# NVIDIA/cuopt

Measured on AMD Instinct MI355X. Metric: pdlp_iterations_per_sec, higher is better.
Workload: dtype f64; 1 GPU; c3: synthetic random sparse LP S(m=1000000,n=1000000,k=10,seed=2), nnz=10000000, longest row 10, CSR fp64/int32, Stable2 preset, tolerances 0 (fixed iteration budget); rows=1000000, cols=1000000, nnz=10000000, parallelism=single GPU

## Files before the change

### cuopt_amd/capi.py

```python
import ctypes as C
import os

import numpy as np

_HERE = os.path.dirname(os.path.abspath(__file__))
LIB_PATH = os.environ.get("CUOPT_AMD_LIB") or os.path.join(_HERE, "lib", "libcuopt.so")

if not os.path.exists(LIB_PATH):
    raise ImportError(
        "cuopt_amd: %s is missing -- build it with `make -C cuopt_amd/csrc` (or "
        "`python -c 'import __graft_entry__ as g; g.build()'`). There is no CPU fallback." % LIB_PATH)

lib = C.CDLL(LIB_PATH, mode=C.RTLD_GLOBAL)

CUOPT_SUCCESS, CUOPT_INVALID_ARGUMENT, CUOPT_MPS_FILE_ERROR, CUOPT_MPS_PARSE_ERROR = 0, 1, 2, 3
CUOPT_VALIDATION_ERROR, CUOPT_OUT_OF_MEMORY, CUOPT_RUNTIME_ERROR = 4, 5, 6
CUOPT_MINIMIZE, CUOPT_MAXIMIZE = 1, -1
STATUS = {0: "NoTermination", 1: "Optimal", 2: "PrimalInfeasible", 3: "DualInfeasible",
          4: "IterationLimit", 5: "TimeLimit", 6: "NumericalError", 7: "PrimalFeasible",
          8: "FeasibleFound", 9: "ConcurrentLimit"}

c_int, c_double, c_void_p, c_char_p = C.c_int32, C.c_double, C.c_void_p, C.c_char_p
P = C.POINTER

# ... 184 lines not shown
for _n in ("cuOptGetObjectiveValue", "cuOptGetSolveTime", "cuOptGetMIPGap", "cuOptGetSolutionBound"):
    _proto(_n, c_int, c_void_p, P(c_double))
_proto("cuOptAmdGetPdlpStats", c_int, c_void_p, P(Result))
_proto("cuOptAmdGetSolveInfo", c_int, c_void_p, c_char_p, c_int)
_proto("cuOptAmdGetName", c_int, c_void_p, c_int, c_int, c_char_p, c_int)

_proto("cuoptamd_last_error", c_char_p)
_proto("cuoptamd_hyper_preset", None, c_int, P(Hyper))
_proto("cuoptamd_default_settings", None, P(SolverSettings))
_proto("cuoptamd_solver_create", c_int, P(c_void_p), P(LP), P(Hyper), P(SolverSettings), c_void_p,
       c_void_p, c_int, c_int, c_int, c_void_p)
_proto("cuoptamd_solver_destroy", None, c_void_p)
_proto("cuoptamd_solver_reset", c_int, c_void_p, c_void_p, c_void_p, c_void_p, c_void_p, P(SolverSettings), c_void_p,
       c_void_p)
_proto("cuoptamd_solver_advance", c_int, c_void_p, c_int, P(Result))
_proto("cuoptamd_solver_get_solution", c_int, c_void_p, c_void_p, c_void_p, c_void_p)
_proto("cuoptamd_solver_device", c_void_p, c_void_p)
_proto("cuoptamd_batch_solve", c_int, c_int, c_void_p, P(Hyper), P(SolverSettings), c_int, c_int, c_void_p, c_void_p, c_void_p, c_void_p)
_proto("cuoptamd_solver_get_warm_start", c_int, c_void_p, P(WarmStart))
_proto("cuoptamd_solver_set_warm_start", c_int, c_void_p, P(WarmStart))
_proto("cuoptamd_warm_start_remap", c_int, P(WarmStart), P(c_int), c_int, P(c_int), c_int, P(WarmStart))
_proto("cuoptamd_solver_row_range", c_int, c_void_p, P(c_int), P(c_int))
_proto("cuoptamd_solver_reorder_info", c_int, c_void_p, c_void_p, c_void_p, c_void_p)
_proto("cuoptamd_partition_rows", None, c_int, c_void_p, c_int, c_void_p)
_proto("cuoptamd_csr_transpose", None, c_int, c_int, *([c_void_p] * 6))

_proto("pdlpdev_last_error", c_char_p)
_proto("pdlpdev_device_count", c_int)
_proto("pdlpdev_device_info", c_int, c_int, c_char_p, c_int, P(c_int), P(C.c_int64))
_proto("pdlpdev_create", c_int, P(c_void_p), c_int, c_int, c_int, *([c_void_p] * 11))
_proto("pdlpdev_destroy", None, c_void_p)
_proto("pdlpdev_comm_unique_id", c_int, c_void_p)
_proto("pdlpdev_comm_init", c_int, c_void_p, c_int, c_int, c_void_p)
_proto("pdlpdev_softcomm_create", c_int, c_int, c_void_p)
_proto("pdlpdev_scaling_compute", c_int, c_void_p, c_int, c_int, c_int, c_double)
_proto("pdlpdev_scale_problem", c_int, c_void_p)
_proto("pdlpdev_init_norms", c_int, c_void_p, c_void_p)
_proto("pdlpdev_problem_norms", c_int, c_void_p, P(c_double), P(c_double))
_proto("pdlpdev_set_step_params", c_int, c_void_p, P(StepParams))
_proto("pdlpdev_set_step", c_int, c_void_p, c_double, c_double)
_proto("pdlpdev_set_k", c_int, c_void_p, c_int)
_proto("pdlpdev_set_initial", c_int, c_void_p, c_void_p, c_void_p)
_proto("pdlpdev_project_primal", c_int, c_void_p)
_proto("pdlpdev_compute_aty", c_int, c_void_p)
_proto("pdlpdev_run", c_int, c_void_p, c_int, P(Ctl))
_proto("pdlpdev_get_ctl", c_int, c_void_p, P(Ctl))
_proto("pdlpdev_clear_error", c_int, c_void_p)
_proto("pdlpdev_set_graph_mode", c_int, c_void_p, c_int)
_proto("pdlpdev_prepare_graphs", c_int, c_void_p)
_proto("pdlpdev_flush_average", c_int, c_void_p)
_proto("pdlpdev_make_average", c_int, c_void_p, c_int)
_proto("pdlpdev_eval", c_int, c_void_p, c_int, c_int, c_double, c_double, c_void_p)
_proto("pdlpdev_restart", c_int, c_void_p, c_int, c_int, c_void_p)
_proto("pdlpdev_save_best", c_int, c_void_p, c_int)
_proto("pdlpdev_trust_region_bounds", c_int, c_void_p, c_int, c_double, c_double, c_double, c_double, c_double, c_double, c_int, c_void_p)
_proto("pdlpdev_eval_infeasibility", c_int, c_void_p, c_int, c_int, c_void_p)
_proto("pdlpdev_get_solution", c_int, c_void_p, c_int, c_void_p, c_void_p, c_void_p)
_proto("pdlpdev_download", C.c_int64, c_void_p, c_int, c_void_p, C.c_int64)
_proto("pdlpdev_spmv", c_int, c_void_p, c_int, c_void_p, c_void_p)
_proto("pdlpdev_time_kernel", c_int, c_void_p, c_int, c_int, P(c_double))
_proto("pdlpdev_synchronize", c_int, c_void_p)
_proto("pdlpdev_device_bytes", C.c_int64, c_void_p)
_proto("cuoptamd_dual_simplex", c_int, c_void_p, c_double, c_int, c_void_p, c_void_p, c_void_p, c_void_p, c_void_p, c_void_p, c_void_p)
_proto("cuoptamd_dual_simplex_from", c_int, c_void_p, c_void_p, c_void_p, c_double, c_int, c_void_p, c_void_p, c_void_p, c_void_p, c_void_p, c_void_p, c_void_p)
_proto("pdlpdev_shard_dataflow", c_int, c_void_p)
_proto("pdlpdev_shard_transport", c_int, c_void_p)
_proto("pdlpdev_shard_wire_bytes", c_int, c_void_p, c_void_p)
_proto("pdlpdev_dense_info", c_int, c_void_p, c_void_p)
_proto("pdlpdev_layout_info", c_int, c_void_p, c_void_p)
_proto("pdlpdev_analyze", c_int, P(c_void_p), c_int, c_int, c_int, c_void_p, c_void_p, c_void_p, c_int)
_proto("pdlpdev_analysis_info", c_int, c_void_p, c_void_p)
_proto("pdlpdev_analysis_maps", c_int, c_void_p, c_void_p, c_void_p)
_proto("pdlpdev_analysis_download", c_int, c_void_p, c_int, c_void_p, c_void_p, c_void_p)
_proto("pdlpdev_create_from_analysis", c_int, P(c_void_p), c_void_p, c_void_p, c_void_p, c_void_p, c_void_p, c_void_p)
_proto("pdlpdev_analysis_destroy", None, c_void_p)
_proto("pdlpdev_debug_sort_pairs", c_int, c_int, C.c_int64, c_void_p, c_void_p, c_int, c_void_p, c_void_p)
_proto("pdlpdev_debug_scan", c_int, c_int, C.c_int64, c_void_p, c_void_p)
_proto("pdlpdev_debug_layout_checksums", c_int, c_void_p, c_void_p)
_proto("cuoptamd_solver_clone", c_int, c_void_p, c_void_p, c_void_p, c_void_p, c_void_p, c_void_p, P(c_void_p))
_proto("cuoptamd_batch_create", c_int, c_void_p, c_int, P(c_void_p))
_proto("cuoptamd_batch_advance", c_int, c_void_p, c_int, c_void_p)
_proto("cuoptamd_batch_destroy", None, c_void_p)
_proto("cuoptamd_batch_reset", c_int, c_void_p, c_void_p, c_void_p, c_void_p, c_void_p)
_proto("cuoptamd_batch_get_solutions", c_int, c_void_p, c_void_p, c_void_p, c_void_p)
_proto("cuoptamd_batch_branch", c_int, c_void_p, c_void_p, c_void_p, c_void_p)
_proto("cuoptamd_batch_solution_views", c_int, c_void_p, c_void_p, c_void_p, c_void_p)
_proto("cuoptamd_batch_device", c_void_p, c_void_p)
_proto("pdlpdev_create_share_stream", None, c_void_p)
_proto("pdlpdev_debug_ipc_export", c_int, c_int, c_int, c_void_p, P(c_void_p))
_proto("pdlpdev_debug_ipc_store", c_int, c_int, c_void_p, c_int, c_double)
_proto("pdlpdev_debug_ipc_wait", c_int, c_int, c_void_p, c_int, c_double)
_proto("pdlpdev_resident_size", c_int, c_int, c_int, C.c_int64)
_proto("pdlpdev_batch_time_kernels", c_int, c_void_p, c_int, c_void_p)
_proto("pdlpdev_synthetic_lp", c_int, c_int, c_int, c_int, c_int, C.c_uint64, *([c_void_p] * 8))

BUF = {n: i for i, n in enumerate(
    ["X", "Y", "X_OTHER", "Y_OTHER", "ATY", "ATY_OTHER", "XBAR", "SUM_X", "SUM_Y", "AVG_X", "AVG_Y",
     "DROW", "DCOL", "A_VALUES", "AT_VALUES", "C", "LB", "UB", "LO", "HI", "RC_CURRENT", "RC_AVERAGE",
     "LAST_RESTART_X", "LAST_RESTART_Y"])}
KERNEL = {n: i for i, n in enumerate(
    ["PRIMAL", "SPMV_A_DUAL", "SPMV_AT_STEP", "STEP_DECISION", "SPMV_A_PLAIN", "SPMV_AT_PLAIN"])}
EV = {n: i for i, n in enumerate(
    ["CX", "DUAL_SUM", "PRES2", "DRES2", "X2", "Y2", "LINF_PRES_REL", "LINF_DRES_REL"])}
CURRENT, AVERAGE = 0, 1


class CuOptError(RuntimeError):
    def __init__(self, code, msg=""):
        super().__init__("cuopt error %d %s" % (code, msg))
        self.code = code


def device_count():
    return int(lib.pdlpdev_device_count())


def device_info(dev=0):
    name = C.create_string_buffer(256)
    cus, mem = c_int(), C.c_int64()
    rc = lib.pdlpdev_device_info(dev, name, 256, C.byref(cus), C.byref(mem))
    if rc != 0:
        raise CuOptError(rc, lib.pdlpdev_last_error().decode())
    return dict(name=name.value.decode(), compute_units=cus.value, hbm_bytes=mem.value)


class Problem:

    def __init__(self, handle):
        self.handle = handle

    @classmethod
    def read(cls, path):
        h = c_void_p()
        rc = lib.cuOptReadProblem(os.fsencode(path), C.byref(h))
        if rc != CUOPT_SUCCESS:
            raise CuOptError(rc, "cuOptReadProblem(%s)" % path)
        return cls(h)

    @classmethod
    def from_dict(cls, p, ranged=True):
        m, n = int(p["m"]), int(p["n"])
        keep = [_i32(p["offsets"]), _i32(p["indices"]), _f64(p["values"]), _f64(p["c"]),
                _f64(p["lb"]), _f64(p["ub"])]
        vt = p.get("var_types")
        vt = (b"C" * n) if vt is None else bytes(bytearray(np.asarray(vt, dtype=np.uint8)))
        h = c_void_p()
        sense = CUOPT_MAXIMIZE if p.get("maximize", False) else CUOPT_MINIMIZE
        off = float(p.get("objective_offset", 0.0))
        if ranged:
            lo, hi = _f64(p["lo"]), _f64(p["hi"])
            rc = lib.cuOptCreateRangedProblem(m, n, sense, off, _ptr(keep[3]), _ptr(keep[0]),
                                              _ptr(keep[1]), _ptr(keep[2]), _ptr(lo), _ptr(hi),
# ... 599 lines not shown
                raise CuOptError(rc, msg)
            self.m, self.n, self.nnz = int(p["m"]), int(p["n"]), len(p["values"])
            return
        m, n = int(p["m"]), int(p["n"])
        off, idx, val = _i32(p["offsets"]), _i32(p["indices"]), _f64(p["values"])
        to, ti, tv = csr_transpose(m, n, off, idx, val)
        c, lo, hi, lb, ub = (_f64(p[k]) for k in ("c", "lo", "hi", "lb", "ub"))
        self.handle = c_void_p()
        rc = lib.pdlpdev_create(C.byref(self.handle), device, m, n, _ptr(off), _ptr(idx), _ptr(val),
                                _ptr(to), _ptr(ti), _ptr(tv), _ptr(c), _ptr(lo), _ptr(hi), _ptr(lb), _ptr(ub))
        if rc != 0:
            msg = lib.pdlpdev_last_error().decode()
            if self.handle:
                lib.pdlpdev_destroy(self.handle)
            self.handle = None
            raise CuOptError(rc, msg)
        self.m, self.n, self.nnz = m, n, len(val)

    def _ck(self, rc):
        if rc != 0:
            raise CuOptError(rc, lib.pdlpdev_last_error().decode())

    def call(self, name, *args):
        self._ck(getattr(lib, "pdlpdev_" + name)(self.handle, *args))

    def ctl(self):
        c = Ctl()
        self._ck(lib.pdlpdev_get_ctl(self.handle, C.byref(c)))
        return c

    def run(self, target_steps):
        c = Ctl()
        self._ck(lib.pdlpdev_run(self.handle, int(target_steps), C.byref(c)))
        return c

    def download(self, name, count):
        out = np.zeros(int(count))
        got = lib.pdlpdev_download(self.handle, BUF[name], _ptr(out), int(count))
        if got < 0:
            raise CuOptError(int(got), lib.pdlpdev_last_error().decode())
        return out[:got]

    def spmv(self, x, transpose=False, rows=None):
        x = _f64(x)
        y = np.zeros(int(rows))
        self._ck(lib.pdlpdev_spmv(self.handle, int(transpose), _ptr(x), _ptr(y)))
        return y

    def eval(self, which, rule_finite=True, eps_p=1e-4, eps_d=1e-4):
        out = np.zeros(len(EV))
        self._ck(lib.pdlpdev_eval(self.handle, which, int(rule_finite), eps_p, eps_d, _ptr(out)))
        return {k: out[i] for k, i in EV.items()}

    def eval_infeasibility(self, which, rule_finite=True):
        out = np.zeros(4)
        self._ck(lib.pdlpdev_eval_infeasibility(self.handle, which, int(rule_finite), _ptr(out)))
        return dict(zip(["max_primal_ray_infeasibility", "primal_ray_linear_objective",
                         "max_dual_ray_infeasibility", "dual_ray_linear_objective"], out.tolist()))

    def trust_region_bounds(self, which, wp, wd, pds=0.5, dds=0.5, primal_weight=1.0, radius=-1.0, scaled_iterates=False):
        out = np.zeros(6)
        self._ck(lib.pdlpdev_trust_region_bounds(self.handle, which, wp, wd, pds, dds, primal_weight, radius,
                                                 int(scaled_iterates), _ptr(out)))
        return dict(zip(["primal_distance2", "dual_distance2", "distance", "lagrangian", "lower_bound",
                         "upper_bound"], out.tolist()))

    def init_norms(self):
        out = np.zeros(3)
        self._ck(lib.pdlpdev_init_norms(self.handle, _ptr(out)))
        return out

    def layout(self):
        out = np.zeros(8, np.int32)
        self._ck(lib.pdlpdev_layout_info(self.handle, _ptr(out)))
        names = {0: "stream", 1: "panel", 2: "resident", 3: "jag", 4: "pb"}

        def side(k):
            d = dict(layout=names[int(out[k])], panels=bool(out[k] == 1), workgroups=int(out[k + 1]))
            if out[k] == 3:
                d["lds_gather_saving_pct"] = int(out[k + 2])
            elif out[k] == 4:
                d["padding_pct"] = int(out[k + 2])
            else:
                d["slabs"] = int(out[k + 2])
                if out[k] == 1:
                    d["row_sums"] = "by_nonzero" if out[6 + k // 3] else "by_row"
            return d
        return dict(A=side(0), At=side(3), resident=bool(out[0] == 2))

    def wire_bytes(self):
        out = np.zeros(3, np.int64)
        self._ck(lib.pdlpdev_shard_wire_bytes(self.handle, _ptr(out)))
        return dict(halo=bool(out[0]), bytes=int(out[1]), bytes_allgather=int(out[2]))

    def layout_checksums(self):
        out = np.zeros(16, np.uint64)
        self._ck(lib.pdlpdev_debug_layout_checksums(self.handle, _ptr(out)))
        return out

    def dense_info(self):
        out = np.zeros(3, np.int64)
        self._ck(lib.pdlpdev_dense_info(self.handle, _ptr(out)))
        return dict(on=bool(out[0]), segments=int(out[1]), entries=int(out[2]))

    def time_kernel(self, kernel, reps=20):
        ms = c_double()
# ... 14 lines not shown
```

### cuopt_amd/csrc/kernels_batch.hip

```cpp
#include <cstring>
#include <hip/hip_runtime.h>

#include "pdlp_ctx.hpp"

#define LAUNCH_CHECK() HIP_TRY(hipGetLastError())

__global__ void k_step_decision_batch(const pdlpdev_decision_args* __restrict__ args);
__global__ void k_set_target(pdlpdev_ctl* ctl, int target);
__global__ void k_set_error(pdlpdev_ctl* ctl);

namespace {

constexpr int kBT = kPanelThreads;
static_assert(kBT == 512, "8 waves of 64 lanes: the reduction below mirrors block_reduce<.., kPanelWaves>");
constexpr int kBatchMax = 16;

struct BatchLp {
  pdlpdev_ctl* ctl;
  double *y0, *y1, *sumy;
  const double *lo, *hi;
  double *x0, *x1, *aty0, *aty1, *sumx;
  const double *c, *lb, *ub;
  pdlpdev_ctx::UniformBounds ubd;
  double *part_a, *part_at;
// ... 777 lines not shown
      const void* f = K == 16 ? batch_jag_kernel<16>(side[t], t == 0) : K == 8 ? batch_jag_kernel<8>(side[t], t == 0)
                    : K == 4  ? batch_jag_kernel<4>(side[t], t == 0)  : batch_jag_kernel<2>(side[t], t == 0);
      HIP_TRY(hipFuncSetAttribute(f, hipFuncAttributeMaxDynamicSharedMemorySize, 160 * 1024));
    }
  pdlpdev_batch* b = new pdlpdev_batch();
  *out      = b;
  b->K = K, b->device = c0->device, b->stream = c0->stream;
  b->a_side = side[0], b->t_side = side[1];
  std::vector<BatchLp>& h = b->lp_host;
  h.resize(K);
  std::vector<pdlpdev_decision_args>& dargs = b->dargs_host;
  dargs.resize(K);
  for (int l = 0; l < K; ++l) {
    pdlpdev_ctx* c = ctx[l];
    b->ctx[l]      = c;
    h[l]     = batch_lp_of(c);
    dargs[l] = pdlpdev_decision_args{c->ctl, c->part_a, side[0].W, c->part_at, side[1].W, c->sp};
    c->batches_alive += 1;
  }
  HIP_TRY(hipMalloc((void**)&b->lp_dev, K * sizeof(BatchLp)));
  HIP_TRY(hipMalloc((void**)&b->xK, ((size_t)c0->n * K + 64) * sizeof(double)));
  HIP_TRY(hipMalloc((void**)&b->yK, ((size_t)c0->m * K + 64) * sizeof(double)));
  HIP_TRY(hipMalloc((void**)&b->dargs_dev, K * sizeof(pdlpdev_decision_args)));
  HIP_TRY(hipMemcpyAsync(b->lp_dev, h.data(), K * sizeof(BatchLp), hipMemcpyHostToDevice, b->stream));
  HIP_TRY(hipMemcpyAsync(b->dargs_dev, dargs.data(), K * sizeof(pdlpdev_decision_args), hipMemcpyHostToDevice, b->stream));
  HIP_TRY(hipMemsetAsync(b->xK, 0, ((size_t)c0->n * K + 64) * sizeof(double), b->stream));
  HIP_TRY(hipMemsetAsync(b->yK, 0, ((size_t)c0->m * K + 64) * sizeof(double), b->stream));
  HIP_TRY(hipStreamSynchronize(b->stream));
  return 0;
}

void pdlpdev_batch_destroy(pdlpdev_batch* b)
{
  if (!b) return;
  for (int l = 0; l < b->K; ++l)
    if (b->ctx[l]) b->ctx[l]->batches_alive -= 1;
  (void)hipSetDevice(b->device);
  if (b->stream) (void)hipStreamSynchronize(b->stream);
  for (auto& kv : b->graphs) (void)hipGraphExecDestroy(kv.second);
  if (b->lp_dev) (void)hipFree(b->lp_dev);
  if (b->dargs_dev) (void)hipFree(b->dargs_dev);
  if (b->xK) (void)hipFree(b->xK);
  if (b->yK) (void)hipFree(b->yK);
  delete b;
}

int pdlpdev_batch_run(pdlpdev_batch* b, const int32_t* targets, pdlpdev_ctl* ctl)
{
  if (!b || !targets) return fail(-1, "pdlpdev_batch_run: null argument");
  roctx::Range range("pdlp: batched PDHG attempts");
  HIP_TRY(hipSetDevice(b->device));
  TRY(batch_refresh_table(b));
  const int K = b->K;
  for (int l = 0; l < K; ++l)
    if (targets[l] > 0) k_set_target<<<1, 1, 0, b->stream>>>(b->ctx[l]->ctl, targets[l]);
  LAUNCH_CHECK();
  TRY(batch_fetch_ctl(b));
  auto wants = [&](int l) { return targets[l] > 0 && b->ctx[l]->ctl_h->error == 0 && b->ctx[l]->ctl_h->steps_taken < targets[l]; };
  int guard = 0;
  for (;;) {
    int remaining = 0;
    int before[kBatchMax], asked[kBatchMax];
    for (int l = 0; l < K; ++l) {
      before[l] = b->ctx[l]->ctl_h->steps_taken;
      asked[l]  = wants(l) ? targets[l] - before[l] : 0;
      remaining = std::max(remaining, asked[l]);
    }
    if (remaining == 0) break;
    const bool use_graph = b->ctx[0]->use_graph != 0;
    while (remaining > 0) {
      int chunk = 1;
      while (chunk * 2 <= remaining && chunk < 64) chunk *= 2;
      if (use_graph) {
        hipGraphExec_t g;
        TRY(batch_graph(b, chunk, &g));
        HIP_TRY(hipGraphLaunch(g, b->stream));
      } else {
        for (int i = 0; i < chunk; ++i) TRY(batch_enqueue(b));
      }
      remaining -= chunk;
    }
    TRY(batch_fetch_ctl(b));
    for (int l = 0; l < K; ++l) {
      if (asked[l] == 0) continue;
      pdlpdev_ctx* c = b->ctx[l];
      c->rejected_in_a_row = c->ctl_h->steps_taken == before[l] ? c->rejected_in_a_row + asked[l] : 0;
      if (c->ctl_h->error == 0 && c->rejected_in_a_row >= 64) {
        c->rejected_in_a_row = 0;
        k_set_error<<<1, 1, 0, b->stream>>>(c->ctl);
        LAUNCH_CHECK();
      }
    }
    TRY(batch_fetch_ctl(b));
    if (++guard > 100000) return fail(-6, "pdlpdev_batch_run: no progress");
  }
  if (ctl)
    for (int l = 0; l < K; ++l) ctl[l] = *b->ctx[l]->ctl_h;
  return 0;
}

int pdlpdev_batch_time_kernels(pdlpdev_batch* b, int reps, double avg_ms[4])
{
  if (!b || !avg_ms) return fail(-1, "pdlpdev_batch_time_kernels: null argument");
  HIP_TRY(hipSetDevice(b->device));
  TRY(batch_refresh_table(b));
  hipStream_t s = b->stream;
  const int K   = b->K;
  if (reps < 1) reps = 1;
  TRY(batch_fetch_ctl(b));
  pdlpdev_ctl saved[kBatchMax], forced[kBatchMax];
  struct Scratch {
    double *sx[kBatchMax] = {nullptr}, *sy[kBatchMax] = {nullptr};
    hipEvent_t ev[8] = {nullptr};
    ~Scratch()
    {
      for (double* p : sx) if (p) (void)hipFree(p);
      for (double* p : sy) if (p) (void)hipFree(p);
      for (hipEvent_t e : ev) if (e) (void)hipEventDestroy(e);
    }
  } scratch;
  double **sx = scratch.sx, **sy = scratch.sy;
  hipEvent_t* ev = scratch.ev;
  for (int l = 0; l < K; ++l) {
    pdlpdev_ctx* c = b->ctx[l];
    saved[l] = forced[l] = *c->ctl_h;
    forced[l].pending_avg = 1, forced[l].target_steps = saved[l].steps_taken + 1, forced[l].error = 0;
    HIP_TRY(hipMalloc((void**)&sx[l], std::max<size_t>(c->n, 1) * sizeof(double)));
    HIP_TRY(hipMalloc((void**)&sy[l], std::max<size_t>(c->m, 1) * sizeof(double)));
    HIP_TRY(hipMemcpyAsync(sx[l], c->sumx, (size_t)c->n * sizeof(double), hipMemcpyDeviceToDevice, s));
    HIP_TRY(hipMemcpyAsync(sy[l], c->sumy, (size_t)c->m * sizeof(double), hipMemcpyDeviceToDevice, s));
  }
  auto arm = [&]() -> int {
    for (int l = 0; l < K; ++l) HIP_TRY(hipMemcpyAsync(b->ctx[l]->ctl, &forced[l], sizeof(pdlpdev_ctl), hipMemcpyHostToDevice, s));
    return 0;
  };
  for (int q = 0; q < 8; ++q) HIP_TRY(hipEventCreate(&ev[q]));
  double sum[4] = {0.0, 0.0, 0.0, 0.0};
  TRY(arm());
  TRY(batch_enqueue(b));
  for (int i = 0; i < reps; ++i) {
    TRY(arm());
    TRY(batch_enqueue(b, ev));
    HIP_TRY(hipStreamSynchronize(s));
    for (int q = 0; q < 4; ++q) {
      float ms = 0.f;
      HIP_TRY(hipEventElapsedTime(&ms, ev[2 * q], ev[2 * q + 1]));
      sum[q] += ms;
    }
  }
  for (int q = 0; q < 4; ++q) avg_ms[q] = sum[q] / reps;
  for (int l = 0; l < K; ++l) {
    pdlpdev_ctx* c = b->ctx[l];
    HIP_TRY(hipMemcpyAsync(c->ctl, &saved[l], sizeof(pdlpdev_ctl), hipMemcpyHostToDevice, s));
    HIP_TRY(hipMemcpyAsync(c->sumx, sx[l], (size_t)c->n * sizeof(double), hipMemcpyDeviceToDevice, s));
    HIP_TRY(hipMemcpyAsync(c->sumy, sy[l], (size_t)c->m * sizeof(double), hipMemcpyDeviceToDevice, s));
  }
  HIP_TRY(hipStreamSynchronize(s));
  return 0;
}

}
```

### cuopt_amd/csrc/kernels_panel.hip

```cpp
#include <hip/hip_runtime.h>

#include "pdlp_kernel_decls.hpp"
#include "pdlp_layouts.hpp"
#include "pdlp_setup.hpp"
#include "spmv_panel.hpp"

template <bool SEG>
__global__ void __launch_bounds__(kPanelThreads)
k_panel_a_dual(PanelView P, const pdlpdev_ctl* __restrict__ ctl, const double* __restrict__ xbar,
               double* __restrict__ y0, double* __restrict__ y1, const double* __restrict__ lo,
               const double* __restrict__ hi, double* __restrict__ sumy, double* __restrict__ part, double* __restrict__ ycopy,
               const p2pdev::Push* __restrict__ push)
{
  if (!loop_active(ctl)) return;
  const int cur = ctl->cur;
  DualEpilogue e{cur ? y1 : y0, cur ? y0 : y1, lo, hi, sumy, ctl->sigma, ctl->step_size,
                 ctl->pending_avg != 0, ycopy, push};
  panel_block<SEG>(P, xbar, e, part);
  if (push) p2pdev::count_exchange(push);
}

template <bool SEG>
__global__ void __launch_bounds__(kPanelThreads)
k_panel_at_step(PanelView P, const pdlpdev_ctl* __restrict__ ctl, const double* __restrict__ y0,
                const double* __restrict__ y1, const double* __restrict__ x0,
                const double* __restrict__ x1, double* __restrict__ aty0, double* __restrict__ aty1,
                double* __restrict__ part)
{
  if (!loop_active(ctl)) return;
  const int cur = ctl->cur;
  StepEpilogue e{cur ? x1 : x0, cur ? x0 : x1, cur ? aty1 : aty0, cur ? aty0 : aty1};
  panel_block<SEG>(P, cur ? y0 : y1 , e, part);
}

template <bool SEG>
__global__ void __launch_bounds__(kPanelThreads)
k_panel_at_cur(PanelView P, const pdlpdev_ctl* __restrict__ ctl, const double* __restrict__ y0,
               const double* __restrict__ y1, double* __restrict__ aty0, double* __restrict__ aty1,
               double* __restrict__ out_override, int use_next)
{
  const int cur = ctl->cur ^ (use_next ? 1 : 0);
  StoreEpilogue e{out_override ? out_override : (cur ? aty1 : aty0)};
  panel_block<SEG>(P, cur ? y1 : y0, e, nullptr);
}

template <bool SEG>
__global__ void __launch_bounds__(kPanelThreads)
k_panel_plain(PanelView P, const double* __restrict__ vec, double* __restrict__ out)
{
  StoreEpilogue e{out};
  panel_block<SEG>(P, vec, e, nullptr);
}

template <bool SEG>
__global__ void __launch_bounds__(kPanelThreads)
k_panel_eval_primal(PanelView P, const pdlpdev_ctl* __restrict__ ctl, int which,
                    const double* __restrict__ x0, const double* __restrict__ x1,
                    const double* __restrict__ avgx, const double* __restrict__ y0,
                    const double* __restrict__ y1, const double* __restrict__ avgy,
                    const double* __restrict__ dr, const double* __restrict__ lo_u,
                    const double* __restrict__ hi_u, double eps_rel, double* __restrict__ linf_rows,
                    double* __restrict__ ax_out, double* __restrict__ part)
{
  const int cur = ctl->cur;
  const double* xv = which == PDLPDEV_AVERAGE ? avgx : (cur ? x1 : x0);
  const double* yv = which == PDLPDEV_AVERAGE ? avgy : (cur ? y1 : y0);
  EvalPrimalEpilogue e{yv, dr, lo_u, hi_u, eps_rel, linf_rows, ax_out};
  panel_block<SEG>(P, xv, e, part);
}

template <bool SEG>
__global__ void __launch_bounds__(kPanelThreads)
k_panel_eval_dual(PanelView P, const pdlpdev_ctl* __restrict__ ctl, int which,
                  const double* __restrict__ x0, const double* __restrict__ x1,
                  const double* __restrict__ avgx, const double* __restrict__ y0,
                  const double* __restrict__ y1, const double* __restrict__ avgy, EvalDualCore core,
                  double* __restrict__ part)
{
  const int cur = ctl->cur;
  core.xhat     = which == PDLPDEV_AVERAGE ? avgx : (cur ? x1 : x0);
  const double* yv = which == PDLPDEV_AVERAGE ? avgy : (cur ? y1 : y0);
  EvalDualEpilogue e{core};
  panel_block<SEG>(P, yv, e, part);
}

template __global__ void k_panel_a_dual<true>(PanelView P, const pdlpdev_ctl* __restrict__ ctl, const double* __restrict__ xbar,
               double* __restrict__ y0, double* __restrict__ y1, const double* __restrict__ lo,
               const double* __restrict__ hi, double* __restrict__ sumy, double* __restrict__ part, double* __restrict__ ycopy,
               const p2pdev::Push* __restrict__ push);
template __global__ void k_panel_a_dual<false>(PanelView P, const pdlpdev_ctl* __restrict__ ctl, const double* __restrict__ xbar,
               double* __restrict__ y0, double* __restrict__ y1, const double* __restrict__ lo,
               const double* __restrict__ hi, double* __restrict__ sumy, double* __restrict__ part, double* __restrict__ ycopy,
               const p2pdev::Push* __restrict__ push);
template __global__ void k_panel_at_step<true>(PanelView P, const pdlpdev_ctl* __restrict__ ctl, const double* __restrict__ y0,
                const double* __restrict__ y1, const double* __restrict__ x0,
                const double* __restrict__ x1, double* __restrict__ aty0, double* __restrict__ aty1,
                double* __restrict__ part);
template __global__ void k_panel_at_step<false>(PanelView P, const pdlpdev_ctl* __restrict__ ctl, const double* __restrict__ y0,
                const double* __restrict__ y1, const double* __restrict__ x0,
                const double* __restrict__ x1, double* __restrict__ aty0, double* __restrict__ aty1,
                double* __restrict__ part);
template __global__ void k_panel_at_cur<true>(PanelView P, const pdlpdev_ctl* __restrict__ ctl, const double* __restrict__ y0,
               const double* __restrict__ y1, double* __restrict__ aty0, double* __restrict__ aty1,
               double* __restrict__ out_override, int use_next);
template __global__ void k_panel_at_cur<false>(PanelView P, const pdlpdev_ctl* __restrict__ ctl, const double* __restrict__ y0,
               const double* __restrict__ y1, double* __restrict__ aty0, double* __restrict__ aty1,
               double* __restrict__ out_override, int use_next);
template __global__ void k_panel_plain<true>(PanelView P, const double* __restrict__ vec, double* __restrict__ out);
template __global__ void k_panel_plain<false>(PanelView P, const double* __restrict__ vec, double* __restrict__ out);
template __global__ void k_panel_eval_primal<true>(PanelView P, const pdlpdev_ctl* __restrict__ ctl, int which,
                    const double* __restrict__ x0, const double* __restrict__ x1,
                    const double* __restrict__ avgx, const double* __restrict__ y0,
                    const double* __restrict__ y1, const double* __restrict__ avgy,
                    const double* __restrict__ dr, const double* __restrict__ lo_u,
                    const double* __restrict__ hi_u, double eps_rel, double* __restrict__ linf_rows,
                    double* __restrict__ ax_out, double* __restrict__ part);
template __global__ void k_panel_eval_primal<false>(PanelView P, const pdlpdev_ctl* __restrict__ ctl, int which,
                    const double* __restrict__ x0, const double* __restrict__ x1,
                    const double* __restrict__ avgx, const double* __restrict__ y0,
                    const double* __restrict__ y1, const double* __restrict__ avgy,
                    const double* __restrict__ dr, const double* __restrict__ lo_u,
                    const double* __restrict__ hi_u, double eps_rel, double* __restrict__ linf_rows,
                    double* __restrict__ ax_out, double* __restrict__ part);
template __global__ void k_panel_eval_dual<true>(PanelView P, const pdlpdev_ctl* __restrict__ ctl, int which,
                  const double* __restrict__ x0, const double* __restrict__ x1,
                  const double* __restrict__ avgx, const double* __restrict__ y0,
                  const double* __restrict__ y1, const double* __restrict__ avgy, EvalDualCore core,
                  double* __restrict__ part);
template __global__ void k_panel_eval_dual<false>(PanelView P, const pdlpdev_ctl* __restrict__ ctl, int which,
                  const double* __restrict__ x0, const double* __restrict__ x1,
                  const double* __restrict__ avgx, const double* __restrict__ y0,
                  const double* __restrict__ y1, const double* __restrict__ avgy, EvalDualCore core,
                  double* __restrict__ part);

int64_t gather_working_set(int32_t rows, int32_t cols, const int32_t* off, const int32_t* idx)
{
// ... 273 lines not shown
```

### cuopt_amd/csrc/pdlp_core_internal.hpp

```cpp
#pragma once
#include "pdlp_ctx.hpp"

#define LAUNCH_CHECK() HIP_TRY(hipGetLastError())

extern "C" {
int fetch_scalars(pdlpdev_ctx* ctx, int count);
int fetch_ctl(pdlpdev_ctx* ctx, pdlpdev_ctl* out);
void launch_plain(pdlpdev_ctx* ctx, int transpose, const double* vec, double* out);
void launch_at_cur(pdlpdev_ctx* ctx, double* out_override, int use_next);
void dense_part(pdlpdev_ctx* ctx, int transpose, const double* v0, const double* v1, int mode, int in_loop);
}

static inline int dual_partials(const pdlpdev_ctx* ctx) { return ctx->pba.on ? ctx->pba.v.B : ctx->ja.on ? ctx->ja.v.nblk + ctx->ja.v.nlong : ctx->pa.on ? ctx->pa.v.W : ctx->a_nb; }
static inline int step_partials(const pdlpdev_ctx* ctx) { return ctx->pbat.on ? ctx->pbat.v.B : ctx->jat.on ? ctx->jat.v.nblk + ctx->jat.v.nlong : ctx->pat.on ? ctx->pat.v.W : ctx->at_nb; }

__global__ void __launch_bounds__(kBlock)
k_flush_average(int n, int m, const pdlpdev_ctl* __restrict__ ctl, const double* __restrict__ x0, const double* __restrict__ x1, const double* __restrict__ y0,
                const double* __restrict__ y1, double* __restrict__ sumx, double* __restrict__ sumy);
__global__ void __launch_bounds__(kBlock) k_finalize(const double* __restrict__ part, int nb, int nq, unsigned op_mask, double* __restrict__ out);
__global__ void __launch_bounds__(kBlock) k_div_inplace(int n, double* __restrict__ v, const double* __restrict__ d);
__global__ void __launch_bounds__(kBlock) k_div_to(int n, double* __restrict__ out, const double* __restrict__ v, const double* __restrict__ d);
__global__ void k_restart_ctl(pdlpdev_ctl* ctl);
__global__ void k_clear_pending(pdlpdev_ctl* ctl);

int sync_panel_values(pdlpdev_ctx* c);
__global__ void __launch_bounds__(kBlock) k_fill(int64_t n, double* __restrict__ d, double v);
__global__ void __launch_bounds__(kBlock) k_scale_vectors(int n, int m, double* __restrict__ c, double* __restrict__ lb, double* __restrict__ ub,
                                                          const double* __restrict__ dc, double* __restrict__ lo, double* __restrict__ hi,
                                                          const double* __restrict__ dr);
__global__ void __launch_bounds__(kBlock) k_scale_matrix(int rows, const int32_t* __restrict__ off, const int32_t* __restrict__ idx, double* __restrict__ val,
                                                         const double* __restrict__ d_self, const double* __restrict__ d_other);
__global__ void __launch_bounds__(kBlock) k_scale_matrix_long(const int32_t* __restrict__ rows_long, const int32_t* __restrict__ off,
                                                              const int32_t* __restrict__ idx, double* __restrict__ val,
                                                              const double* __restrict__ d_self, const double* __restrict__ d_other);
```

### cuopt_amd/csrc/pdlp_create.hip

```cpp
#include "pdlp_ctx.hpp"
#include "pdlp_layouts.hpp"
#include "pdlp_setup.hpp"

__global__ void k_fill(int64_t n, double* __restrict__ d, double v);
int sync_panel_values(pdlpdev_ctx* c);
int resident_tier(int m, int n, int64_t nnz);

static thread_local int g_create_sharded = 0;
static thread_local int g_create_batch_lanes = 0;

static int create_impl(pdlpdev_ctx** out, int device, int32_t m, int32_t n, const int32_t* a_offsets,
                       const int32_t* a_indices, const double* a_values, const int32_t* at_offsets,
                       const int32_t* at_indices, const double* at_values,
                       void (*transpose_ready)(void*), void* user, const double* c, const double* lo,
                       const double* hi, const double* lb, const double* ub, pdlpdev_analysis* an);

extern "C" {

const char* pdlpdev_last_error(void) { return g_err.c_str(); }
void pdlpdev_create_hint(int sharded) { g_create_sharded = sharded; }
void pdlpdev_create_batch_lanes(int lanes) { g_create_batch_lanes = lanes; }
static thread_local pdlpdev_ctx* g_create_stream_donor = nullptr;
void pdlpdev_create_share_stream(pdlpdev_ctx* donor) { g_create_stream_donor = donor; }
int pdlpdev_resident_size(int32_t m, int32_t n, int64_t nnz) { return resident_tier(m, n, nnz) >= 0 ? 1 : 0; }
// ... 445 lines not shown
      rbt = build_row_blocks(n, T.off);
      wlap("row blocks");
      if (walk) at_rc = layout_walk(ctx, P, T);
    };
    struct Join {
      std::thread t;
      ~Join() { if (t.joinable()) t.join(); }
    } worker;
    if (at_thread) worker.t = std::thread(at_side, true);
    {
      LayoutSide A;
      init_side(A, 0);
      A.off = A_off, A.idx = A_idx, A.d_off = ctx->ha_off, A.d_idx = ctx->ha_idx, A.d_val = ctx->ha_val, A.lap = lap;
      A.first_seg = DH.on ? &DH.first_seg : nullptr;
      TRY(layout_walk(ctx, P, A));
      TRY(upload_side(ctx, P, A));
      if (ctx->pa.on && DH.on) TRY(own_segments(ctx, DH, A.ph));
      lap("upload layouts A");
    }
    if (at_thread) worker.t.join();
    else at_side(false);
    lap("wait for the A^T side");
    if ((int64_t)at_offsets[n] != ctx->nnz) return fail(-1, "pdlpdev_create: A and A^T disagree on nnz");
    if (!an) {
      TRY(upload_i32(ctx, &ctx->at_off, at_offsets, (size_t)n + 1));
      TRY(upload_i32(ctx, &ctx->at_idx, at_indices, nnz, 8));
      TRY(upload_f64(ctx, &ctx->at_val, at_values, nnz, 8));
    }
    ctx->at_nlong = (int)lat.size();
    if (ctx->at_nlong) TRY(upload_i32(ctx, &ctx->at_long, lat.data(), lat.size()));
    const bool hot_t = !hT_off.empty();
    ctx->hat_off = ctx->at_off, ctx->hat_idx = ctx->at_idx, ctx->hat_val = ctx->at_val;
    ctx->hot_nnz_at = (int64_t)T.off[n];
    if (hot_t) {
      TRY(upload_i32(ctx, &ctx->hat_off, T.off, (size_t)n + 1));
      TRY(upload_i32(ctx, &ctx->hat_idx, T.idx, (size_t)ctx->hot_nnz_at, 8));
      TRY(dev_alloc(ctx, &ctx->hat_val, (size_t)ctx->hot_nnz_at + 8));
      TRY(upload_i32(ctx, &ctx->dense.s_perm_at, hT_perm.data(), hT_perm.size()));
    }
    if (DH.on) TRY(dev_alloc(ctx, &ctx->dense.add_n, (size_t)n));
    ctx->at_nb = (int)rbt.size() / 2 - 1;
    TRY(upload_i32(ctx, &ctx->at_rb, rbt.data(), rbt.size()));
    lap("upload A^T");
    T.d_off = ctx->hat_off, T.d_idx = ctx->hat_idx, T.d_val = ctx->hat_val;
    TRY(at_thread ? at_rc : layout_walk(ctx, P, T));
    TRY(upload_side(ctx, P, T));
    if (ctx->pat.on && DH.on) TRY(column_segments(ctx, DH, T.ph));
    lap("upload layouts A^T");
    HIP_TRY(hipStreamSynchronize(ctx->stream));
  }
  {
    const char* small_env = getenv("CUOPT_AMD_SMALL");
    const int tier        = resident_tier(m, n, ctx->nnz);
    ctx->small_resident   = tier >= 0 && !(small_env && atoi(small_env) == 0) && !ctx->dense.add_m && !ctx->dense.add_n;
    if (small_env && atoi(small_env) != 0 && tier < 0)
      return fail(-1, "CUOPT_AMD_SMALL=1: the LP does not fit the resident kernel (m, n <= 2048, nnz <= 4096 ...)");
  }
  ctx->pa.v.dense_add = ctx->ja.v.dense_add = ctx->pba.v.dense_add = ctx->dense.add_m;
  ctx->pat.v.dense_add = ctx->jat.v.dense_add = ctx->pbat.v.dense_add = ctx->dense.add_n;
  if (ctx->pa.v.dn_own_seg) ctx->pa.v.dense_add = nullptr;
  if (ctx->pat.v.dn_pan_ptr) ctx->pat.v.dense_add = nullptr;
  ctx->slab_cap += slab_rest;
  TRY(dev_alloc(ctx, &ctx->part_a, (size_t)8 * std::max({ctx->a_nb, ctx->pba.on ? ctx->pba.v.B : 0, ctx->pa.on ? ctx->pa.v.W : 0, ctx->ja.on ? ctx->ja.v.nblk + ctx->ja.v.nlong : 0, 1})));
  TRY(dev_alloc(ctx, &ctx->part_at, (size_t)8 * std::max({ctx->at_nb, ctx->pbat.on ? ctx->pbat.v.B : 0, ctx->pat.on ? ctx->pat.v.W : 0, ctx->jat.on ? ctx->jat.v.nblk + ctx->jat.v.nlong : 0, 1})));
  TRY(dev_alloc(ctx, &ctx->part_g, (size_t)8 * 2048));
  TRY(dev_alloc(ctx, &ctx->scal, kScalars));
  TRY(dev_alloc(ctx, &ctx->ctl, 1));
  TRY(dev_alloc(ctx, &ctx->ar_buf, (size_t)n + kSlicePad));
  lap("partial buffers");
  k_fill<<<grid_for(m), kBlock, 0, ctx->stream>>>(m, ctx->dr, 1.0);
  k_fill<<<grid_for(n), kBlock, 0, ctx->stream>>>(n, ctx->dc, 1.0);
  HIP_TRY(hipGetLastError());
  lap("fill D");
  TRY(sync_panel_values(ctx));
  lap("panel values (permute)");
  if (P.mode == LayoutPolicy::kTimed) {
    TRY(pick_layout(ctx, &ctx->pa, m, ctx->a_nb, ctx->a_rb, ctx->ha_off, ctx->ha_idx, ctx->ha_val, ctx->tmp_n, ctx->tmp_m, "A"));
    lap("layout autotune A");
    TRY(pick_layout(ctx, &ctx->pat, n, ctx->at_nb, ctx->at_rb, ctx->hat_off, ctx->hat_idx, ctx->hat_val, ctx->tmp_m, ctx->tmp_n, "A^T"));
    lap("layout autotune");
  }
  HIP_TRY(hipStreamSynchronize(ctx->stream));
  scratch_free(ctx);
  return 0;
}

extern "C" {

void pdlpdev_destroy(pdlpdev_ctx* ctx)
{
  if (!ctx) return;
  (void)hipSetDevice(ctx->device);
  if (ctx->stream) (void)hipStreamSynchronize(ctx->stream);
  scratch_free(ctx);
  for (auto& kv : ctx->graphs) (void)hipGraphExecDestroy(kv.second);
  if (ctx->shared_with_parent && ctx->parent) ctx->parent->clones_alive -= 1;
  if (ctx->batches_alive > 0)
    fprintf(stderr, "[cuopt_amd] pdlpdev_destroy: %d batch(es) still hold this context -- destroy the batch before its members\n", ctx->batches_alive);
  if (ctx->clones_alive > 0)
    fprintf(stderr, "[cuopt_amd] pdlpdev_destroy: %d clone(s) of this context are still alive -- they alias its matrices and must be destroyed first\n", ctx->clones_alive);
  for (void* mapped : ctx->p2p.opened) (void)hipIpcCloseMemHandle(mapped);
  if (ctx->p2p.base) (void)hipFree(ctx->p2p.base);
  if (ctx->comm && !ctx->soft) comm_cache::release(ctx->comm_key);
  for (void* p : ctx->allocs) (void)hipFree(p);
  const bool whole = ctx->stream && ctx->scal_h && ctx->first_chunk && !ctx->shared_with_parent && !ctx->stream_borrowed;
  if (!(whole && give_recycled(Recycled{ctx->device, ctx->stream, ctx->scal_h, ctx->first_chunk}))) {
// ... 9 lines not shown
```

### cuopt_amd/csrc/pdlp_ctx.hpp

```cpp
#pragma once
#include <hip/hip_runtime.h>
#include <hip/hip_ext.h>

#include <tuple>
#include <utility>

#include <dlfcn.h>
#include <unistd.h>
#include <mutex>
#include <math.h>
#include <stdarg.h>
#include <stdio.h>
#include <string.h>

#include <algorithm>
#include <chrono>
#include <map>
#include <memory>
#include <string>
#include <vector>

#include "host_parallel.hpp"
#include "pdlp_kernels.hpp"
#include "pdlp_epilogues.hpp"
// ... 327 lines not shown
  double *lrx = nullptr, *lry = nullptr, *rc[2] = {nullptr, nullptr};
  double *tmp_n = nullptr, *tmp_m = nullptr;
  double *ax_u[3] = {nullptr, nullptr, nullptr}, *aty_u[3] = {nullptr, nullptr, nullptr};
  double* rc_scratch = nullptr;
  double *bestx = nullptr, *besty = nullptr, *bestrc = nullptr;
  double *part_a = nullptr, *part_at = nullptr;
  double *part_g = nullptr;
  double *scal = nullptr;
  double *scal_h = nullptr;
  pdlpdev_ctl *ctl = nullptr, *ctl_h = nullptr;
  pdlpdev_step_params sp = {0.3, 0.6, 0.5, 0.5};
  rccl::comm_t comm = nullptr;
  softcomm::Comm* soft = nullptr;
  std::string comm_key;
  int rank = 0, world = 1;
  double* ar_buf = nullptr;
  bool rsag = false;
  int slice = 0;
  double* rs_buf = nullptr;
  double* rs_scal = nullptr;
  bool owner = false;
  int ypad = 0;
  double* ygather = nullptr;
  int32_t oc_rows = 0;
  int64_t oc_nnz = 0;
  int32_t *oc_off = nullptr, *oc_idx = nullptr, *oc_rb = nullptr, *oc_long = nullptr;
  double* oc_val = nullptr;
  int oc_nb = 0, oc_nlong = 0;
  Panels poc;
  Jag joc;
  double* part_oc = nullptr;
  struct Halo {
    bool on = false;
    std::vector<int32_t> recv_off[2], recv_cnt[2], send_off[2], send_cnt[2];
    int64_t bytes = 0, bytes_allgather = 0;
  } halo;
  struct P2P {
    bool on = false;
    char* base = nullptr;
    size_t bytes = 0;
    size_t off_x = 0, off_y = 0, off_s = 0, off_f = 0;
    p2pdev::Peers peers{};
    std::vector<void*> opened;
    unsigned long long* epoch = nullptr;
    int* fault = nullptr;
    p2pdev::Push* push_dev = nullptr;
    p2pdev::Push push_host[p2pdev::kKinds];
  } p2p;
  bool prof_armed = false;
  static constexpr int kProfPairs = 8;
  hipEvent_t prof_ev[2 * kProfPairs] = {};
  int prof_used = 0;
  int rejected_in_a_row = 0;
  int use_graph = 1;
  int batch_lanes = 0;
  bool comm_warm = false;
  bool graph_comm_failed = false;
  char* slab = nullptr;
  size_t slab_cap = 0, slab_used = 0;
  char* arena = nullptr;
  char* first_chunk = nullptr;
  bool stream_borrowed = false;
  size_t arena_used = 0;
  bool small_resident = false;
  bool shared_with_parent = false;
  pdlpdev_ctx* parent = nullptr;
  bool rows_aliased = false;
  int clones_alive = 0;
  bool rows_private = false;
  int batches_alive = 0;
  std::map<int, hipGraphExec_t> graphs;
  std::vector<void*> allocs;
  int64_t bytes = 0;
  struct Scratch {
    void* p;
    size_t bytes;
    bool busy;
  };
  std::vector<Scratch> scratch;
};
inline int scratch_take(pdlpdev_ctx* c, void** p, size_t bytes)
{
  bytes = std::max<size_t>(bytes, 256);
  for (auto& b : c->scratch)
    if (!b.busy && b.bytes >= bytes && b.bytes <= 2 * bytes + 4096) {
      b.busy = true;
      *p     = b.p;
      return 0;
    }
  HIP_TRY(hipMalloc(p, bytes));
  c->scratch.push_back(pdlpdev_ctx::Scratch{*p, bytes, true});
  return 0;
}
inline void scratch_release(pdlpdev_ctx* c, void* p)
{
  for (auto& b : c->scratch)
    if (b.p == p) b.busy = false;
}
inline void scratch_free(pdlpdev_ctx* c)
{
  for (auto& b : c->scratch) (void)hipFree(b.p);
  c->scratch.clear();
}

struct pdlpdev_decision_args {
  pdlpdev_ctl* ctl;
  const double* part_dy;
  int nb_dy;
  const double* part_t;
  int nb_t;
  pdlpdev_step_params sp;
};

constexpr int kGenericBlocks = 1024;
constexpr int kScalars       = 64;

struct PerDeviceOnce {
  std::mutex m;
  bool done[64] = {};
  template <class F>
  int run(int device, F&& f)
  {
    std::lock_guard<std::mutex> lock(m);
    if (device < 0 || device >= 64) return f();
    if (done[device]) return 0;
    const int rc = f();
    if (rc == 0) done[device] = true;
    return rc;
  }
};

struct Recycled {
  int device;
  hipStream_t stream;
  double* pinned;
  char* chunk;
};
inline std::mutex g_recycle_mutex;
inline std::vector<Recycled> g_recycled;
inline bool take_recycled(int device, Recycled* out)
{
  std::lock_guard<std::mutex> lock(g_recycle_mutex);
  for (size_t i = 0; i < g_recycled.size(); ++i)
    if (g_recycled[i].device == device) {
      *out = g_recycled[i];
      g_recycled.erase(g_recycled.begin() + i);
      return true;
    }
  return false;
}
inline bool give_recycled(const Recycled& r)
{
  std::lock_guard<std::mutex> lock(g_recycle_mutex);
  if (g_recycled.size() >= 16) return false;
  g_recycled.push_back(r);
  return true;
}

constexpr size_t kArenaChunk = (size_t)1 << 20, kArenaMaxItem = (size_t)256 << 10;
template <class T>
inline int dev_alloc(pdlpdev_ctx* c, T** p, size_t count)
{
  size_t bytes = std::max<size_t>(count, 1) * sizeof(T);
  c->bytes += (int64_t)bytes;
  if (bytes <= kArenaMaxItem) {
    const size_t need = (bytes + 255) & ~(size_t)255;
    if (c->arena == nullptr || c->arena_used + need > kArenaChunk) {
      HIP_TRY(hipMalloc((void**)&c->arena, kArenaChunk));
// ... 48 lines not shown
```

### cuopt_amd/csrc/pdlp_device.hip

```cpp
#include "pdlp_ctx.hpp"
#include "pdlp_layouts.hpp"
#include "pdlp_setup.hpp"


__global__ void __launch_bounds__(kBlock) k_fill(int64_t n, double* __restrict__ d, double v)
{
  for (int64_t i = blockIdx.x * (int64_t)kBlock + threadIdx.x; i < n; i += (int64_t)gridDim.x * kBlock)
    d[i] = v;
}
__global__ void __launch_bounds__(kBlock) k_scale_vectors(int n, int m, double* __restrict__ c,
                                                          double* __restrict__ lb,
                                                          double* __restrict__ ub,
                                                          const double* __restrict__ dc,
                                                          double* __restrict__ lo,
                                                          double* __restrict__ hi,
                                                          const double* __restrict__ dr)
{
  const int tot = n > m ? n : m;
  for (int i = blockIdx.x * kBlock + threadIdx.x; i < tot; i += gridDim.x * kBlock) {
    if (i < n) {
      c[i]  = c[i] * dc[i];
      lb[i] = lb[i] / dc[i];
      ub[i] = ub[i] / dc[i];
    }
// ... 190 lines not shown
{
  if (!loop_active(ctl)) return;
  {
    __shared__ double red[3 * 8];
    double acc[3] = {0.0, 0.0, 0.0};
    for (int i = threadIdx.x; i < nb_dy; i += kBlock) acc[0] += part_dy[i];
    for (int i = threadIdx.x; i < nb_t; i += kBlock) {
      acc[1] += part_t[i];
      acc[2] += part_t[nb_t + i];
    }
    block_reduce<SumOp, 3>(acc, red);
    if (threadIdx.x == 0) {
      for (int q = 0; q < push->world; ++q) {
        double* d = push->slot(q);
        p2pdev::put(d, acc[0]), p2pdev::put(d + 1, acc[1]), p2pdev::put(d + 2, acc[2]);
      }
      asm volatile("s_waitcnt vmcnt(0)" ::: "memory");
      push->epoch[push->kind] = push->epoch[push->kind] + 1;
      p2pdev::raise(push);
    }
    __syncthreads();
  }
  if (!p2pdev::wait_flags(flags, world, 2, epoch)) {
    if (threadIdx.x == 0) *fault = 1, ctl->error = 1;
    return;
  }
  if (threadIdx.x != 0) return;
  double sum[3] = {0.0, 0.0, 0.0};
  for (int q = 0; q < world; ++q)
    for (int k = 0; k < 3; ++k) sum[k] += __hip_atomic_load(landed + 4 * q + k, __ATOMIC_RELAXED, __HIP_MEMORY_SCOPE_SYSTEM);
  pdlpdev_ctl lc = *ctl;
  apply_step_decision(&lc, sum[0], sum[1], sum[2], sp);
  *ctl = lc;
}

__global__ void __launch_bounds__(kBlock)
k_permute_pad(int64_t n, const int32_t* __restrict__ perm, const double* __restrict__ src, double* __restrict__ dst)
{
  for (int64_t i = blockIdx.x * (int64_t)kBlock + threadIdx.x; i < n; i += (int64_t)gridDim.x * kBlock) {
    const int32_t k = perm[i];
    dst[i]          = k >= 0 ? src[k] : 0.0;
  }
}
__global__ void __launch_bounds__(kBlock)
k_permute(int64_t n, const int32_t* __restrict__ perm, const double* __restrict__ src, double* __restrict__ dst)
{
  for (int64_t i = blockIdx.x * (int64_t)kBlock + threadIdx.x; i < n; i += (int64_t)gridDim.x * kBlock)
    dst[i] = src[perm[i]];
}

__global__ void __launch_bounds__(kBlock)
k_flush_average(int n, int m, const pdlpdev_ctl* __restrict__ ctl, const double* __restrict__ x0,
                const double* __restrict__ x1, const double* __restrict__ y0,
                const double* __restrict__ y1, double* __restrict__ sumx, double* __restrict__ sumy)
{
  if (ctl->pending_avg == 0) return;
  const int cur           = ctl->cur;
  const double w          = ctl->step_size;
  const double* __restrict__ x = cur ? x1 : x0;
  const double* __restrict__ y = cur ? y1 : y0;
  const int tot = n > m ? n : m;
  for (int i = blockIdx.x * kBlock + threadIdx.x; i < tot; i += gridDim.x * kBlock) {
    if (i < n) sumx[i] = sumx[i] + w * x[i];
    if (i < m) sumy[i] = sumy[i] + w * y[i];
  }
}
__global__ void k_clear_pending(pdlpdev_ctl* ctl) { ctl->pending_avg = 0; }

__global__ void __launch_bounds__(kBlock)
k_sum_partials_to(const double* __restrict__ part, int nb, double* __restrict__ out)
{
  __shared__ double red[8];
  double acc[1] = {0.0};
  for (int i = threadIdx.x; i < nb; i += kBlock) acc[0] += part[i];
  block_reduce<SumOp, 1>(acc, red);
  if (threadIdx.x == 0) out[0] = acc[0];
}

__global__ void __launch_bounds__(kBlock)
k_pack_step_sums(const double* __restrict__ part_dy, int nb_dy, const double* __restrict__ part_t, int nb_t, double* __restrict__ out)
{
  __shared__ double red[3 * 8];
  double acc[3] = {0.0, 0.0, 0.0};
  for (int i = threadIdx.x; i < nb_dy; i += kBlock) acc[0] += part_dy[i];
  for (int i = threadIdx.x; i < nb_t; i += kBlock) {
    acc[1] += part_t[i];
    acc[2] += part_t[nb_t + i];
  }
  block_reduce<SumOp, 3>(acc, red);
  if (threadIdx.x == 0) {
    out[0] = acc[0], out[1] = acc[1], out[2] = acc[2];
  }
}

__global__ void k_restart_ctl(pdlpdev_ctl* ctl)
{
  ctl->sum_weights       = 0.0;
  ctl->its_since_restart = 0;
  ctl->pending_avg       = 0;
}
__global__ void k_set_step(pdlpdev_ctl* ctl, double step, double w)
{
  if (step >= 0.0) ctl->step_size = step;
  ctl->primal_weight = w;
  ctl->tau           = ctl->step_size / w;
  ctl->sigma         = ctl->step_size * w;
}
__global__ void k_set_target(pdlpdev_ctl* ctl, int target) { ctl->target_steps = target; }
__global__ void k_set_k(pdlpdev_ctl* ctl, int k) { ctl->k = k; }
// ... 125 lines not shown
                        (mode == LayoutPolicy::kAuto && gcols * 8 > P.ws_limit && gather_working_set(nc, (int32_t)gcols, off, ridx.data()) > P.ws_limit);
    if (nc > 0 && !ctx->joc.on && panels) {
      PanelHost h = build_panels(nc, (int32_t)gcols, off, ridx.data(), P.slab_bytes, true);
      TRY(upload_panels(ctx, &ctx->poc, h, ctx->oc_off, ctx->oc_idx, ctx->oc_val));
    }
  }
  TRY(dev_alloc(ctx, &ctx->part_oc, (size_t)8 * std::max(oc_partials(ctx), 1)));
  {
    const char* tr = getenv("CUOPT_AMD_SHARD_TRANSPORT");
    if (tr && std::string(tr) == "p2p") TRY(p2p_setup(ctx));
    else if (tr && std::string(tr) != "collective") return fail(-1, "CUOPT_AMD_SHARD_TRANSPORT must be collective or p2p");
  }
  if (ctx->poc.on) k_permute<<<grid_for(ctx->poc.nent), kBlock, 0, s>>>(ctx->poc.nent, ctx->poc.perm, ctx->oc_val, ctx->poc.val);
  if (ctx->joc.on) k_permute<<<grid_for(ctx->joc.nent), kBlock, 0, s>>>(ctx->joc.nent, ctx->joc.perm, ctx->oc_val, ctx->joc.val);
  HIP_TRY(hipGetLastError());
  {
    const int W = ctx->world;
    std::vector<int32_t> need((size_t)4 * W, 0), xl(W, 0x7fffffff), xh(W, -1);
    int32_t *d_lo = nullptr, *d_hi = nullptr;
    TRY(dev_alloc(ctx, &d_lo, 16));
    TRY(dev_alloc(ctx, &d_hi, 16));
    HIP_TRY(hipMemcpyAsync(d_lo, xl.data(), W * sizeof(int32_t), hipMemcpyHostToDevice, s));
    HIP_TRY(hipMemcpyAsync(d_hi, xh.data(), W * sizeof(int32_t), hipMemcpyHostToDevice, s));
    if (ctx->nnz > 0) k_slice_ranges<<<grid_for(ctx->nnz, 8), kBlock, 0, s>>>(ctx->nnz, ctx->a_idx, ctx->slice, W, d_lo, d_hi);
    HIP_TRY(hipMemcpyAsync(xl.data(), d_lo, W * sizeof(int32_t), hipMemcpyDeviceToHost, s));
    HIP_TRY(hipMemcpyAsync(xh.data(), d_hi, W * sizeof(int32_t), hipMemcpyDeviceToHost, s));
    HIP_TRY(hipStreamSynchronize(s));
    std::vector<int32_t> yl(W, 0x7fffffff), yh(W, -1);
    for (int64_t k = 0; k < nnz; ++k) {
      const int32_t pos = ridx[(size_t)k];
      const int q       = pos / ctx->ypad;
      yl[q] = std::min(yl[q], pos), yh[q] = std::max(yh[q], pos);
    }
    for (int q = 0; q < W; ++q) {
      need[(size_t)4 * q + 0] = xh[q] >= 0 ? xl[q] : 0, need[(size_t)4 * q + 1] = xh[q] >= 0 ? xh[q] + 1 : 0;
      need[(size_t)4 * q + 2] = yh[q] >= 0 ? yl[q] : 0, need[(size_t)4 * q + 3] = yh[q] >= 0 ? yh[q] + 1 : 0;
    }
    TRY(halo_setup(ctx, need.data()));
  }
  HIP_TRY(hipStreamSynchronize(s));
  return 0;
}

int fetch_scalars(pdlpdev_ctx* ctx, int count)
{
  HIP_TRY(hipMemcpyAsync(ctx->scal_h, ctx->scal, count * sizeof(double), hipMemcpyDeviceToHost, ctx->stream));
  HIP_TRY(hipStreamSynchronize(ctx->stream));
  return 0;
}
int fetch_ctl(pdlpdev_ctx* ctx, pdlpdev_ctl* out)
{
  HIP_TRY(hipMemcpyAsync(ctx->ctl_h, ctx->ctl, sizeof(pdlpdev_ctl), hipMemcpyDeviceToHost, ctx->stream));
  HIP_TRY(hipStreamSynchronize(ctx->stream));
  if (out) *out = *ctx->ctl_h;
  return 0;
}


static int reduce_vec(pdlpdev_ctx* ctx, int mode, int64_t n, const double* a, const double* b, int slot)
{
  const int g = std::min(grid_for(n), kGenericBlocks);
  switch (mode) {
    case 0: k_reduce<0><<<g, kBlock, 0, ctx->stream>>>(n, a, b, ctx->part_g); break;
    case 1: k_reduce<1><<<g, kBlock, 0, ctx->stream>>>(n, a, b, ctx->part_g); break;
    case 2: k_reduce<2><<<g, kBlock, 0, ctx->stream>>>(n, a, b, ctx->part_g); break;
    default: k_reduce<3><<<g, kBlock, 0, ctx->stream>>>(n, a, b, ctx->part_g); break;
  }
  k_finalize<<<1, kBlock, 0, ctx->stream>>>(ctx->part_g, g, 1, mode == 0 ? 1u : 0u, ctx->scal + slot);
  LAUNCH_CHECK();
  return 0;
}

int pdlpdev_agree_max(pdlpdev_ctx* ctx, double* value)
{
  if (!ctx->comm) return 0;
  HIP_TRY(hipSetDevice(ctx->device));
  HIP_TRY(hipMemcpyAsync(ctx->scal + 60, value, sizeof(double), hipMemcpyHostToDevice, ctx->stream));
  TRY(allreduce(ctx, ctx->scal + 60, 1, rccl::kMax));
  HIP_TRY(hipMemcpyAsync(ctx->scal_h + 60, ctx->scal + 60, sizeof(double), hipMemcpyDeviceToHost, ctx->stream));
  HIP_TRY(hipStreamSynchronize(ctx->stream));
  *value = ctx->scal_h[60];
  return 0;
}

int pdlpdev_init_norms(pdlpdev_ctx* ctx, double out[3])
{
  HIP_TRY(hipSetDevice(ctx->device));
  TRY(reduce_vec(ctx, 0, ctx->nnz, ctx->a_val, nullptr, 0));
  TRY(reduce_vec(ctx, 1, ctx->n, ctx->c, nullptr, 1));
  TRY(reduce_vec(ctx, 2, ctx->m, ctx->lo, ctx->hi, 2));
  TRY(allreduce(ctx, ctx->scal + 0, 1, rccl::kMax));
  TRY(allreduce(ctx, ctx->scal + 2, 1, rccl::kSum));
  TRY(fetch_scalars(ctx, 3));
  out[0] = ctx->scal_h[0], out[1] = ctx->scal_h[1], out[2] = ctx->scal_h[2];
  return 0;
}

int pdlpdev_reset(pdlpdev_ctx* ctx, const double* lb, const double* ub, const double* lo, const double* hi)
{
  HIP_TRY(hipSetDevice(ctx->device));
  if (!ctx->scaled) return fail(-1, "pdlpdev_reset: the problem has not been scaled yet");
  ctx->rejected_in_a_row = 0;
  hipStream_t s = ctx->stream;
  const size_t nb = (size_t)ctx->n * sizeof(double), mb = (size_t)ctx->m * sizeof(double);
  auto put = [&](const double* src, double* unscaled, double* scaled, size_t bytes) -> int {
    if (!src || bytes == 0) return 0;
    HIP_TRY(hipMemcpyAsync(unscaled, src, bytes, hipMemcpyHostToDevice, s));
    HIP_TRY(hipMemcpyAsync(scaled, unscaled, bytes, hipMemcpyDeviceToDevice, s));
    return 0;
  };
  TRY(put(lb, ctx->lb_u, ctx->lb, nb));
  TRY(put(ub, ctx->ub_u, ctx->ub, nb));
  {
    const pdlpdev_ctx::UniformBounds before = ctx->ubd;
    ctx->note_uniform_bounds(lb, ub);
    const pdlpdev_ctx::UniformBounds& now = ctx->ubd;
    if (before.lb_same != now.lb_same || before.ub_same != now.ub_same || (now.lb_same && before.lb != now.lb) || (now.ub_same && before.ub != now.ub)) {
      for (auto& kv : ctx->graphs) (void)hipGraphExecDestroy(kv.second);
      ctx->graphs.clear();
    }
  }
  if ((lo || hi) && (ctx->rows_aliased || (ctx->clones_alive > 0 && !ctx->rows_private))) {
    for (double** v : {&ctx->lo, &ctx->lo_u, &ctx->hi, &ctx->hi_u}) {
      const double* src = *v;
      TRY(dev_alloc(ctx, v, (size_t)ctx->m));
      HIP_TRY(hipMemcpyAsync(*v, src, mb, hipMemcpyDeviceToDevice, s));
    }
    ctx->rows_aliased = false;
    ctx->rows_private = true;
    for (auto& kv : ctx->graphs) (void)hipGraphExecDestroy(kv.second);
    ctx->graphs.clear();
  }
  TRY(put(lo, ctx->lo_u, ctx->lo, mb));
  TRY(put(hi, ctx->hi_u, ctx->hi, mb));
  if (lb || ub || lo || hi)
    k_scale_bounds<<<grid_for(std::max(ctx->m, ctx->n)), kBlock, 0, s>>>(ctx->n, ctx->m, lb ? ctx->lb : nullptr, ub ? ctx->ub : nullptr,
                                                                      ctx->dc, lo ? ctx->lo : nullptr, hi ? ctx->hi : nullptr, ctx->dr);
  for (int i = 0; i < 2; ++i) {
    HIP_TRY(hipMemsetAsync(ctx->x[i], 0, nb, s));
    HIP_TRY(hipMemsetAsync(ctx->aty[i], 0, nb, s));
    HIP_TRY(hipMemsetAsync(ctx->rc[i], 0, nb, s));
    HIP_TRY(hipMemsetAsync(ctx->y[i], 0, mb, s));
  }
  for (double* v : {ctx->xbar, ctx->sumx, ctx->avgx, ctx->lrx}) HIP_TRY(hipMemsetAsync(v, 0, nb, s));
  for (double* v : {ctx->sumy, ctx->avgy, ctx->lry}) HIP_TRY(hipMemsetAsync(v, 0, mb, s));
  HIP_TRY(hipMemsetAsync(ctx->ctl, 0, sizeof(pdlpdev_ctl), s));
  LAUNCH_CHECK();
  return 0;
}
int pdlpdev_weight_norms(pdlpdev_ctx* ctx, int unscaled, double out[2])
{
  HIP_TRY(hipSetDevice(ctx->device));
  TRY(reduce_vec(ctx, 1, ctx->n, unscaled ? ctx->c_u : ctx->c, nullptr, 1));
  TRY(reduce_vec(ctx, 2, ctx->m, unscaled ? ctx->lo_u : ctx->lo, unscaled ? ctx->hi_u : ctx->hi, 2));
  TRY(allreduce(ctx, ctx->scal + 2, 1, rccl::kSum));
  TRY(fetch_scalars(ctx, 3));
  out[0] = ctx->scal_h[1], out[1] = ctx->scal_h[2];
  return 0;
}


int pdlpdev_problem_norms(pdlpdev_ctx* ctx, double* norm_c, double* norm_b)
{
  HIP_TRY(hipSetDevice(ctx->device));
  TRY(reduce_vec(ctx, 1, ctx->n, ctx->c_u, nullptr, 0));
  TRY(reduce_vec(ctx, 2, ctx->m, ctx->lo_u, ctx->hi_u, 1));
  TRY(allreduce(ctx, ctx->scal + 1, 1, rccl::kSum));
  TRY(fetch_scalars(ctx, 2));
  if (norm_c) *norm_c = sqrt(ctx->scal_h[0]);
  if (norm_b) *norm_b = sqrt(ctx->scal_h[1]);
  return 0;
}

int pdlpdev_set_step_params(pdlpdev_ctx* ctx, const pdlpdev_step_params* p)
{
  ctx->sp = *p;
  for (auto& kv : ctx->graphs) (void)hipGraphExecDestroy(kv.second);
  ctx->graphs.clear();
  return 0;
}
int pdlpdev_set_step(pdlpdev_ctx* ctx, double step_size, double primal_weight)
{
  HIP_TRY(hipSetDevice(ctx->device));
  k_set_step<<<1, 1, 0, ctx->stream>>>(ctx->ctl, step_size, primal_weight);
  LAUNCH_CHECK();
  return 0;
}
int pdlpdev_set_k(pdlpdev_ctx* ctx, int32_t k)
{
  HIP_TRY(hipSetDevice(ctx->device));
  k_set_k<<<1, 1, 0, ctx->stream>>>(ctx->ctl, k);
  LAUNCH_CHECK();
  return 0;
}
int pdlpdev_set_initial(pdlpdev_ctx* ctx, const double* x, const double* y)
{
  HIP_TRY(hipSetDevice(ctx->device));
  TRY(fetch_ctl(ctx, nullptr));
  const int cur = ctx->ctl_h->cur;
  if (x) {
    HIP_TRY(hipMemcpyAsync(ctx->x[cur], x, (size_t)ctx->n * sizeof(double), hipMemcpyHostToDevice, ctx->stream));
    k_div_inplace<<<grid_for(ctx->n), kBlock, 0, ctx->stream>>>(ctx->n, ctx->x[cur], ctx->dc);
  }
  if (y) {
    HIP_TRY(hipMemcpyAsync(ctx->y[cur], y, (size_t)ctx->m * sizeof(double), hipMemcpyHostToDevice, ctx->stream));
    k_div_inplace<<<grid_for(ctx->m), kBlock, 0, ctx->stream>>>(ctx->m, ctx->y[cur], ctx->dr);
  }
  LAUNCH_CHECK();
  HIP_TRY(hipStreamSynchronize(ctx->stream));
  return 0;
}
}
extern "C" {
int pdlpdev_initial_solution_stats(pdlpdev_ctx* ctx, double out[5], const double* x0_unscaled, const double* y0_unscaled)
{
  HIP_TRY(hipSetDevice(ctx->device));
  if ((x0_unscaled == nullptr) != (y0_unscaled == nullptr)) return fail(-1, "initial_solution_stats: both unscaled vectors or none");
  hipStream_t s = ctx->stream;
  const int n = ctx->n, m = ctx->m;
  TRY(fetch_ctl(ctx, nullptr));
  const int cur = ctx->ctl_h->cur;
  const double *xv = ctx->x[cur], *yv = ctx->y[cur], *atyv = ctx->aty[cur];
  if (x0_unscaled) {
    const int nxt = 1 - cur;
    HIP_TRY(hipMemcpyAsync(ctx->x[nxt], x0_unscaled, (size_t)n * sizeof(double), hipMemcpyHostToDevice, s));
    HIP_TRY(hipMemcpyAsync(ctx->y[nxt], y0_unscaled, (size_t)m * sizeof(double), hipMemcpyHostToDevice, s));
    double* prod = ctx->comm ? ctx->ar_buf : ctx->aty[nxt];
    launch_plain(ctx, 1, ctx->y[nxt], prod);
    LAUNCH_CHECK();
    if (ctx->comm) TRY(allreduce(ctx, prod, (size_t)n, rccl::kSum));
    xv = ctx->x[nxt], yv = ctx->y[nxt], atyv = prod;
  } else {
    TRY(pdlpdev_compute_aty(ctx));
  }
  const int g = std::min(grid_for(n), kGenericBlocks);
  k_dot<<<g, kBlock, 0, s>>>(n, xv, atyv, ctx->part_g);
  k_finalize<<<1, kBlock, 0, s>>>(ctx->part_g, g, 1, 0u, ctx->scal + 48);
  TRY(reduce_vec(ctx, 1, n, xv, nullptr, 49));
  TRY(reduce_vec(ctx, 1, m, yv, nullptr, 50));
  TRY(reduce_vec(ctx, 0, n, xv, nullptr, 51));
  TRY(reduce_vec(ctx, 0, m, yv, nullptr, 52));
  LAUNCH_CHECK();
  if (ctx->comm) {
    TRY(allreduce(ctx, ctx->scal + 50, 1, rccl::kSum));
    TRY(allreduce(ctx, ctx->scal + 52, 1, rccl::kMax));
  }
  HIP_TRY(hipMemcpyAsync(ctx->scal_h + 48, ctx->scal + 48, 5 * sizeof(double), hipMemcpyDeviceToHost, s));
  HIP_TRY(hipStreamSynchronize(s));
  for (int i = 0; i < 5; ++i) out[i] = ctx->scal_h[48 + i];
  return 0;
}
// ... 187 lines not shown
    launch_a_dual(ctx);
    launch_at_cur(ctx, ctx->ar_buf, 1);
    LAUNCH_CHECK();
    TRY(reduce_scatter(ctx, ctx->ar_buf, ctx->rs_buf, (size_t)ctx->slice));
    const int g = std::min(grid_for(len), kGenericBlocks);
    launch_k(ctx, k_step_stats, g, kBlock, 0, len, g, ctx->ctl, ctx->rs_buf, ctx->x[0] + cs, ctx->x[1] + cs, ctx->aty[0] + cs, ctx->aty[1] + cs, ctx->part_g);
    launch_k(ctx, k_pack_step_sums, 1, kBlock, 0, ctx->part_a, dual_partials(ctx), ctx->part_g, g, ctx->rs_scal);
    LAUNCH_CHECK();
    TRY(allreduce(ctx, ctx->rs_scal, 3, rccl::kSum));
    launch_k(ctx, k_step_decision, 1, kDecisionThreads, 0, ctx->ctl, nullptr, 0, ctx->rs_scal + 1, 1, ctx->rs_scal, ctx->sp);
    LAUNCH_CHECK();
    return 0;
  }
  launch_k(ctx, k_primal, grid_for(n), kBlock, 0, n, ctx->ctl, ctx->x[0], ctx->x[1], ctx->aty[0], ctx->aty[1], ctx->c, ctx->lb, ctx->ub, ctx->xbar, ctx->sumx, (const p2pdev::Push*)nullptr, ctx->ubd);
  launch_a_dual(ctx);
  if (!ctx->comm) {
    launch_at_step(ctx);
    launch_decision(ctx);
  } else {
    launch_at_cur(ctx, ctx->ar_buf, 1);
    launch_k(ctx, k_sum_partials_to, 1, kBlock, 0, ctx->part_a, dual_partials(ctx), ctx->ar_buf + n);
    LAUNCH_CHECK();
    TRY(allreduce(ctx, ctx->ar_buf, (size_t)n + 1, rccl::kSum));
    const int g = std::min(grid_for(n), kGenericBlocks);
    launch_k(ctx, k_step_stats, g, kBlock, 0, n, g, ctx->ctl, ctx->ar_buf, ctx->x[0], ctx->x[1], ctx->aty[0], ctx->aty[1], ctx->part_g);
    launch_k(ctx, k_step_decision, 1, kDecisionThreads, 0, ctx->ctl, nullptr, 0, ctx->part_g, g, ctx->ar_buf + n, ctx->sp);
  }
  LAUNCH_CHECK();
  return 0;
}

static int get_graph(pdlpdev_ctx* ctx, int attempts, hipGraphExec_t* out)
{
  auto it = ctx->graphs.find(attempts);
  if (it != ctx->graphs.end()) {
    *out = it->second;
    return 0;
  }
  hipGraph_t graph;
  HIP_TRY(hipStreamBeginCapture(ctx->stream, hipStreamCaptureModeThreadLocal));
  int rc = 0;
  for (int i = 0; i < attempts && rc == 0; ++i) rc = enqueue_attempt(ctx);
  hipError_t e = hipStreamEndCapture(ctx->stream, &graph);
  if (rc != 0) return rc;
  HIP_TRY(e);
  hipGraphExec_t exec;
  HIP_TRY(hipGraphInstantiate(&exec, graph, nullptr, nullptr, 0));
  HIP_TRY(hipGraphDestroy(graph));
  ctx->graphs[attempts] = exec;
  *out                  = exec;
  return 0;
}

int pdlpdev_run(pdlpdev_ctx* ctx, int32_t target_steps, pdlpdev_ctl* ctl)
{
  roctx::Range range("pdlp: PDHG attempts");
  HIP_TRY(hipSetDevice(ctx->device));
  if (ctx->small_resident && !ctx->comm) {
    TRY(resident_run(ctx, target_steps));
    if (ctl) *ctl = *ctx->ctl_h;
    return 0;
  }
  k_set_target<<<1, 1, 0, ctx->stream>>>(ctx->ctl, target_steps);
  LAUNCH_CHECK();
  TRY(fetch_ctl(ctx, nullptr));
  int guard = 0;
  while (ctx->ctl_h->error == 0 && ctx->ctl_h->steps_taken < target_steps) {
    int remaining = target_steps - ctx->ctl_h->steps_taken;
    const bool rccl_graphs = ctx->comm && !ctx->p2p.on && !ctx->soft && !ctx->graph_comm_failed;
    bool replayed = false;
    if (rccl_graphs && ctx->use_graph && !ctx->comm_warm) {
      TRY(enqueue_attempt(ctx));
      ctx->comm_warm = true;
      remaining -= 1;
    }
    if (ctx->use_graph && (!ctx->comm || ctx->p2p.on || rccl_graphs)) {
      replayed = true;
      while (remaining > 0) {
        int chunk = 1;
        while (chunk * 2 <= remaining && chunk < 64) chunk *= 2;
        hipGraphExec_t g;
        const int grc = get_graph(ctx, chunk, &g);
        if (grc != 0 && rccl_graphs) {
          ctx->graph_comm_failed = true;
          (void)hipGetLastError();
          replayed = false;
          break;
        }
        TRY(grc);
        HIP_TRY(hipGraphLaunch(g, ctx->stream));
        remaining -= chunk;
      }
    }
    if (!replayed) {
      for (int i = 0; i < remaining; ++i) TRY(enqueue_attempt(ctx));
    }
    const int before = ctx->ctl_h->steps_taken, asked = target_steps - before;
    TRY(fetch_ctl(ctx, nullptr));
    if (ctx->p2p.on && ctx->ctl_h->error != 0) {
      int fault = 0;
      HIP_TRY(hipMemcpy(&fault, ctx->p2p.fault, sizeof(int), hipMemcpyDeviceToHost));
      if (fault) return fail(-6, "direct peer transport: rank %d waited 5 s for another rank's data (a peer failed or is stuck)", ctx->rank);
    }
    ctx->rejected_in_a_row = ctx->ctl_h->steps_taken == before ? ctx->rejected_in_a_row + asked : 0;
    if (ctx->ctl_h->error == 0 && ctx->rejected_in_a_row >= 64) {
      ctx->rejected_in_a_row = 0;
      k_set_error<<<1, 1, 0, ctx->stream>>>(ctx->ctl);
      LAUNCH_CHECK();
      TRY(fetch_ctl(ctx, nullptr));
    }
    if (++guard > 100000) return fail(-6, "pdlpdev_run: no progress");
  }
  if (ctx->rsag && guard > 0) {
    const int cur = ctx->ctl_h->cur;
    TRY(all_gather(ctx, ctx->x[cur], (size_t)ctx->slice));
    TRY(all_gather(ctx, ctx->aty[cur], (size_t)ctx->slice));
    TRY(all_gather(ctx, ctx->sumx, (size_t)ctx->slice));
  }
  if (ctl) *ctl = *ctx->ctl_h;
  return 0;
}

int pdlpdev_copy_in(void* dst, const void* src, size_t bytes)
{
  if (bytes == 0) return 0;
  if (!dst || !src) return fail(-1, "pdlpdev_copy_in: null pointer");
  hipPointerAttribute_t attr;
  memset(&attr, 0, sizeof(attr));
  const hipError_t e = hipPointerGetAttributes(&attr, src);
  if (e == hipSuccess && (attr.type == hipMemoryTypeDevice || attr.type == hipMemoryTypeManaged)) {
    HIP_TRY(hipMemcpy(dst, src, bytes, hipMemcpyDeviceToHost));
    return 0;
  }
  (void)hipGetLastError();
  memcpy(dst, src, bytes);
  return 0;
}

void pdlpdev_range_push(const char* name)
{
  roctx::load();
  if (roctx::Push) roctx::Push(name);
}
void pdlpdev_range_pop(void)
{
  if (roctx::Pop) roctx::Pop();
}

int pdlpdev_prepare_graphs(pdlpdev_ctx* ctx)
{
  HIP_TRY(hipSetDevice(ctx->device));
  if (!ctx->use_graph || (ctx->comm && !ctx->p2p.on) || ctx->small_resident) return 0;
  for (int chunk = 1; chunk <= 64; chunk *= 2) {
    hipGraphExec_t g;
    TRY(get_graph(ctx, chunk, &g));
  }
  return 0;
}

int pdlpdev_get_ctl(pdlpdev_ctx* ctx, pdlpdev_ctl* ctl)
{
  HIP_TRY(hipSetDevice(ctx->device));
  return fetch_ctl(ctx, ctl);
}
int pdlpdev_clear_error(pdlpdev_ctx* ctx)
{
  HIP_TRY(hipSetDevice(ctx->device));
  k_clear_error<<<1, 1, 0, ctx->stream>>>(ctx->ctl);
  LAUNCH_CHECK();
  return 0;
}
int pdlpdev_set_graph_mode(pdlpdev_ctx* ctx, int use_graph)
{
  ctx->use_graph = use_graph;
  return 0;
}

int pdlpdev_get_solution(pdlpdev_ctx* ctx, int which, double* x, double* y, double* rc)
{
  HIP_TRY(hipSetDevice(ctx->device));
  TRY(fetch_ctl(ctx, nullptr));
  const int cur = ctx->ctl_h->cur;
  hipStream_t s = ctx->stream;
  if (which == PDLPDEV_BEST) {
    if (!ctx->bestx) return fail(-1, "pdlpdev_get_solution(BEST): nothing was saved");
    if (x) {
      k_unscale<<<grid_for(ctx->n), kBlock, 0, s>>>(ctx->n, ctx->bestx, ctx->dc, ctx->tmp_n);
      HIP_TRY(hipMemcpyAsync(x, ctx->tmp_n, (size_t)ctx->n * sizeof(double), hipMemcpyDeviceToHost, s));
    }
    if (y) {
      k_unscale<<<grid_for(ctx->m), kBlock, 0, s>>>(ctx->m, ctx->besty, ctx->dr, ctx->tmp_m);
      HIP_TRY(hipMemcpyAsync(y, ctx->tmp_m, (size_t)ctx->m * sizeof(double), hipMemcpyDeviceToHost, s));
    }
    if (rc) HIP_TRY(hipMemcpyAsync(rc, ctx->bestrc, (size_t)ctx->n * sizeof(double), hipMemcpyDeviceToHost, s));
    LAUNCH_CHECK();
    HIP_TRY(hipStreamSynchronize(s));
    return 0;
  }
  if (x) {
    k_unscale<<<grid_for(ctx->n), kBlock, 0, s>>>(ctx->n, which == PDLPDEV_AVERAGE ? ctx->avgx : ctx->x[cur], ctx->dc, ctx->tmp_n);
    HIP_TRY(hipMemcpyAsync(x, ctx->tmp_n, (size_t)ctx->n * sizeof(double), hipMemcpyDeviceToHost, s));
  }
  if (y) {
    k_unscale<<<grid_for(ctx->m), kBlock, 0, s>>>(ctx->m, which == PDLPDEV_AVERAGE ? ctx->avgy : ctx->y[cur], ctx->dr, ctx->tmp_m);
    HIP_TRY(hipMemcpyAsync(y, ctx->tmp_m, (size_t)ctx->m * sizeof(double), hipMemcpyDeviceToHost, s));
  }
  if (rc)
    HIP_TRY(hipMemcpyAsync(rc, ctx->rc[which == PDLPDEV_AVERAGE ? 1 : 0], (size_t)ctx->n * sizeof(double), hipMemcpyDeviceToHost, s));
  LAUNCH_CHECK();
  HIP_TRY(hipStreamSynchronize(s));
  return 0;
}

static int64_t locate_buffer(pdlpdev_ctx* ctx, int id, double** ptr)
{
  if (hipSetDevice(ctx->device) != hipSuccess) return -2;
  if (fetch_ctl(ctx, nullptr) != 0) return -2;
  const int cur = ctx->ctl_h->cur;
  double* src   = nullptr;
  int64_t count = 0;
  const int64_t n = ctx->n, m = ctx->m, nnz = ctx->nnz;
  switch (id) {
    case PDLPDEV_BUF_X: src = ctx->x[cur], count = n; break;
    case PDLPDEV_BUF_Y: src = ctx->y[cur], count = m; break;
    case PDLPDEV_BUF_X_OTHER: src = ctx->x[cur ^ 1], count = n; break;
    case PDLPDEV_BUF_Y_OTHER: src = ctx->y[cur ^ 1], count = m; break;
    case PDLPDEV_BUF_ATY: src = ctx->aty[cur], count = n; break;
    case PDLPDEV_BUF_ATY_OTHER: src = ctx->aty[cur ^ 1], count = n; break;
    case PDLPDEV_BUF_XBAR: src = ctx->xbar, count = n; break;
    case PDLPDEV_BUF_SUM_X: src = ctx->sumx, count = n; break;
    case PDLPDEV_BUF_SUM_Y: src = ctx->sumy, count = m; break;
    case PDLPDEV_BUF_AVG_X: src = ctx->avgx, count = n; break;
    case PDLPDEV_BUF_AVG_Y: src = ctx->avgy, count = m; break;
    case PDLPDEV_BUF_DROW: src = ctx->dr, count = m; break;
    case PDLPDEV_BUF_DCOL: src = ctx->dc, count = n; break;
    case PDLPDEV_BUF_A_VALUES: src = ctx->a_val, count = nnz; break;
    case PDLPDEV_BUF_AT_VALUES: src = ctx->at_val, count = nnz; break;
    case PDLPDEV_BUF_C: src = ctx->c, count = n; break;
    case PDLPDEV_BUF_LB: src = ctx->lb, count = n; break;
    case PDLPDEV_BUF_UB: src = ctx->ub, count = n; break;
    case PDLPDEV_BUF_LO: src = ctx->lo, count = m; break;
    case PDLPDEV_BUF_HI: src = ctx->hi, count = m; break;
    case PDLPDEV_BUF_RC_CURRENT: src = ctx->rc[0], count = n; break;
    case PDLPDEV_BUF_RC_AVERAGE: src = ctx->rc[1], count = n; break;
    case PDLPDEV_BUF_LAST_RESTART_X: src = ctx->lrx, count = n; break;
    case PDLPDEV_BUF_LAST_RESTART_Y: src = ctx->lry, count = m; break;
    default: fail(-1, "unknown buffer %d", id); return -1;
  }
  *ptr = src;
  return count;
}

int64_t pdlpdev_download(pdlpdev_ctx* ctx, int id, void* host, int64_t max_elements)
{
  double* src   = nullptr;
  int64_t count = locate_buffer(ctx, id, &src);
  if (count < 0) return count;
  count = std::min(count, max_elements);
  if (count > 0) {
    if (hipMemcpyAsync(host, src, (size_t)count * sizeof(double), hipMemcpyDeviceToHost, ctx->stream) != hipSuccess) return -2;
    if (hipStreamSynchronize(ctx->stream) != hipSuccess) return -2;
  }
  return count;
}

int64_t pdlpdev_upload(pdlpdev_ctx* ctx, int id, const void* host, int64_t elements)
{
  double* dst   = nullptr;
  int64_t count = locate_buffer(ctx, id, &dst);
  if (count < 0) return count;
  if (id == PDLPDEV_BUF_A_VALUES || id == PDLPDEV_BUF_AT_VALUES) {
    fail(-1, "matrix values cannot be overwritten");
    return -1;
  }
  count = std::min(count, elements);
  if ((id == PDLPDEV_BUF_LB && ctx->ubd.lb_same) || (id == PDLPDEV_BUF_UB && ctx->ubd.ub_same)) {
    if (id == PDLPDEV_BUF_LB) ctx->ubd.lb_same = 0;
    else ctx->ubd.ub_same = 0;
    for (auto& kv : ctx->graphs) (void)hipGraphExecDestroy(kv.second);
    ctx->graphs.clear();
  }
  if (count > 0) {
    if (hipMemcpyAsync(dst, host, (size_t)count * sizeof(double), hipMemcpyHostToDevice, ctx->stream) != hipSuccess) return -2;
    if (hipStreamSynchronize(ctx->stream) != hipSuccess) return -2;
  }
  return count;
}

int pdlpdev_set_loop_state(pdlpdev_ctx* ctx, double sum_weights, int32_t its_since_restart, int32_t k)
{
  HIP_TRY(hipSetDevice(ctx->device));
  k_set_loop_state<<<1, 1, 0, ctx->stream>>>(ctx->ctl, sum_weights, its_since_restart, k);
  LAUNCH_CHECK();
  return 0;
}

int pdlpdev_spmv(pdlpdev_ctx* ctx, int transpose, const double* x, double* y)
{
  HIP_TRY(hipSetDevice(ctx->device));
  hipStream_t s  = ctx->stream;
  const int rows = transpose ? ctx->n : ctx->m, cols = transpose ? ctx->m : ctx->n;
  double* in     = transpose ? ctx->tmp_m : ctx->tmp_n;
  double* outv   = transpose ? ctx->tmp_n : ctx->tmp_m;
  HIP_TRY(hipMemcpyAsync(in, x, (size_t)cols * sizeof(double), hipMemcpyHostToDevice, s));
  launch_plain(ctx, transpose, in, outv);
  LAUNCH_CHECK();
  HIP_TRY(hipMemcpyAsync(y, outv, (size_t)rows * sizeof(double), hipMemcpyDeviceToHost, s));
  HIP_TRY(hipStreamSynchronize(s));
  return 0;
}

int pdlpdev_time_kernel(pdlpdev_ctx* ctx, int kernel_id, int reps, double* avg_ms)
{
  HIP_TRY(hipSetDevice(ctx->device));
  hipStream_t s = ctx->stream;
  if (reps < 1) reps = 1;
  TRY(fetch_ctl(ctx, nullptr));
  pdlpdev_ctl saved = *ctx->ctl_h;
  pdlpdev_ctl forced = saved;
  forced.pending_avg  = 1;
  forced.target_steps = saved.steps_taken + 1;
  forced.error        = 0;
  double *sx = nullptr, *sy = nullptr;
  HIP_TRY(hipMalloc((void**)&sx, std::max<size_t>(ctx->n, 1) * sizeof(double)));
  HIP_TRY(hipMalloc((void**)&sy, std::max<size_t>(ctx->m, 1) * sizeof(double)));
  HIP_TRY(hipMemcpyAsync(sx, ctx->sumx, (size_t)ctx->n * sizeof(double), hipMemcpyDeviceToDevice, s));
  HIP_TRY(hipMemcpyAsync(sy, ctx->sumy, (size_t)ctx->m * sizeof(double), hipMemcpyDeviceToDevice, s));
  HIP_TRY(hipMemcpyAsync(ctx->ctl, &forced, sizeof(forced), hipMemcpyHostToDevice, s));
  HIP_TRY(hipStreamSynchronize(s));
  for (hipEvent_t& e : ctx->prof_ev) HIP_TRY(hipEventCreate(&e));
  auto one = [&]() {
    switch (kernel_id) {
      case PDLPDEV_K_PRIMAL:
        launch_k(ctx, k_primal, grid_for(ctx->n), kBlock, 0, ctx->n, ctx->ctl, ctx->x[0], ctx->x[1], ctx->aty[0], ctx->aty[1], ctx->c, ctx->lb, ctx->ub, ctx->xbar, ctx->sumx, (const p2pdev::Push*)nullptr, ctx->ubd);
        break;
      case PDLPDEV_K_SPMV_A_DUAL: launch_a_dual(ctx); break;
      case PDLPDEV_K_SPMV_AT_STEP: launch_at_step(ctx); break;
      case PDLPDEV_K_STEP_DECISION: launch_decision(ctx); break;
      case PDLPDEV_K_SPMV_A_PLAIN:
        launch_plain(ctx, 0, ctx->xbar, ctx->tmp_m);
        break;
      case PDLPDEV_K_SPMV_AT_PLAIN:
        launch_plain(ctx, 1, ctx->y[saved.cur], ctx->tmp_n);
        break;
      default: return fail(-1, "pdlpdev_time_kernel: unknown kernel %d", kernel_id);
    }
    return 0;
  };
  const bool loop_kernel = kernel_id == PDLPDEV_K_PRIMAL || kernel_id == PDLPDEV_K_SPMV_A_DUAL ||
                           kernel_id == PDLPDEV_K_SPMV_AT_STEP || kernel_id == PDLPDEV_K_STEP_DECISION;
  auto attempt = [&](bool timed) -> int {
    const int order[4] = {PDLPDEV_K_PRIMAL, PDLPDEV_K_SPMV_A_DUAL, PDLPDEV_K_SPMV_AT_STEP, PDLPDEV_K_STEP_DECISION};
    const int wanted   = kernel_id;
    const int slot = loop_kernel ? wanted : (wanted == PDLPDEV_K_SPMV_A_PLAIN ? PDLPDEV_K_SPMV_A_DUAL : PDLPDEV_K_SPMV_AT_STEP);
    int rc = 0;
    for (int id : order) {
      const bool mine = id == slot;
      kernel_id       = mine ? wanted : id;
      ctx->prof_armed = mine && timed;
      if (ctx->prof_armed) ctx->prof_used = 0;
      rc              = one();
      ctx->prof_armed = false;
      if (rc != 0) break;
      if (id == PDLPDEV_K_STEP_DECISION)
        HIP_TRY(hipMemcpyAsync(ctx->ctl, &forced, sizeof(forced), hipMemcpyHostToDevice, s));
    }
    kernel_id = wanted;
    return rc;
  };
  TRY(attempt(false));
// ... 130 lines not shown
```

### cuopt_amd/csrc/pdlp_eval.hip

```cpp
#include "pdlp_ctx.hpp"
#include "pdlp_layouts.hpp"
#include "pdlp_setup.hpp"
#include "pdlp_launch.hpp"
#include "pdlp_core_internal.hpp"

__global__ void __launch_bounds__(kBlock)
k_make_average(int n, int m, int mode, const pdlpdev_ctl* __restrict__ ctl,
               const double* __restrict__ x0, const double* __restrict__ x1,
               const double* __restrict__ y0, const double* __restrict__ y1,
               const double* __restrict__ sumx, const double* __restrict__ sumy,
               double* __restrict__ avgx, double* __restrict__ avgy)
{
  const int cur = ctl->cur;
  const double* __restrict__ x = cur ? x1 : x0;
  const double* __restrict__ y = cur ? y1 : y0;
  const double sw = ctl->sum_weights;
  const int tot   = n > m ? n : m;
  for (int i = blockIdx.x * kBlock + threadIdx.x; i < tot; i += gridDim.x * kBlock) {
    if (i < n) avgx[i] = mode == 0 ? x[i] : (mode == 1 ? 0.0 : sumx[i] / sw);
    if (i < m) avgy[i] = mode == 0 ? y[i] : (mode == 1 ? 0.0 : sumy[i] / sw);
  }
}


__global__ void __launch_bounds__(kBlock)
k_eval_dual_elementwise(int n, int nbg, const pdlpdev_ctl* __restrict__ ctl, int which,
                        const double* __restrict__ x0, const double* __restrict__ x1,
                        const double* __restrict__ avgx, const double* __restrict__ reduced,
                        EvalDualCore core, double* __restrict__ part)
{
  __shared__ double red[20];
  const int cur = ctl->cur;
  core.xhat     = which == PDLPDEV_AVERAGE ? avgx : (cur ? x1 : x0);
  double acc[4] = {0.0, 0.0, 0.0, 0.0};
  for (int j = blockIdx.x * kBlock + threadIdx.x; j < n; j += gridDim.x * kBlock)
    core.col(j, reduced[j], acc);
  block_reduce<SumOp, 4>(acc, red);
  if (threadIdx.x == 0)
    for (int q = 0; q < 4; ++q) part[(size_t)q * nbg + blockIdx.x] = acc[q];
}
__global__ void __launch_bounds__(kBlock)
k_max_partials(int n, const double* __restrict__ v, double* __restrict__ part)
{
  __shared__ double red[8];
  double acc[1] = {0.0};
  for (int i = blockIdx.x * kBlock + threadIdx.x; i < n; i += gridDim.x * kBlock)
    acc[0] = v[i] > acc[0] ? v[i] : acc[0];
  block_reduce<MaxOp, 1>(acc, red);
  if (threadIdx.x == 0) part[blockIdx.x] = acc[0];
}


__global__ void __launch_bounds__(kBlock)
k_infeas_rows(int m, int nbg, const pdlpdev_ctl* __restrict__ ctl, int which, const double* __restrict__ ax,
              const double* __restrict__ y0, const double* __restrict__ y1, const double* __restrict__ avgy,
              const double* __restrict__ dr, const double* __restrict__ lo_u, const double* __restrict__ hi_u,
              double* __restrict__ part)
{
  __shared__ double red[12];
  const int cur = ctl->cur;
  const double* __restrict__ yv = which == PDLPDEV_AVERAGE ? avgy : (cur ? y1 : y0);
  double mx[2] = {0.0, 0.0}, sm[1] = {0.0};
  for (int i = blockIdx.x * kBlock + threadIdx.x; i < m; i += gridDim.x * kBlock) {
    const double lo = lo_u[i], hi = hi_u[i];
    const double hl = dfinite(lo) ? 0.0 : lo, hu = dfinite(hi) ? 0.0 : hi;
// ... 158 lines not shown
__global__ void __launch_bounds__(kBlock) k_tr_pass(TrPoint P, double t, int nbg, double* __restrict__ part)
{
  __shared__ double red[12];
  double sm[2] = {0.0, 0.0};
  const int N = P.n + P.m;
  for (int k = P.first + blockIdx.x * kBlock + threadIdx.x; k < N; k += gridDim.x * kBlock) {
    const TrElem e = tr_element(P, k);
    if (e.dir == 0.0) continue;
    if (e.thr <= t) {
      const double tp = dmin(dmax(e.center + t * e.dir, e.lb), e.ub);
      const double d  = tp - e.center;
      sm[0] += (d * d) * e.w;
    } else {
      sm[1] += (e.dir * e.dir) * e.w;
    }
  }
  block_reduce<SumOp, 2>(sm, red);
  if (threadIdx.x == 0) {
    part[blockIdx.x]       = sm[0];
    part[nbg + blockIdx.x] = sm[1];
  }
}
__global__ void __launch_bounds__(kBlock) k_tr_final(TrPoint P, double t, int nbg, double* __restrict__ part)
{
  __shared__ double red[12];
  double sm[2] = {0.0, 0.0};
  const int N = P.n + P.m;
  for (int k = P.first + blockIdx.x * kBlock + threadIdx.x; k < N; k += gridDim.x * kBlock) {
    const TrElem e = tr_element(P, k);
    double tr      = e.center;
    if (e.dir != 0.0) tr = dmin(dmax(e.center + t * e.dir, e.lb), e.ub);
    sm[k < P.n ? 0 : 1] += (tr - e.center) * e.grad;
  }
  block_reduce<SumOp, 2>(sm, red);
  if (threadIdx.x == 0) {
    part[blockIdx.x]       = sm[0];
    part[nbg + blockIdx.x] = sm[1];
  }
}

__global__ void __launch_bounds__(kBlock)
k_restart(int n, int m, int which, int unscaled, const double* __restrict__ dc, const double* __restrict__ dr,
          const pdlpdev_ctl* __restrict__ ctl, double* __restrict__ x0,
          double* __restrict__ x1, double* __restrict__ y0, double* __restrict__ y1,
          const double* __restrict__ avgx, const double* __restrict__ avgy, double* __restrict__ lrx,
          double* __restrict__ lry, double* __restrict__ sumx, double* __restrict__ sumy,
          double* __restrict__ part)
{
  __shared__ double red[12];
  const RestartView R{n, m, which, unscaled, dc, dr, ctl, x0, x1, y0, y1, avgx, avgy, lrx, lry, sumx, sumy, part};
  restart_block(R, blockIdx.x, gridDim.x, red);
}

extern "C" {

int pdlpdev_flush_average(pdlpdev_ctx* ctx)
{
  HIP_TRY(hipSetDevice(ctx->device));
  k_flush_average<<<grid_for(std::max(ctx->n, ctx->m)), kBlock, 0, ctx->stream>>>(ctx->n, ctx->m, ctx->ctl, ctx->x[0], ctx->x[1], ctx->y[0], ctx->y[1], ctx->sumx, ctx->sumy);
  k_clear_pending<<<1, 1, 0, ctx->stream>>>(ctx->ctl);
  LAUNCH_CHECK();
  return 0;
}
int pdlpdev_make_average(pdlpdev_ctx* ctx, int mode)
{
  HIP_TRY(hipSetDevice(ctx->device));
  k_make_average<<<grid_for(std::max(ctx->n, ctx->m)), kBlock, 0, ctx->stream>>>(ctx->n, ctx->m, mode, ctx->ctl, ctx->x[0], ctx->x[1], ctx->y[0], ctx->y[1], ctx->sumx, ctx->sumy, ctx->avgx, ctx->avgy);
  LAUNCH_CHECK();
  return 0;
}

static int enqueue_eval(pdlpdev_ctx* ctx, int which, int rc_rule_finite_bounds, double eps_rel_primal,
                        double eps_rel_dual, double* sc)
{
  hipStream_t s = ctx->stream;
  const int n = ctx->n, m = ctx->m;
  const double* altx = which == PDLPDEV_LAST_RESTART ? ctx->lrx : ctx->avgx;
  const double* alty = which == PDLPDEV_LAST_RESTART ? ctx->lry : ctx->avgy;
  const int kw       = which == PDLPDEV_CURRENT ? PDLPDEV_CURRENT : PDLPDEV_AVERAGE;
  const bool want_linf = eps_rel_primal >= 0.0 && eps_rel_dual >= 0.0;
  double* linf_m = want_linf ? ctx->tmp_m : nullptr;
  double* linf_n = want_linf ? ctx->tmp_n : nullptr;
  if (kw == PDLPDEV_AVERAGE) dense_part(ctx, 0, altx, nullptr, 0, 0);
  else dense_part(ctx, 0, ctx->x[0], ctx->x[1], 2, 0);
  if (ctx->pba.on) {
    if (kw == PDLPDEV_AVERAGE) TRY(pb_products(ctx, ctx->pba, altx, nullptr, 0, 0));
    else TRY(pb_products(ctx, ctx->pba, ctx->x[0], ctx->x[1], 2, 0));
    TRY(pb_rows(ctx, k_pb_eval_primal, ctx->pba, ctx->ctl, kw, ctx->y[0], ctx->y[1], alty, ctx->dr, ctx->lo_u, ctx->hi_u, eps_rel_primal, linf_m, ctx->ax_u[which], ctx->part_a));
  } else if (ctx->ja.on)
    (void)JAG_LAUNCH(ctx, k_jag_eval_primal, ctx->ja.v, ctx->ctl, kw, ctx->x[0], ctx->x[1], altx, ctx->y[0], ctx->y[1], alty, ctx->dr, ctx->lo_u, ctx->hi_u, eps_rel_primal, linf_m, ctx->ax_u[which], ctx->part_a);
  else if (ctx->pa.on)
    (ctx->pa.v.seg ? k_panel_eval_primal<true> : k_panel_eval_primal<false>)<<<ctx->pa.v.W, kPanelThreads, 0, s>>>(ctx->pa.v, ctx->ctl, kw, ctx->x[0], ctx->x[1], altx, ctx->y[0], ctx->y[1], alty, ctx->dr, ctx->lo_u, ctx->hi_u, eps_rel_primal, linf_m, ctx->ax_u[which], ctx->part_a);
  else
    k_eval_primal<<<stream_grid(ctx->a_nb), kBlock, 0, s>>>(ctx->a_nb, ctx->a_rb, ctx->ha_off, ctx->ha_idx, ctx->ha_val, ctx->ctl, kw, ctx->x[0], ctx->x[1], altx, ctx->y[0], ctx->y[1], alty, ctx->dr, ctx->lo_u, ctx->hi_u, eps_rel_primal, linf_m, ctx->ax_u[which], ctx->part_a, ctx->dense.add_m);
  k_finalize<<<1, kBlock, 0, s>>>(ctx->part_a, dual_partials(ctx), 3, 0u, sc + 0);
  if (want_linf) {
    const int g = std::min(grid_for(m), kGenericBlocks);
    k_max_partials<<<g, kBlock, 0, s>>>(m, ctx->tmp_m, ctx->part_g);
    k_finalize<<<1, kBlock, 0, s>>>(ctx->part_g, g, 1, 1u, sc + 3);
  }
  EvalDualCore core{nullptr, ctx->dc, ctx->c_u, ctx->lb_u, ctx->ub_u, eps_rel_dual, rc_rule_finite_bounds, which == PDLPDEV_LAST_RESTART ? ctx->rc_scratch : ctx->rc[which == PDLPDEV_AVERAGE ? 1 : 0], linf_n, ctx->aty_u[which]};
  if (!ctx->comm) {
    if (kw == PDLPDEV_AVERAGE) dense_part(ctx, 1, alty, nullptr, 0, 0);
    else dense_part(ctx, 1, ctx->y[0], ctx->y[1], 2, 0);
    if (ctx->pbat.on) {
      if (kw == PDLPDEV_AVERAGE) TRY(pb_products(ctx, ctx->pbat, alty, nullptr, 0, 0));
      else TRY(pb_products(ctx, ctx->pbat, ctx->y[0], ctx->y[1], 2, 0));
      TRY(pb_rows(ctx, k_pb_eval_dual, ctx->pbat, ctx->ctl, kw, ctx->x[0], ctx->x[1], altx, core, ctx->part_at));
    } else if (ctx->jat.on)
      (void)JAG_LAUNCH(ctx, k_jag_eval_dual, ctx->jat.v, ctx->ctl, kw, ctx->x[0], ctx->x[1], altx, ctx->y[0], ctx->y[1], alty, core, ctx->part_at);
    else if (ctx->pat.on)
      (ctx->pat.v.seg ? k_panel_eval_dual<true> : k_panel_eval_dual<false>)<<<ctx->pat.v.W, kPanelThreads, 0, s>>>(ctx->pat.v, ctx->ctl, kw, ctx->x[0], ctx->x[1], altx, ctx->y[0], ctx->y[1], alty, core, ctx->part_at);
    else
      k_eval_dual<<<stream_grid(ctx->at_nb), kBlock, 0, s>>>(ctx->at_nb, ctx->at_rb, ctx->hat_off, ctx->hat_idx, ctx->hat_val, ctx->ctl, kw, ctx->x[0], ctx->x[1], altx, ctx->y[0], ctx->y[1], alty, core, ctx->part_at, ctx->dense.add_n);
    k_finalize<<<1, kBlock, 0, s>>>(ctx->part_at, step_partials(ctx), 4, 0u, sc + 4);
  } else {
    if (kw == PDLPDEV_AVERAGE) {
      launch_plain(ctx, 1, alty, ctx->ar_buf);
    } else {
      launch_at_cur(ctx, ctx->ar_buf, 0);
    }
    HIP_TRY(hipMemcpyAsync(ctx->ar_buf + n, sc, 3 * sizeof(double), hipMemcpyDeviceToDevice, s));
    TRY(allreduce(ctx, ctx->ar_buf, (size_t)n + 3, rccl::kSum));
    HIP_TRY(hipMemcpyAsync(sc, ctx->ar_buf + n, 3 * sizeof(double), hipMemcpyDeviceToDevice, s));
    if (want_linf) TRY(allreduce(ctx, sc + 3, 1, rccl::kMax));
    const int g = std::min(grid_for(n), kGenericBlocks);
    k_eval_dual_elementwise<<<g, kBlock, 0, s>>>(n, g, ctx->ctl, kw, ctx->x[0], ctx->x[1], altx, ctx->ar_buf, core, ctx->part_g);
    k_finalize<<<1, kBlock, 0, s>>>(ctx->part_g, g, 4, 0u, sc + 4);
  }
  if (want_linf) {
    const int g = std::min(grid_for(n), kGenericBlocks);
    k_max_partials<<<g, kBlock, 0, s>>>(n, ctx->tmp_n, ctx->part_g);
    k_finalize<<<1, kBlock, 0, s>>>(ctx->part_g, g, 1, 1u, sc + 8);
  }
  LAUNCH_CHECK();
  return 0;
}
int pdlpdev_eval(pdlpdev_ctx* ctx, int which, int rc_rule_finite_bounds, double eps_rel_primal,
                 double eps_rel_dual, double out[PDLPDEV_EV_COUNT])
{
  HIP_TRY(hipSetDevice(ctx->device));
  TRY(enqueue_eval(ctx, which, rc_rule_finite_bounds, eps_rel_primal, eps_rel_dual, ctx->scal));
  TRY(fetch_scalars(ctx, 9));
  read_eval(ctx->scal_h, eps_rel_primal >= 0.0 && eps_rel_dual >= 0.0, out);
  return 0;
}

int pdlpdev_major_eval(pdlpdev_ctx* ctx, int average_mode, int rc_rule_finite_bounds, double eps_rel_primal,
                       double eps_rel_dual, double out_current[PDLPDEV_EV_COUNT], double out_average[PDLPDEV_EV_COUNT])
{
  roctx::Range range("pdlp: major iteration evaluation (averages + convergence information)");
  HIP_TRY(hipSetDevice(ctx->device));
  const bool want_linf = eps_rel_primal >= 0.0 && eps_rel_dual >= 0.0;
  if (ctx->small_resident && !ctx->comm) {
    TRY(resident_major_eval(ctx, average_mode, rc_rule_finite_bounds, want_linf ? 1 : 0, eps_rel_primal, eps_rel_dual));
  } else {
    TRY(pdlpdev_flush_average(ctx));
    TRY(pdlpdev_make_average(ctx, average_mode));
    TRY(enqueue_eval(ctx, PDLPDEV_CURRENT, rc_rule_finite_bounds, eps_rel_primal, eps_rel_dual, ctx->scal));
    TRY(enqueue_eval(ctx, PDLPDEV_AVERAGE, rc_rule_finite_bounds, eps_rel_primal, eps_rel_dual, ctx->scal + 32));
    TRY(fetch_scalars(ctx, 41));
  }
  read_eval(ctx->scal_h, want_linf, out_current);
  read_eval(ctx->scal_h + 32, want_linf, out_average);
  return 0;
}

int pdlpdev_eval_infeasibility(pdlpdev_ctx* ctx, int which, int rc_rule_finite_bounds, double out[4])
{
  HIP_TRY(hipSetDevice(ctx->device));
  hipStream_t s = ctx->stream;
  const int n = ctx->n, m = ctx->m;
  const int gr = std::min(grid_for(m), kGenericBlocks), gc = std::min(grid_for(n), kGenericBlocks);
  double* part_rows = ctx->part_g;
  double* part_cols = ctx->part_g + 3 * 2048;
  k_infeas_rows<<<gr, kBlock, 0, s>>>(m, gr, ctx->ctl, which, ctx->ax_u[which], ctx->y[0], ctx->y[1], ctx->avgy, ctx->dr, ctx->lo_u, ctx->hi_u, part_rows);
  k_finalize<<<1, kBlock, 0, s>>>(part_rows, gr, 3, 0x3u, ctx->scal + 16);
  if (ctx->comm) {
    LAUNCH_CHECK();
    TRY(allreduce(ctx, ctx->scal + 16, 2, rccl::kMax));
    TRY(allreduce(ctx, ctx->scal + 18, 1, rccl::kSum));
  }
  k_infeas_cols<<<gc, kBlock, 0, s>>>(n, gc, ctx->ctl, which, ctx->aty_u[which], ctx->x[0], ctx->x[1], ctx->avgx, ctx->dc, ctx->c_u, ctx->lb_u, ctx->ub_u, rc_rule_finite_bounds, part_cols);
  k_finalize<<<1, kBlock, 0, s>>>(part_cols, gc, 6, 0xFu, ctx->scal + 24);
  LAUNCH_CHECK();
  HIP_TRY(hipMemcpyAsync(ctx->scal_h + 16, ctx->scal + 16, 16 * sizeof(double), hipMemcpyDeviceToHost, s));
  HIP_TRY(hipStreamSynchronize(s));
  const double* r = ctx->scal_h + 16;
  const double* c = ctx->scal_h + 24;
  double max_primal = r[0], primal_obj = c[2] == 0.0 ? 0.0 : c[5] * (1.0 / c[2]);
  double max_dual = c[0], dual_obj = r[2] + c[4];
  const double scaling = std::max(r[1], c[1]);
  if (scaling != 0.0) {
    max_dual /= scaling;
    dual_obj /= scaling;
  } else {
    max_dual = 0.0, dual_obj = 0.0;
  }
  if (c[2] > 0.0) {
    max_primal = std::max(max_primal, c[3]) / c[2];
  } else {
    max_primal = 0.0, primal_obj = 0.0;
  }
  out[0] = max_primal, out[1] = primal_obj, out[2] = max_dual, out[3] = dual_obj;
  return 0;
}

int pdlpdev_trust_region_bounds(pdlpdev_ctx* ctx, int which, double wp, double wd, double pds, double dds,
                                double primal_weight, double radius, int scaled_iterates, double out[6])
{
  HIP_TRY(hipSetDevice(ctx->device));
  TRY(fetch_ctl(ctx, nullptr));
  const int cur = ctx->ctl_h->cur;
  hipStream_t s = ctx->stream;
  const double* px = which == PDLPDEV_CURRENT ? ctx->x[cur] : (which == PDLPDEV_AVERAGE ? ctx->avgx : ctx->lrx);
  const double* py = which == PDLPDEV_CURRENT ? ctx->y[cur] : (which == PDLPDEV_AVERAGE ? ctx->avgy : ctx->lry);
  if (scaled_iterates) {
    const int nxt = 1 - cur, n = ctx->n, m = ctx->m;
// ... 18 lines not shown
  const int g = std::min(grid_for((int64_t)ctx->n + ctx->m), kGenericBlocks);
  k_tr_stats<<<g, kBlock, 0, s>>>(P, g, ctx->part_g);
  k_finalize<<<1, kBlock, 0, s>>>(ctx->part_g, g, 8, 0x80u, ctx->scal + 32);
  LAUNCH_CHECK();
  if (ctx->comm) {
    TRY(allreduce(ctx, ctx->scal + 32, 7, rccl::kSum));
    TRY(allreduce(ctx, ctx->scal + 39, 1, rccl::kMax));
  }
  HIP_TRY(hipMemcpyAsync(ctx->scal_h + 32, ctx->scal + 32, 8 * sizeof(double), hipMemcpyDeviceToHost, s));
  HIP_TRY(hipStreamSynchronize(s));
  const double* st = ctx->scal_h + 32;
  const double pd2 = st[0], dd2 = st[1];
  const double own = sqrt(pd2 * pds * primal_weight + dd2 * (dds / primal_weight));
  const double T   = radius >= 0.0 ? radius : own;
  const double lagrangian = (st[2] - st[3]) + st[4];
  double t = 0.0;
  if (!(T == 0.0 || sqrt(st[5]) == 0.0)) {
    t = st[6] > 0.0 ? T / sqrt(st[6]) : 0.0;
    for (int it = 0; it < 200; ++it) {
      k_tr_pass<<<g, kBlock, 0, s>>>(P, t, g, ctx->part_g);
      k_finalize<<<1, kBlock, 0, s>>>(ctx->part_g, g, 2, 0u, ctx->scal + 40);
      LAUNCH_CHECK();
      if (ctx->comm) TRY(allreduce(ctx, ctx->scal + 40, 2, rccl::kSum));
      HIP_TRY(hipMemcpyAsync(ctx->scal_h + 40, ctx->scal + 40, 2 * sizeof(double), hipMemcpyDeviceToHost, s));
      HIP_TRY(hipStreamSynchronize(s));
      const double low = ctx->scal_h[40], high = ctx->scal_h[41];
      if (high <= 0.0) {
        t = st[7];
        break;
      }
      const double rem = T * T - low;
      const double tn  = rem > 0.0 ? sqrt(rem / high) : t;
      if (!(tn > t)) break;
      t = tn;
    }
  }
  k_tr_final<<<g, kBlock, 0, s>>>(P, t, g, ctx->part_g);
  k_finalize<<<1, kBlock, 0, s>>>(ctx->part_g, g, 2, 0u, ctx->scal + 40);
  LAUNCH_CHECK();
  if (ctx->comm) TRY(allreduce(ctx, ctx->scal + 40, 2, rccl::kSum));
  HIP_TRY(hipMemcpyAsync(ctx->scal_h + 40, ctx->scal + 40, 2 * sizeof(double), hipMemcpyDeviceToHost, s));
  HIP_TRY(hipStreamSynchronize(s));
  out[0] = pd2, out[1] = dd2, out[2] = own, out[3] = lagrangian;
  out[4] = lagrangian + ctx->scal_h[40];
  out[5] = lagrangian + ctx->scal_h[41];
  return 0;
}

int pdlpdev_restart(pdlpdev_ctx* ctx, int which, int unscaled_distances, double dist2[2])
{
  HIP_TRY(hipSetDevice(ctx->device));
  hipStream_t s = ctx->stream;
  const int g = std::min(grid_for(std::max(ctx->n, ctx->m)), kGenericBlocks);
  k_restart<<<g, kBlock, 0, s>>>(ctx->n, ctx->m, which, unscaled_distances, ctx->dc, ctx->dr, ctx->ctl, ctx->x[0], ctx->x[1], ctx->y[0], ctx->y[1], ctx->avgx, ctx->avgy, ctx->lrx, ctx->lry, ctx->sumx, ctx->sumy, ctx->part_g);
  k_finalize<<<1, kBlock, 0, s>>>(ctx->part_g, g, 2, 0u, ctx->scal);
  k_restart_ctl<<<1, 1, 0, s>>>(ctx->ctl);
  LAUNCH_CHECK();
  TRY(allreduce(ctx, ctx->scal + 1, 1, rccl::kSum));
  TRY(fetch_scalars(ctx, 2));
  dist2[0] = ctx->scal_h[0], dist2[1] = ctx->scal_h[1];
  return 0;
}

int pdlpdev_save_best(pdlpdev_ctx* ctx, int which)
{
  HIP_TRY(hipSetDevice(ctx->device));
  if (!ctx->bestx) {
    TRY(dev_alloc(ctx, &ctx->bestx, ctx->n));
    TRY(dev_alloc(ctx, &ctx->besty, ctx->m));
    TRY(dev_alloc(ctx, &ctx->bestrc, ctx->n));
  }
  TRY(fetch_ctl(ctx, nullptr));
  const int cur = ctx->ctl_h->cur;
  hipStream_t s = ctx->stream;
  const bool avg = which == PDLPDEV_AVERAGE;
  HIP_TRY(hipMemcpyAsync(ctx->bestx, avg ? ctx->avgx : ctx->x[cur], (size_t)ctx->n * sizeof(double), hipMemcpyDeviceToDevice, s));
  HIP_TRY(hipMemcpyAsync(ctx->besty, avg ? ctx->avgy : ctx->y[cur], (size_t)ctx->m * sizeof(double), hipMemcpyDeviceToDevice, s));
  HIP_TRY(hipMemcpyAsync(ctx->bestrc, ctx->rc[avg ? 1 : 0], (size_t)ctx->n * sizeof(double), hipMemcpyDeviceToDevice, s));
  return 0;
}

}
```

### cuopt_amd/csrc/pdlp_kernel_decls.hpp

```cpp
#pragma once
#include "pdlp_epilogues.hpp"

__global__ void __launch_bounds__(kBlock)
k_spmv_a_dual(int nb, const int32_t* __restrict__ rb, const int32_t* __restrict__ off,
              const int32_t* __restrict__ idx, const double* __restrict__ val,
              const pdlpdev_ctl* __restrict__ ctl, const double* __restrict__ xbar,
              double* __restrict__ y0, double* __restrict__ y1, const double* __restrict__ lo,
              const double* __restrict__ hi, double* __restrict__ sumy, double* __restrict__ part, double* __restrict__ ycopy,
              const p2pdev::Push* __restrict__ push, const double* __restrict__ dadd);
__global__ void __launch_bounds__(kBlock)
k_spmv_at_step(int nb, const int32_t* __restrict__ rb, const int32_t* __restrict__ off,
               const int32_t* __restrict__ idx, const double* __restrict__ val,
               const pdlpdev_ctl* __restrict__ ctl, const double* __restrict__ y0,
               const double* __restrict__ y1, const double* __restrict__ x0,
               const double* __restrict__ x1, double* __restrict__ aty0, double* __restrict__ aty1,
               double* __restrict__ part, const double* __restrict__ dadd);
__global__ void __launch_bounds__(kBlock)
k_spmv_plain(int nb, const int32_t* __restrict__ rb, const int32_t* __restrict__ off,
             const int32_t* __restrict__ idx, const double* __restrict__ val,
             const double* __restrict__ vec, double* __restrict__ out, const double* __restrict__ dadd);
__global__ void __launch_bounds__(kBlock)
k_spmv_at_cur(int nb, const int32_t* __restrict__ rb, const int32_t* __restrict__ off,
              const int32_t* __restrict__ idx, const double* __restrict__ val,
              const pdlpdev_ctl* __restrict__ ctl, const double* __restrict__ y0,
// ... 49 lines not shown
               const double* __restrict__ y1, double* __restrict__ aty0, double* __restrict__ aty1,
               double* __restrict__ out_override, int use_next);
extern template __global__ void k_panel_at_cur<true>(PanelView P, const pdlpdev_ctl* __restrict__ ctl, const double* __restrict__ y0,
               const double* __restrict__ y1, double* __restrict__ aty0, double* __restrict__ aty1,
               double* __restrict__ out_override, int use_next);
extern template __global__ void k_panel_at_cur<false>(PanelView P, const pdlpdev_ctl* __restrict__ ctl, const double* __restrict__ y0,
               const double* __restrict__ y1, double* __restrict__ aty0, double* __restrict__ aty1,
               double* __restrict__ out_override, int use_next);
template <bool SEG>
__global__ void __launch_bounds__(kPanelThreads)
k_panel_plain(PanelView P, const double* __restrict__ vec, double* __restrict__ out);
extern template __global__ void k_panel_plain<true>(PanelView P, const double* __restrict__ vec, double* __restrict__ out);
extern template __global__ void k_panel_plain<false>(PanelView P, const double* __restrict__ vec, double* __restrict__ out);
template <bool SEG>
__global__ void __launch_bounds__(kPanelThreads)
k_panel_eval_primal(PanelView P, const pdlpdev_ctl* __restrict__ ctl, int which,
                    const double* __restrict__ x0, const double* __restrict__ x1,
                    const double* __restrict__ avgx, const double* __restrict__ y0,
                    const double* __restrict__ y1, const double* __restrict__ avgy,
                    const double* __restrict__ dr, const double* __restrict__ lo_u,
                    const double* __restrict__ hi_u, double eps_rel, double* __restrict__ linf_rows,
                    double* __restrict__ ax_out, double* __restrict__ part);
extern template __global__ void k_panel_eval_primal<true>(PanelView P, const pdlpdev_ctl* __restrict__ ctl, int which,
                    const double* __restrict__ x0, const double* __restrict__ x1,
                    const double* __restrict__ avgx, const double* __restrict__ y0,
                    const double* __restrict__ y1, const double* __restrict__ avgy,
                    const double* __restrict__ dr, const double* __restrict__ lo_u,
                    const double* __restrict__ hi_u, double eps_rel, double* __restrict__ linf_rows,
                    double* __restrict__ ax_out, double* __restrict__ part);
extern template __global__ void k_panel_eval_primal<false>(PanelView P, const pdlpdev_ctl* __restrict__ ctl, int which,
                    const double* __restrict__ x0, const double* __restrict__ x1,
                    const double* __restrict__ avgx, const double* __restrict__ y0,
                    const double* __restrict__ y1, const double* __restrict__ avgy,
                    const double* __restrict__ dr, const double* __restrict__ lo_u,
                    const double* __restrict__ hi_u, double eps_rel, double* __restrict__ linf_rows,
                    double* __restrict__ ax_out, double* __restrict__ part);
template <bool SEG>
__global__ void __launch_bounds__(kPanelThreads)
k_panel_eval_dual(PanelView P, const pdlpdev_ctl* __restrict__ ctl, int which,
                  const double* __restrict__ x0, const double* __restrict__ x1,
                  const double* __restrict__ avgx, const double* __restrict__ y0,
                  const double* __restrict__ y1, const double* __restrict__ avgy, EvalDualCore core,
                  double* __restrict__ part);
extern template __global__ void k_panel_eval_dual<true>(PanelView P, const pdlpdev_ctl* __restrict__ ctl, int which,
                  const double* __restrict__ x0, const double* __restrict__ x1,
                  const double* __restrict__ avgx, const double* __restrict__ y0,
                  const double* __restrict__ y1, const double* __restrict__ avgy, EvalDualCore core,
                  double* __restrict__ part);
extern template __global__ void k_panel_eval_dual<false>(PanelView P, const pdlpdev_ctl* __restrict__ ctl, int which,
                  const double* __restrict__ x0, const double* __restrict__ x1,
                  const double* __restrict__ avgx, const double* __restrict__ y0,
                  const double* __restrict__ y1, const double* __restrict__ avgy, EvalDualCore core,
                  double* __restrict__ part);
template <int WAVES>
__global__ void __launch_bounds__(WAVES * 64)
k_jag_a_dual(JagView J, const pdlpdev_ctl* __restrict__ ctl, const double* __restrict__ xbar,
             double* __restrict__ y0, double* __restrict__ y1, const double* __restrict__ lo,
             const double* __restrict__ hi, double* __restrict__ sumy, double* __restrict__ part, double* __restrict__ ycopy,
             const p2pdev::Push* __restrict__ push);
extern template __global__ void k_jag_a_dual<8>(JagView J, const pdlpdev_ctl* __restrict__ ctl, const double* __restrict__ xbar,
             double* __restrict__ y0, double* __restrict__ y1, const double* __restrict__ lo,
             const double* __restrict__ hi, double* __restrict__ sumy, double* __restrict__ part, double* __restrict__ ycopy,
             const p2pdev::Push* __restrict__ push);
extern template __global__ void k_jag_a_dual<16>(JagView J, const pdlpdev_ctl* __restrict__ ctl, const double* __restrict__ xbar,
             double* __restrict__ y0, double* __restrict__ y1, const double* __restrict__ lo,
             const double* __restrict__ hi, double* __restrict__ sumy, double* __restrict__ part, double* __restrict__ ycopy,
             const p2pdev::Push* __restrict__ push);
template <int WAVES>
__global__ void __launch_bounds__(WAVES * 64)
k_jag_at_step(JagView J, const pdlpdev_ctl* __restrict__ ctl, const double* __restrict__ y0,
              const double* __restrict__ y1, const double* __restrict__ x0,
              const double* __restrict__ x1, double* __restrict__ aty0, double* __restrict__ aty1,
              double* __restrict__ part);
extern template __global__ void k_jag_at_step<8>(JagView J, const pdlpdev_ctl* __restrict__ ctl, const double* __restrict__ y0,
              const double* __restrict__ y1, const double* __restrict__ x0,
              const double* __restrict__ x1, double* __restrict__ aty0, double* __restrict__ aty1,
              double* __restrict__ part);
extern template __global__ void k_jag_at_step<16>(JagView J, const pdlpdev_ctl* __restrict__ ctl, const double* __restrict__ y0,
              const double* __restrict__ y1, const double* __restrict__ x0,
              const double* __restrict__ x1, double* __restrict__ aty0, double* __restrict__ aty1,
              double* __restrict__ part);
template <int WAVES>
__global__ void __launch_bounds__(WAVES * 64)
k_jag_at_cur(JagView J, const pdlpdev_ctl* __restrict__ ctl, const double* __restrict__ y0,
             const double* __restrict__ y1, double* __restrict__ aty0, double* __restrict__ aty1,
             double* __restrict__ out_override, int use_next);
extern template __global__ void k_jag_at_cur<8>(JagView J, const pdlpdev_ctl* __restrict__ ctl, const double* __restrict__ y0,
             const double* __restrict__ y1, double* __restrict__ aty0, double* __restrict__ aty1,
             double* __restrict__ out_override, int use_next);
extern template __global__ void k_jag_at_cur<16>(JagView J, const pdlpdev_ctl* __restrict__ ctl, const double* __restrict__ y0,
             const double* __restrict__ y1, double* __restrict__ aty0, double* __restrict__ aty1,
             double* __restrict__ out_override, int use_next);
template <int WAVES>
__global__ void __launch_bounds__(WAVES * 64)
k_jag_plain(JagView J, const double* __restrict__ vec, double* __restrict__ out);
extern template __global__ void k_jag_plain<8>(JagView J, const double* __restrict__ vec, double* __restrict__ out);
extern template __global__ void k_jag_plain<16>(JagView J, const double* __restrict__ vec, double* __restrict__ out);
template <int WAVES>
__global__ void __launch_bounds__(WAVES * 64)
k_jag_eval_primal(JagView J, const pdlpdev_ctl* __restrict__ ctl, int which,
                  const double* __restrict__ x0, const double* __restrict__ x1,
                  const double* __restrict__ avgx, const double* __restrict__ y0,
                  const double* __restrict__ y1, const double* __restrict__ avgy,
                  const double* __restrict__ dr, const double* __restrict__ lo_u,
                  const double* __restrict__ hi_u, double eps_rel, double* __restrict__ linf_rows,
                  double* __restrict__ ax_out, double* __restrict__ part);
// ... 98 lines not shown
```

### cuopt_amd/csrc/pdlp_kernels.hpp

```cpp
#pragma once
#include <hip/hip_runtime.h>
#include <stdint.h>


#include "cuopt_amd/pdlp_device.h"

namespace pdlp {

typedef double vec4d __attribute__((ext_vector_type(4)));
typedef int vec4i __attribute__((ext_vector_type(4)));

constexpr int kBlock    = 256;
constexpr int kNnzTile  = 2048;
constexpr int kNnzBlock = kNnzTile - 4;
constexpr int kLongRow  = 128;
constexpr int kMaxRowsPerBlock = 1024;

template <int XOR_MASK>
__device__ __forceinline__ double swizzle_xor(double v)
{
  static_assert(XOR_MASK >= 1 && XOR_MASK <= 16, "ds_swizzle works inside 32 lanes");
  constexpr int pattern = (XOR_MASK << 10) | 0x1F;
  int lo = __double2loint(v), hi = __double2hiint(v);
  lo = __builtin_amdgcn_ds_swizzle(lo, pattern);
// ... 42 lines not shown
  }
}

template <int CTRL>
__device__ __forceinline__ double dpp_move(double v)
{
  int lo = __double2loint(v), hi = __double2hiint(v);
  lo = __builtin_amdgcn_update_dpp(0, lo, CTRL, 0xf, 0xf, false);
  hi = __builtin_amdgcn_update_dpp(0, hi, CTRL, 0xf, 0xf, false);
  return __hiloint2double(hi, lo);
}
__device__ __forceinline__ double row16_sum(double v)
{
  v = v + dpp_move<0xB1>(v);
  v = v + dpp_move<0x4E>(v);
  v = v + dpp_move<0x141>(v);
  v = v + dpp_move<0x140>(v);
  return v;
}
__device__ __forceinline__ double read_lane(double v, int lane)
{
  const int lo = __builtin_amdgcn_readlane(__double2loint(v), lane);
  const int hi = __builtin_amdgcn_readlane(__double2hiint(v), lane);
  return __hiloint2double(hi, lo);
}
__device__ __forceinline__ double wave_sum_dpp(double v)
{
  v = row16_sum(v);
  return ((read_lane(v, 0) + read_lane(v, 16)) + read_lane(v, 32)) + read_lane(v, 48);
}
template <int NQ, int WAVES>
__device__ __forceinline__ void block_sum_fast(double (&v)[NQ], double* scratch )
{
  static_assert(NQ <= 4 && WAVES <= 16, "one DPP row per quantity");
  const int lane = threadIdx.x & 63, wave = threadIdx.x >> 6;
#pragma unroll
  for (int q = 0; q < NQ; ++q) {
    const double w = wave_sum_dpp(v[q]);
    if (lane == 0) scratch[q * 16 + wave] = w;
  }
  __syncthreads();
  const int q = lane >> 4, i = lane & 15;
  double part = (q < NQ && i < WAVES) ? scratch[q * 16 + i] : 0.0;
  part        = row16_sum(part);
#pragma unroll
  for (int k = 0; k < NQ; ++k) v[k] = read_lane(part, 16 * k);
}

__device__ __forceinline__ double dense_plus(const double* __restrict__ add, int r, double v) { return add ? v + add[r] : v; }

__device__ __forceinline__ bool loop_active(const pdlpdev_ctl* ctl)
{
  return ctl->error == 0 && ctl->steps_taken < ctl->target_steps;
}

__device__ __forceinline__ int xcd_remap(int b, int nb)
{
  const int per = (nb + 7) >> 3;
  const int v   = (b & 7) * per + (b >> 3);
  return v;
}



constexpr int kPanelThreads = 512;
constexpr int kPanelChunk   = 4096;
constexpr int kPanelMaxRows = 3584;
constexpr int kPanelWaves   = kPanelThreads / 64;

struct PanelView {
  int W, S;
  int any_long;
  const int32_t* __restrict__ row0;
  const int32_t* __restrict__ tile_ptr;
  const uint16_t* __restrict__ rowptr;
  const int64_t* __restrict__ rp_base;
  const int32_t* __restrict__ col;
  const double* __restrict__ val;
  const double* __restrict__ dense_add = nullptr;
  int seg = 0, slab_w = 0;
  int NP = 0;
  const int32_t* __restrict__ own_row = nullptr;
  const int32_t* __restrict__ own_ptr = nullptr;
  const int32_t* __restrict__ csr_off = nullptr;
  const int32_t* __restrict__ csr_idx = nullptr;
  const double* __restrict__ csr_val  = nullptr;
  const int32_t* __restrict__ dn_own_seg   = nullptr;
  const int32_t* __restrict__ dn_pan_ptr   = nullptr;
  const int32_t* __restrict__ dn_pan_seg   = nullptr;
  const int32_t* __restrict__ dn_seg_row   = nullptr;
  const int32_t* __restrict__ dn_seg_c0    = nullptr;
  const int32_t* __restrict__ dn_seg_len   = nullptr;
  const int32_t* __restrict__ dn_seg_ptr   = nullptr;
  const double* __restrict__ dn_val        = nullptr;
};
constexpr int kPanelOwnRow = 4096;
constexpr int kPanelDenseSegs = 32;
constexpr long long kPanelNotMine = 0x7FF8C0DEC0DEC0DELL;

constexpr int kPanelPer     = kPanelChunk / kPanelThreads;
constexpr int kPanelRowsPer = (kPanelMaxRows + kPanelThreads - 1) / kPanelThreads;
constexpr int kSegColBits = 20;
constexpr unsigned kSegColMask = (1u << kSegColBits) - 1u;

constexpr int kJagMaxGroup = 256;
constexpr int kJagBatchRows = 16384;
// ... 196 lines not shown
```

### cuopt_amd/csrc/pdlp_solver.cpp

```cpp
#include <algorithm>
#include <chrono>
#include <cmath>
#include <cstdarg>
#include <cstdio>
#include <cstdlib>
#include <condition_variable>
#include <cstring>
#include <functional>
#include <limits>
#include <mutex>
#include <memory>
#include <string>
#include <thread>
#include <vector>

#include "cuopt_amd/pdlp_solver.h"
#include "host_parallel.hpp"

namespace {

thread_local std::string g_error;
int fail(int code, const char* fmt, ...)
{
  char buf[1024];
// ... 1 lines not shown
  va_start(ap, fmt);
  vsnprintf(buf, sizeof(buf), fmt, ap);
  va_end(ap);
  g_error = buf;
  return code;
}
#define DEV(expr)                                                          \
  do {                                                                     \
    int rc_ = (expr);                                                      \
    if (rc_ != 0) return fail(rc_, "%s: %s", #expr, pdlpdev_last_error()); \
  } while (0)

using clock_type = std::chrono::steady_clock;
double seconds_since(clock_type::time_point t0)
{
  return std::chrono::duration<double>(clock_type::now() - t0).count();
}

enum : int {
  kNoTermination  = 0,
  kOptimal        = 1,
  kPrimalInfeasible = 2,
  kDualInfeasible   = 3,
  kIterationLimit = 4,
  kTimeLimit      = 5,
  kNumericalError = 6,
  kPrimalFeasible = 7,
};

struct Convergence {
  double primal_objective = 0, dual_objective = 0, gap = 0, abs_objective = 0;
  double l2_primal_residual = 0, l2_dual_residual = 0, l2_x = 0, l2_y = 0;
  double linf_rel_primal_residual = 0, linf_rel_dual_residual = 0;
  double infeasibility[4] = {0, 0, 0, 0};
};

}

struct cuoptamd_solver {
  pdlpdev_ctx* dev = nullptr;
  pdlpdev_analysis* spent_analysis = nullptr;
  cuoptamd_hyper H{};
  cuoptamd_settings S{};
  int32_t m_global = 0, n = 0, row_begin = 0, row_end = 0;
  int rank = 0, world = 1;
  bool empty_problem = false;
  double objective_scale = 1.0, objective_offset = 0.0;
  double norm_b = 0.0, norm_c = 0.0;
  double computed_step = 0.0, computed_weight = 0.0;
  int32_t total_iterations = 0;
  int32_t iteration_offset = 0;
  int32_t attempt_offset   = 0;
  int32_t major_done_at    = -1;
  bool step_error = false, need_aty = true, last_restart_was_average = false;
  double last_candidate_kkt = 0.0, last_restart_kkt = 0.0;
  double gap_reduction_ratio_last_trial = 1.0;
  struct Quality {
    bool feasible = false;
    double residual = std::numeric_limits<double>::infinity();
    double objective = 0.0;
    bool operator==(const Quality& o) const { return feasible == o.feasible && residual == o.residual && objective == o.objective; }
  } best_quality;
  bool have_best = false, maximize = false;
  cuoptamd_result best_result{};
  bool have_accepted = false;
  cuoptamd_result accepted_result{};
  std::string log_path;
  pdlpdev_ctl ctl{};
  Convergence conv_current, conv_average;
  int returned_which = PDLPDEV_CURRENT;
  bool finished = false, warm_started = false;
  cuoptamd_result result{};
  clock_type::time_point solve_start;
  bool started = false;
  std::vector<int32_t> row_new2old, col_new2old;
  int reorder_method = 0;
  int32_t analysis_info[10] = {0};
  const double* cols_in(const double* v, std::vector<double>& tmp) const { return to_device_order(col_new2old, v, tmp); }
  const double* rows_in(const double* v, std::vector<double>& tmp) const { return to_device_order(row_new2old, v, tmp); }
  static const double* to_device_order(const std::vector<int32_t>& new2old, const double* v, std::vector<double>& tmp)
  {
    if (!v || new2old.empty()) return v;
    tmp.resize(new2old.size());
    for (size_t i = 0; i < new2old.size(); ++i) tmp[i] = v[new2old[i]];
    return tmp.data();
  }
  static void to_caller_order(const std::vector<int32_t>& new2old, const double* dev, double* user, size_t first, size_t last)
  {
    for (size_t i = first; i < last; ++i) user[new2old[i]] = dev[i];
  }
};

namespace {

void preset_stable2(cuoptamd_hyper& h)
{
  h.initial_step_size_scaling                                  = 1.0;
  h.ruiz_iterations                                            = 10;
  h.do_pock_chambolle                                          = 1;
  h.do_ruiz                                                    = 1;
  h.alpha_pock_chambolle                                       = 1.0;
  h.artificial_restart_threshold                               = 0.36;
  h.compute_initial_step_size_before_scaling                   = 0;
  h.compute_initial_primal_weight_before_scaling               = 0;
  h.initial_primal_weight_c_scaling                            = 1.0;
  h.initial_primal_weight_b_scaling                            = 1.0;
// ... 107 lines not shown
  r.l2_relative_dual_residual   = c.l2_dual_residual / (1.0 + s->norm_c);
  r.step_size              = s->ctl.step_size;
  r.primal_weight          = s->ctl.primal_weight;
  r.max_primal_ray_infeasibility = c.infeasibility[0];
  r.primal_ray_linear_objective  = c.infeasibility[1];
  r.max_dual_ray_infeasibility   = c.infeasibility[2];
  r.dual_ray_linear_objective    = c.infeasibility[3];
  s->returned_which        = which;
}


void log_line(const cuoptamd_solver* s, const char* fmt, ...)
{
  if (!s->S.log_to_console && s->log_path.empty()) return;
  char buf[512];
  va_list ap;
  va_start(ap, fmt);
  vsnprintf(buf, sizeof(buf), fmt, ap);
  va_end(ap);
  if (s->S.log_to_console) {
    std::fputs(buf, stdout);
    std::fflush(stdout);
  }
  if (!s->log_path.empty()) {
    if (FILE* f = std::fopen(s->log_path.c_str(), "a")) {
      std::fputs(buf, f);
      std::fclose(f);
    }
  }
}
void log_iteration(const cuoptamd_solver* s, const Convergence& c)
{
  log_line(s, "%7d %+.8e %+.8e  %8.2e   %8.2e     %8.2e   %.3fs\n", s->total_iterations, c.primal_objective,
           c.dual_objective, c.gap, c.l2_primal_residual, c.l2_dual_residual, seconds_since(s->solve_start));
}

const cuoptamd_solver::Quality& best_of(const cuoptamd_solver* s, const cuoptamd_solver::Quality& a,
                                        const cuoptamd_solver::Quality& b)
{
  if (a.feasible && !b.feasible) return a;
  if (!a.feasible && b.feasible) return b;
  if (a.feasible && b.feasible) {
    const bool a_lower = a.objective < b.objective;
    return ((!s->maximize && a_lower) || (s->maximize && !a_lower)) ? a : b;
  }
  return a.residual < b.residual ? a : b;
}

struct HostRange {
  explicit HostRange(const char* name) { pdlpdev_range_push(name); }
  ~HostRange() { pdlpdev_range_pop(); }
};

pdlpdev_small_eval major_eval_request(const cuoptamd_solver* s)
{
  int mode = 2;
  if (s->total_iterations - s->iteration_offset <= 1 && !s->warm_started)
    mode = 0;
  else if (s->ctl.its_since_restart == 0)
    mode = 1;
  pdlpdev_small_eval r;
  r.mode        = mode;
  r.rule_finite = s->H.handle_some_primal_gradients_on_finite_bounds_as_residuals == 0;
  r.eps_p = s->S.per_constraint_residual ? s->S.relative_primal_tolerance : -1.0;
  r.eps_d = s->S.per_constraint_residual ? s->S.relative_dual_tolerance : -1.0;
  return r;
}
struct MajorPlan {
  bool restart = false;
  int which = PDLPDEV_CURRENT, unscaled = 0;
  bool really_average = false;
  double candidate = 0.0;
};
int major_head(cuoptamd_solver* s, const double* ev, const double* ev_avg, bool* terminated, MajorPlan* plan);
double major_restart_done(cuoptamd_solver* s, const MajorPlan& plan, const double dist2[2]);

int major_iteration(cuoptamd_solver* s, bool* terminated)
{
  HostRange range("pdlp: major iteration (termination + restart logic)");
  pdlpdev_ctx* dev = s->dev;
  const pdlpdev_small_eval rq = major_eval_request(s);
  double ev[PDLPDEV_EV_COUNT], ev_avg[PDLPDEV_EV_COUNT];
  DEV(pdlpdev_major_eval(dev, rq.mode, rq.rule_finite, rq.eps_p, rq.eps_d, ev, ev_avg));
  MajorPlan plan;
  int rc = major_head(s, ev, ev_avg, terminated, &plan);
  if (rc != 0 || *terminated || !plan.restart) return rc;
  double dist2[2];
  DEV(pdlpdev_restart(dev, plan.which, plan.unscaled, dist2));
  const double nw = major_restart_done(s, plan, dist2);
  if (nw > 0.0) DEV(pdlpdev_set_step(dev, -1.0, nw));
  return 0;
}

double major_restart_done(cuoptamd_solver* s, const MajorPlan& plan, const double dist2[2])
{
  const double w = s->ctl.primal_weight;
  double nw      = -1.0;
  s->last_restart_was_average = plan.really_average;
  if (plan.really_average) s->need_aty = true;
  s->ctl.its_since_restart = 0;
  s->ctl.sum_weights       = 0.0;
  const double pd = std::sqrt(dist2[0]), dd = std::sqrt(dist2[1]);
  const double guard = 1.0e-10;
  if (!(pd < guard || pd >= 1.0 / guard || dd < guard || dd >= 1.0 / guard)) {
    const double theta = s->H.primal_weight_update_smoothing;
    nw                 = std::exp(theta * std::log(dd / pd) + (1.0 - theta) * std::log(w));
    s->ctl.primal_weight = nw;
  }
  s->last_restart_kkt = plan.candidate;
  return nw;
}

int major_head(cuoptamd_solver* s, const double* ev, const double* ev_avg, bool* terminated, MajorPlan* plan)
{
  const cuoptamd_hyper& H = s->H;
  pdlpdev_ctx* dev        = s->dev;
  *terminated             = false;
  *plan                   = MajorPlan();
  s->result.num_major_iterations += 1;
  const int rule_finite = H.handle_some_primal_gradients_on_finite_bounds_as_residuals == 0;
  s->conv_current = to_convergence(s, ev);
  s->conv_average = to_convergence(s, ev_avg);
  if (s->S.detect_infeasibility) {
    DEV(pdlpdev_eval_infeasibility(dev, PDLPDEV_CURRENT, rule_finite, s->conv_current.infeasibility));
    DEV(pdlpdev_eval_infeasibility(dev, PDLPDEV_AVERAGE, rule_finite, s->conv_average.infeasibility));
  }
  const int t_cur = verdict(s, s->conv_current), t_avg = verdict(s, s->conv_average);
  const double w  = s->ctl.primal_weight;

  bool done = false;
  int status = kNumericalError, which = PDLPDEV_CURRENT;
  if (s->total_iterations > 1) {
    if (s->S.first_primal_feasible) {
      if (t_avg == kPrimalFeasible && t_cur == kPrimalFeasible) {
        done = true, status = kPrimalFeasible;
        which = s->conv_current.l2_primal_residual < s->conv_average.l2_primal_residual ? PDLPDEV_CURRENT : PDLPDEV_AVERAGE;
// ... 626 lines not shown
    return 0;
  };
  if (hyper->compute_initial_step_size_before_scaling) { int rc = initial_step_size(); if (rc) return rc; }
  if (hyper->compute_initial_primal_weight_before_scaling) { int rc = initial_primal_weight(); if (rc) return rc; }
  lap("norms + params");
  DEV(pdlpdev_scaling_compute(s->dev, hyper->do_ruiz, hyper->ruiz_iterations, hyper->do_pock_chambolle, hyper->alpha_pock_chambolle));
  lap("scaling_compute");
  DEV(pdlpdev_scale_problem(s->dev));
  lap("scale_problem");
  if (comm_id && pdlpdev_shard_dataflow(s->dev) == 3) {
    int32_t cb = 0, nc = 0;
    DEV(pdlpdev_owner_slice(s->dev, &cb, &nc));
    std::vector<int32_t> coff((size_t)nc + 1, 0);
    const int64_t nnz_g = L->offsets[m];
    for (int64_t k = 0; k < nnz_g; ++k) {
      const int32_t j = L->indices[k] - cb;
      if (j >= 0 && j < nc) ++coff[j + 1];
    }
    for (int32_t j = 0; j < nc; ++j) coff[j + 1] += coff[j];
    std::vector<int32_t> cidx((size_t)std::max<int32_t>(coff[nc], 1)), cur(coff.begin(), coff.end() - 1);
    std::vector<double> cval((size_t)std::max<int32_t>(coff[nc], 1));
    for (int32_t i = 0; i < m; ++i)
      for (int32_t k = L->offsets[i]; k < L->offsets[i + 1]; ++k) {
        const int32_t j = L->indices[k] - cb;
        if (j >= 0 && j < nc) {
          const int32_t p = cur[j]++;
          cidx[p] = i, cval[p] = L->values[k];
        }
      }
    DEV(pdlpdev_owner_setup(s->dev, coff.data(), cidx.data(), cval.data(), bounds.data()));
    lap("owner-computes column block");
  }
  if (!hyper->compute_initial_step_size_before_scaling) { int rc = initial_step_size(); if (rc) return rc; }
  if (!hyper->compute_initial_primal_weight_before_scaling) { int rc = initial_primal_weight(); if (rc) return rc; }
  s->computed_step = step, s->computed_weight = weight;
  { int rc = start_run(s, init_x, init_y); if (rc) return rc; }
  lap("initial step/weight/iterate");
  s->result.setup_seconds = seconds_since(t0);
  return 0;
}

void cuoptamd_solver_destroy(cuoptamd_solver* s)
{
  if (!s) return;
  if (s->dev) pdlpdev_destroy(s->dev);
  if (s->spent_analysis) pdlpdev_analysis_destroy(s->spent_analysis);
  delete s;
}

static void reset_host_state(cuoptamd_solver* s)
{
  const cuoptamd_result blank{};
  s->total_iterations = 0, s->iteration_offset = 0, s->attempt_offset = 0, s->major_done_at = -1;
  s->step_error = false, s->need_aty = true, s->last_restart_was_average = false;
  s->last_candidate_kkt = 0.0, s->last_restart_kkt = 0.0, s->gap_reduction_ratio_last_trial = 1.0;
  s->best_quality = cuoptamd_solver::Quality{};
  s->best_quality.objective = s->maximize ? -std::numeric_limits<double>::infinity() : std::numeric_limits<double>::infinity();
  s->have_best = false, s->best_result = blank;
  s->have_accepted = false, s->accepted_result = blank;
  s->conv_current = Convergence{}, s->conv_average = Convergence{};
  s->returned_which = PDLPDEV_CURRENT, s->finished = false, s->warm_started = false, s->started = false;
  s->result = blank;
}

int cuoptamd_solver_reset(cuoptamd_solver* s, const double* lb, const double* ub, const double* lo, const double* hi,
                          const cuoptamd_settings* settings, const double* init_x, const double* init_y)
{
  if (!s) return fail(-1, "cuoptamd_solver_reset: null solver");
  const auto t0 = clock_type::now();
  if (settings) {
    s->S = *settings;
    if (settings->log_file && settings->log_file[0]) s->log_path = settings->log_file;
    s->S.log_file = nullptr;
  }
  reset_host_state(s);
  if (s->empty_problem) return 0;
  {
    std::vector<double> tlb, tub, tlo, thi;
    lb = s->cols_in(lb, tlb), ub = s->cols_in(ub, tub), lo = s->rows_in(lo, tlo), hi = s->rows_in(hi, thi);
    DEV(pdlpdev_reset(s->dev, lb, ub, lo ? lo + s->row_begin : nullptr, hi ? hi + s->row_begin : nullptr));
  }
  const bool timing = std::getenv("CUOPT_AMD_TIMING") != nullptr;
  const double t_reset = seconds_since(t0);
  DEV(pdlpdev_problem_norms(s->dev, &s->norm_c, &s->norm_b));
  if (lo || hi) {
    double nr[2];
    DEV(pdlpdev_weight_norms(s->dev, s->H.compute_initial_primal_weight_before_scaling, nr));
    const double cn = std::sqrt(s->H.initial_primal_weight_c_scaling * nr[0]);
    const double bn = std::sqrt(s->H.initial_primal_weight_b_scaling * nr[1]);
    s->computed_weight = (bn > 0.0 && cn > 0.0) ? s->H.primal_importance * (cn / bn) : s->H.primal_importance;
  }
  DEV(pdlpdev_set_graph_mode(s->dev, s->S.use_graph));
  const double t_norms = seconds_since(t0);
  { int rc = start_run(s, init_x, init_y); if (rc) return rc; }
  s->result.setup_seconds = seconds_since(t0);
  if (timing)
    fprintf(stderr, "[cuopt_amd setup] reset: bounds to the device %.2f ms, norms + weight %.2f ms, initial iterate / step %.2f ms\n", 1e3 * t_reset,
            1e3 * (t_norms - t_reset), 1e3 * (s->result.setup_seconds - t_norms));
  return 0;
}

static bool major_due(const cuoptamd_solver* s)
{
  const cuoptamd_hyper& H = s->H;
  const int32_t it = s->total_iterations;
  const bool major = (it % H.major_iteration == 0 && it > 0) || it <= H.min_iteration_restart;
// ... 48 lines not shown
  if (!next_target(s, budget_end, target_out)) {
    *stop = true;
    return 0;
  }
  if (s->step_error) {
    s->step_error = false;
    int rc = pdlpdev_clear_error(s->dev);
    if (rc != 0) return fail(rc, "pdlpdev_clear_error: %s", pdlpdev_last_error());
  }
  if (s->need_aty) {
    int rc = pdlpdev_compute_aty(s->dev);
    if (rc != 0) return fail(rc, "pdlpdev_compute_aty: %s", pdlpdev_last_error());
    s->need_aty = false;
  }
  return 0;
}
static void advance_after_attempts(cuoptamd_solver* s)
{
  s->total_iterations = s->iteration_offset + s->ctl.steps_taken;
  if (s->ctl.error) s->step_error = true;
}
static void advance_begin(cuoptamd_solver* s, clock_type::time_point t0)
{
  if (s->started) return;
  s->started     = true;
  s->solve_start = t0;
  log_line(s, "PDLP on gfx950: %d constraints, %d variables\n", s->m_global, s->n);
  log_line(s, "   Iter    Primal Obj.      Dual Obj.    Gap        Primal Res.  Dual Res.   Time\n");
}
static int32_t advance_budget_end(const cuoptamd_solver* s, int32_t max_new_iterations)
{
  const int64_t budget_end64 = (int64_t)s->total_iterations + std::max<int64_t>(max_new_iterations, 0);
  return (int32_t)std::min<int64_t>(budget_end64, std::numeric_limits<int32_t>::max());
}

int cuoptamd_solver_advance(cuoptamd_solver* s, int32_t max_new_iterations, cuoptamd_result* result)
{
  if (!s) return fail(-1, "cuoptamd_solver_advance: null solver");
  const auto t0 = clock_type::now();
  advance_begin(s, t0);
  auto leave = [&](int rc) {
    s->result.gpus = s->world;
    s->result.loop_seconds += seconds_since(t0);
    if (result) *result = s->result;
    return rc;
  };
  if (s->empty_problem) {
    s->result.status = kNumericalError;
    s->finished      = true;
    return leave(0);
  }
  if (s->finished) return leave(0);
  const int32_t budget_end = advance_budget_end(s, max_new_iterations);
  for (;;) {
    int32_t target = 0;
    bool stop      = false;
    int rc         = advance_to_attempts(s, budget_end, &target, &stop);
    if (rc != 0 || stop) return leave(rc);
    rc = pdlpdev_run(s->dev, target, &s->ctl);
    if (rc != 0) return leave(fail(rc, "pdlpdev_run: %s", pdlpdev_last_error()));
    advance_after_attempts(s);
  }
}

struct cuoptamd_batch {
  int K = 0;
  std::vector<cuoptamd_solver*> s;
  pdlpdev_batch* dev = nullptr;
  pdlpdev_small_batch* small = nullptr;
};

int cuoptamd_solver_clone(cuoptamd_solver* parent, const double* lb, const double* ub, const double* lo, const double* hi,
                          const cuoptamd_settings* settings, cuoptamd_solver** out)
{
  if (!parent || !out) return fail(-1, "cuoptamd_solver_clone: null argument");
  if (parent->empty_problem || !parent->dev || parent->world != 1) return fail(-7, "cuoptamd_solver_clone: not for empty or sharded solvers");
  const bool timing = std::getenv("CUOPT_AMD_TIMING") != nullptr;
  const auto t0     = clock_type::now();
  pdlpdev_ctx* dev = nullptr;
  int rc           = pdlpdev_clone_shared(&dev, parent->dev);
  if (rc != 0) {
    if (dev) pdlpdev_destroy(dev);
    return fail(rc, "pdlpdev_clone_shared: %s", pdlpdev_last_error());
  }
  const double t_dev = seconds_since(t0);
  cuoptamd_solver* s = new cuoptamd_solver(*parent);
  s->spent_analysis = nullptr;
  s->dev             = dev;
  rc = cuoptamd_solver_reset(s, lb, ub, lo, hi, settings, nullptr, nullptr);
  if (timing) fprintf(stderr, "[cuopt_amd setup] clone: device context %.2f ms, reset to its bounds %.2f ms\n", 1e3 * t_dev, 1e3 * (seconds_since(t0) - t_dev));
  if (rc != 0) {
    cuoptamd_solver_destroy(s);
    return rc;
  }
  *out = s;
  return 0;
}

int cuoptamd_batch_create(cuoptamd_solver** solvers, int K, cuoptamd_batch** out)
{
  if (!solvers || !out || K < 1) return fail(-1, "cuoptamd_batch_create: null argument");
  std::vector<pdlpdev_ctx*> ctx(K);
  for (int l = 0; l < K; ++l) {
    if (!solvers[l] || !solvers[l]->dev) return fail(-1, "cuoptamd_batch_create: null solver");
    ctx[l] = solvers[l]->dev;
  }
  pdlpdev_small_batch* small = nullptr;
  int rc                     = pdlpdev_small_batch_create(&small, ctx.data(), K);
  pdlpdev_batch* dev         = nullptr;
  if (rc == -7) {
    if (K > 16) return fail(-7, "cuoptamd_batch_create: more than 16 LPs need the resident small-LP path (%s)", pdlpdev_last_error());
    rc = pdlpdev_batch_create(&dev, ctx.data(), K);
  }
// ... 698 lines not shown
```

### include/cuopt_amd/pdlp_device.h

```cpp
#ifndef CUOPT_AMD_PDLP_DEVICE_H
#define CUOPT_AMD_PDLP_DEVICE_H

#include <stdint.h>

#ifdef __cplusplus
extern "C" {
#endif

typedef struct pdlpdev_ctx pdlpdev_ctx;

typedef struct pdlpdev_ctl {
  double step_size;
  double primal_weight;
  double tau;
  double sigma;
  double sum_weights;
  double last_interaction, last_movement, last_dx2, last_dy2;
  int32_t k;
  int32_t cur;
  int32_t pending_avg;
  int32_t steps_taken;
  int32_t attempts;
  int32_t target_steps;
  int32_t error;
  int32_t its_since_restart;
} pdlpdev_ctl;

typedef struct pdlpdev_step_params {
  double reduction_exponent;
  double growth_exponent;
  double primal_distance_smoothing;
  double dual_distance_smoothing;
} pdlpdev_step_params;

enum {
  PDLPDEV_EV_CX = 0,
  PDLPDEV_EV_DUAL_SUM,
  PDLPDEV_EV_PRES2,
  PDLPDEV_EV_DRES2,
  PDLPDEV_EV_X2,
  PDLPDEV_EV_Y2,
  PDLPDEV_EV_LINF_PRES_REL,
  PDLPDEV_EV_LINF_DRES_REL,
  PDLPDEV_EV_COUNT
};

enum {
  PDLPDEV_CURRENT = 0,
  PDLPDEV_AVERAGE = 1,
  PDLPDEV_LAST_RESTART = 2,
  PDLPDEV_BEST = 3
};

enum {
  PDLPDEV_BUF_X = 0,
  PDLPDEV_BUF_Y,
  PDLPDEV_BUF_X_OTHER,
  PDLPDEV_BUF_Y_OTHER,
  PDLPDEV_BUF_ATY,
  PDLPDEV_BUF_ATY_OTHER,
  PDLPDEV_BUF_XBAR,
  PDLPDEV_BUF_SUM_X,
  PDLPDEV_BUF_SUM_Y,
  PDLPDEV_BUF_AVG_X,
  PDLPDEV_BUF_AVG_Y,
  PDLPDEV_BUF_DROW,
  PDLPDEV_BUF_DCOL,
  PDLPDEV_BUF_A_VALUES,
  PDLPDEV_BUF_AT_VALUES,
  PDLPDEV_BUF_C,
  PDLPDEV_BUF_LB, PDLPDEV_BUF_UB,
  PDLPDEV_BUF_LO, PDLPDEV_BUF_HI,
  PDLPDEV_BUF_RC_CURRENT,
  PDLPDEV_BUF_RC_AVERAGE,
  PDLPDEV_BUF_LAST_RESTART_X, PDLPDEV_BUF_LAST_RESTART_Y,
  PDLPDEV_BUF_COUNT
};

enum {
  PDLPDEV_K_PRIMAL = 0,
  PDLPDEV_K_SPMV_A_DUAL,
  PDLPDEV_K_SPMV_AT_STEP,
  PDLPDEV_K_STEP_DECISION,
  PDLPDEV_K_SPMV_A_PLAIN,
  PDLPDEV_K_SPMV_AT_PLAIN,
  PDLPDEV_K_ITERATION,
  PDLPDEV_K_COUNT
};

const char* pdlpdev_last_error(void);
int pdlpdev_device_count(void);
int pdlpdev_device_info(int dev, char* name, int len, int* compute_units, int64_t* hbm_bytes);

int pdlpdev_create(pdlpdev_ctx** out, int device, int32_t m, int32_t n, const int32_t* a_offsets,
                   const int32_t* a_indices, const double* a_values, const int32_t* at_offsets,
                   const int32_t* at_indices, const double* at_values, const double* c,
                   const double* lo, const double* hi, const double* lb, const double* ub);
void pdlpdev_create_hint(int sharded);
void pdlpdev_create_batch_lanes(int lanes);
void pdlpdev_create_share_stream(pdlpdev_ctx* donor);
int pdlpdev_resident_size(int32_t m, int32_t n, int64_t nnz);
int pdlpdev_create_overlapped(pdlpdev_ctx** out, int device, int32_t m, int32_t n, const int32_t* a_offsets,
                              const int32_t* a_indices, const double* a_values, const int32_t* at_offsets,
                              const int32_t* at_indices, const double* at_values,
                              void (*transpose_ready)(void*), void* user, const double* c, const double* lo,
                              const double* hi, const double* lb, const double* ub);
void pdlpdev_destroy(pdlpdev_ctx* ctx);

typedef struct pdlpdev_analysis pdlpdev_analysis;
int pdlpdev_analyze(pdlpdev_analysis** out, int device, int32_t m, int32_t n, const int32_t* a_offsets, const int32_t* a_indices,
                    const double* a_values, int flags);
int pdlpdev_analyze_with_vectors(pdlpdev_analysis** out, int device, int32_t m, int32_t n, const int32_t* a_offsets, const int32_t* a_indices,
                                 const double* a_values, int flags, const double* c, const double* lo, const double* hi, const double* lb,
                                 const double* ub);
int pdlpdev_analysis_info(pdlpdev_analysis* an, int32_t out[10]);
int pdlpdev_analysis_maps(pdlpdev_analysis* an, int32_t* row_new2old, int32_t* col_new2old);
int pdlpdev_analysis_vectors_in_order(pdlpdev_analysis* an);
void pdlpdev_analysis_release_workspace(pdlpdev_analysis* an);
int pdlpdev_analysis_download(pdlpdev_analysis* an, int which, int32_t* offsets, int32_t* indices, double* values);
int pdlpdev_create_from_analysis(pdlpdev_ctx** out, pdlpdev_analysis* an, const double* c, const double* lo, const double* hi,
                                 const double* lb, const double* ub);
void pdlpdev_analysis_destroy(pdlpdev_analysis* an);
int pdlpdev_debug_sort_pairs(int device, int64_t n, const uint32_t* keys, const uint32_t* vals, int bits, uint32_t* keys_out,
                             uint32_t* vals_out);
int pdlpdev_debug_scan(int device, int64_t n, const int32_t* in, int32_t* out);
int pdlpdev_debug_ipc_export(int device, int count, uint8_t handle[64], void** base);
int pdlpdev_debug_ipc_store(int device, const uint8_t handle[64], int count, double seed);
int pdlpdev_debug_ipc_wait(int device, void* base, int count, double seed);
// ... 14 lines not shown
int pdlpdev_scale_problem(pdlpdev_ctx* ctx);
int pdlpdev_init_norms(pdlpdev_ctx* ctx, double out[3]);
int pdlpdev_agree_max(pdlpdev_ctx* ctx, double* value);
int pdlpdev_weight_norms(pdlpdev_ctx* ctx, int unscaled, double out[2]);
int pdlpdev_reset(pdlpdev_ctx* ctx, const double* lb, const double* ub, const double* lo, const double* hi);
int pdlpdev_problem_norms(pdlpdev_ctx* ctx, double* norm_c, double* norm_b);
int pdlpdev_set_step_params(pdlpdev_ctx* ctx, const pdlpdev_step_params* p);
int pdlpdev_set_step(pdlpdev_ctx* ctx, double step_size, double primal_weight);
int pdlpdev_set_k(pdlpdev_ctx* ctx, int32_t k);
int pdlpdev_set_initial(pdlpdev_ctx* ctx, const double* x, const double* y);
int pdlpdev_project_primal(pdlpdev_ctx* ctx);
int pdlpdev_initial_solution_stats(pdlpdev_ctx* ctx, double out[5], const double* x0_unscaled, const double* y0_unscaled);

int pdlpdev_compute_aty(pdlpdev_ctx* ctx);
int pdlpdev_run(pdlpdev_ctx* ctx, int32_t target_steps, pdlpdev_ctl* ctl);
int pdlpdev_get_ctl(pdlpdev_ctx* ctx, pdlpdev_ctl* ctl);
typedef struct pdlpdev_batch pdlpdev_batch;
int pdlpdev_clone_shared(pdlpdev_ctx** out, pdlpdev_ctx* parent);
int pdlpdev_batch_create(pdlpdev_batch** out, pdlpdev_ctx** ctx, int K);
int pdlpdev_batch_run(pdlpdev_batch* batch, const int32_t* targets, pdlpdev_ctl* ctl);
void pdlpdev_batch_destroy(pdlpdev_batch* batch);
int pdlpdev_batch_time_kernels(pdlpdev_batch* batch, int reps, double avg_ms[4]);
typedef struct pdlpdev_small_batch pdlpdev_small_batch;
typedef struct pdlpdev_small_eval {
  int32_t mode;
  int32_t rule_finite;
  double eps_p, eps_d;
} pdlpdev_small_eval;
int pdlpdev_small_batch_create(pdlpdev_small_batch** out, pdlpdev_ctx** ctx, int K);
void pdlpdev_small_batch_destroy(pdlpdev_small_batch* batch);
int pdlpdev_small_batch_run(pdlpdev_small_batch* batch, const int32_t* targets, pdlpdev_ctl* ctl, const pdlpdev_small_eval* eval_after,
                            double* out_current, double* out_average, int32_t* evaluated);
int pdlpdev_small_batch_major_eval(pdlpdev_small_batch* batch, const pdlpdev_small_eval* req, double* out_current, double* out_average);
int pdlpdev_small_batch_restart(pdlpdev_small_batch* batch, const int32_t* which, const int32_t* unscaled_distances, double* dist2);
int pdlpdev_small_batch_prepare(pdlpdev_small_batch* batch, const int32_t* clear_error, const double* primal_weight, const int32_t* compute_aty);
int pdlpdev_small_batch_reset(pdlpdev_small_batch* batch, const int32_t* take, const double* const* lb, const double* const* ub, const double* const* x0,
                              const double* const* y0, const double* step, const double* weight, const int32_t* k, int project, pdlpdev_ctl* ctl,
                              const int32_t* var, const double* var_lb, const double* var_ub, const int32_t* warm);
int pdlpdev_small_batch_solution_views(pdlpdev_small_batch* batch, const int32_t* which, const double** x_view, const double** y_view, const double** rc_view);
int pdlpdev_small_batch_get_solutions(pdlpdev_small_batch* batch, const int32_t* which, double* const* x, double* const* y, double* const* rc);
int pdlpdev_clear_error(pdlpdev_ctx* ctx);
int pdlpdev_set_graph_mode(pdlpdev_ctx* ctx, int use_graph);
int pdlpdev_prepare_graphs(pdlpdev_ctx* ctx);
int pdlpdev_copy_in(void* dst, const void* src, size_t bytes);
void pdlpdev_range_push(const char* name);
void pdlpdev_range_pop(void);

int pdlpdev_flush_average(pdlpdev_ctx* ctx);
int pdlpdev_make_average(pdlpdev_ctx* ctx, int mode);
int pdlpdev_eval(pdlpdev_ctx* ctx, int which, int rc_rule_finite_bounds, double eps_rel_primal,
                 double eps_rel_dual, double out[PDLPDEV_EV_COUNT]);
int pdlpdev_major_eval(pdlpdev_ctx* ctx, int average_mode, int rc_rule_finite_bounds, double eps_rel_primal,
                       double eps_rel_dual, double out_current[PDLPDEV_EV_COUNT], double out_average[PDLPDEV_EV_COUNT]);
int pdlpdev_eval_infeasibility(pdlpdev_ctx* ctx, int which, int rc_rule_finite_bounds, double out[4]);
int pdlpdev_restart(pdlpdev_ctx* ctx, int which, int unscaled_distances, double dist2[2]);
int pdlpdev_trust_region_bounds(pdlpdev_ctx* ctx, int which, double primal_norm_weight,
                                double dual_norm_weight, double primal_distance_smoothing,
                                double dual_distance_smoothing, double primal_weight, double radius,
                                int scaled_iterates, double out[6]);

int pdlpdev_save_best(pdlpdev_ctx* ctx, int which);

int pdlpdev_get_solution(pdlpdev_ctx* ctx, int which, double* x, double* y, double* rc);
int64_t pdlpdev_download(pdlpdev_ctx* ctx, int buffer_id, void* host, int64_t max_elements);

int64_t pdlpdev_upload(pdlpdev_ctx* ctx, int buffer_id, const void* host, int64_t elements);
int pdlpdev_set_loop_state(pdlpdev_ctx* ctx, double sum_weights, int32_t its_since_restart, int32_t k);

int pdlpdev_spmv(pdlpdev_ctx* ctx, int transpose, const double* x, double* y);
int pdlpdev_time_kernel(pdlpdev_ctx* ctx, int kernel_id, int reps, double* avg_ms);
int pdlpdev_synchronize(pdlpdev_ctx* ctx);
int64_t pdlpdev_device_bytes(pdlpdev_ctx* ctx);
int pdlpdev_shard_dataflow(pdlpdev_ctx* ctx);
int pdlpdev_dense_info(pdlpdev_ctx* ctx, int64_t out[3]);
int pdlpdev_shard_transport(pdlpdev_ctx* ctx);
int pdlpdev_shard_wire_bytes(pdlpdev_ctx* ctx, int64_t out[3]);
int pdlpdev_owner_slice(pdlpdev_ctx* ctx, int32_t* col_begin, int32_t* ncols);
int pdlpdev_owner_setup(pdlpdev_ctx* ctx, const int32_t* offsets, const int32_t* indices, const double* values,
                        const int32_t* row_bounds);
int pdlpdev_layout_info(pdlpdev_ctx* ctx, int32_t out[8]);

#ifdef __cplusplus
}
#endif
#endif
```

Before: 5997 iterations/s.

## Fuse major evaluation into the attempt run and reuse cached A^T y

Adds a period path that enqueues the major KKT evaluation behind the PDHG attempts, guarded on device by a target-reached check, so the host needs one sync per period instead of separate run and eval round trips. The evaluation can also reuse the already computed A^T y instead of redoing the transpose SpMV. Host-side control state is cached so set_target can skip a fetch. The risk is stale state if the validity flags are not invalidated on every mutation, plus wasted guarded launches when the period is not reached.

```diff
diff --git a/cuopt_amd/capi.py b/cuopt_amd/capi.py
--- a/cuopt_amd/capi.py
+++ b/cuopt_amd/capi.py
@@ -260,6 +260,10 @@
 _proto("pdlpdev_make_average", c_int, c_void_p, c_int)
 _proto("pdlpdev_eval", c_int, c_void_p, c_int, c_int, c_double, c_double, c_void_p)
 _proto("pdlpdev_restart", c_int, c_void_p, c_int, c_int, c_void_p)
+_proto("pdlpdev_major_eval", c_int, c_void_p, c_int, c_int, c_double, c_double, c_void_p, c_void_p)
+if hasattr(lib, "pdlpdev_loop_stats"):
+    _proto("pdlpdev_loop_stats", c_int, c_void_p, c_void_p)
+    _proto("pdlpdev_run_period", c_int, c_void_p, c_int, c_void_p, c_void_p, c_void_p, c_void_p, c_void_p)
 _proto("pdlpdev_save_best", c_int, c_void_p, c_int)
 _proto("pdlpdev_trust_region_bounds", c_int, c_void_p, c_int, c_double, c_double, c_double, c_double, c_double, c_double, c_int, c_void_p)
 _proto("pdlpdev_eval_infeasibility", c_int, c_void_p, c_int, c_int, c_void_p)
@@ -305,7 +309,7 @@
 BUF = {n: i for i, n in enumerate(
     ["X", "Y", "X_OTHER", "Y_OTHER", "ATY", "ATY_OTHER", "XBAR", "SUM_X", "SUM_Y", "AVG_X", "AVG_Y",
      "DROW", "DCOL", "A_VALUES", "AT_VALUES", "C", "LB", "UB", "LO", "HI", "RC_CURRENT", "RC_AVERAGE",
-     "LAST_RESTART_X", "LAST_RESTART_Y"])}
+     "LAST_RESTART_X", "LAST_RESTART_Y", "ATY_U_CURRENT", "ATY_U_AVERAGE"])}
 KERNEL = {n: i for i, n in enumerate(
     ["PRIMAL", "SPMV_A_DUAL", "SPMV_AT_STEP", "STEP_DECISION", "SPMV_A_PLAIN", "SPMV_AT_PLAIN"])}
 EV = {n: i for i, n in enumerate(
@@ -1011,6 +1015,16 @@
         self._ck(lib.pdlpdev_eval(self.handle, which, int(rule_finite), eps_p, eps_d, _ptr(out)))
         return {k: out[i] for k, i in EV.items()}
 
+    def major_eval(self, average_mode=2, rule_finite=True, eps_p=-1.0, eps_d=-1.0):
+        cur, avg = np.zeros(len(EV)), np.zeros(len(EV))
+        self._ck(lib.pdlpdev_major_eval(self.handle, int(average_mode), int(rule_finite), C.c_double(eps_p), C.c_double(eps_d), _ptr(cur), _ptr(avg)))
+        return cur, avg
+
+    def loop_stats(self):
+        out = np.zeros(4, dtype=np.int64)
+        self._ck(lib.pdlpdev_loop_stats(self.handle, out.ctypes.data_as(C.c_void_p)))
+        return dict(zip(["eval_reused_aty", "eval_product", "loop_syncs", "empty_attempts"], (int(v) for v in out)))
+
     def eval_infeasibility(self, which, rule_finite=True):
         out = np.zeros(4)
         self._ck(lib.pdlpdev_eval_infeasibility(self.handle, which, int(rule_finite), _ptr(out)))
diff --git a/cuopt_amd/csrc/kernels_batch.hip b/cuopt_amd/csrc/kernels_batch.hip
--- a/cuopt_amd/csrc/kernels_batch.hip
+++ b/cuopt_amd/csrc/kernels_batch.hip
@@ -853,6 +853,7 @@
   HIP_TRY(hipSetDevice(b->device));
   TRY(batch_refresh_table(b));
   const int K = b->K;
+  for (int l = 0; l < K; ++l) loop_state_touched(b->ctx[l]);
   for (int l = 0; l < K; ++l)
     if (targets[l] > 0) k_set_target<<<1, 1, 0, b->stream>>>(b->ctx[l]->ctl, targets[l]);
   LAUNCH_CHECK();
@@ -924,6 +925,7 @@
   hipEvent_t* ev = scratch.ev;
   for (int l = 0; l < K; ++l) {
     pdlpdev_ctx* c = b->ctx[l];
+    loop_state_touched(c);
     saved[l] = forced[l] = *c->ctl_h;
     forced[l].pending_avg = 1, forced[l].target_steps = saved[l].steps_taken + 1, forced[l].error = 0;
     HIP_TRY(hipMalloc((void**)&sx[l], std::max<size_t>(c->n, 1) * sizeof(double)));
diff --git a/cuopt_amd/csrc/kernels_panel.hip b/cuopt_amd/csrc/kernels_panel.hip
--- a/cuopt_amd/csrc/kernels_panel.hip
+++ b/cuopt_amd/csrc/kernels_panel.hip
@@ -62,6 +62,7 @@
                     const double* __restrict__ hi_u, double eps_rel, double* __restrict__ linf_rows,
                     double* __restrict__ ax_out, double* __restrict__ part)
 {
+  if (period_guard_skips(ctl, which)) return;
   const int cur = ctl->cur;
   const double* xv = which == PDLPDEV_AVERAGE ? avgx : (cur ? x1 : x0);
   const double* yv = which == PDLPDEV_AVERAGE ? avgy : (cur ? y1 : y0);
@@ -77,11 +78,54 @@
                   const double* __restrict__ y1, const double* __restrict__ avgy, EvalDualCore core,
                   double* __restrict__ part)
 {
+  if (period_guard_skips(ctl, which)) return;
   const int cur = ctl->cur;
   core.xhat     = which == PDLPDEV_AVERAGE ? avgx : (cur ? x1 : x0);
   const double* yv = which == PDLPDEV_AVERAGE ? avgy : (cur ? y1 : y0);
   EvalDualEpilogue e{core};
   panel_block<SEG>(P, yv, e, part);
+}
+
+__global__ void __launch_bounds__(kPanelThreads)
+k_panel_eval_dual_from_aty(PanelView P, const pdlpdev_ctl* __restrict__ ctl, const double* __restrict__ x0, const double* __restrict__ x1,
+                           const double* __restrict__ aty0, const double* __restrict__ aty1, EvalDualCore core,
+                           double* __restrict__ part, int guard)
+{
+  if (guard && !period_reached(ctl)) return;
+  __shared__ double red[kPanelWaves * EvalDualEpilogue::NQ];
+  __shared__ unsigned char own[kPanelMaxRows];
+  const int cur = ctl->cur;
+  core.xhat     = cur ? x1 : x0;
+  const double* __restrict__ src = cur ? aty1 : aty0;
+  EvalDualEpilogue e{core};
+  const int w  = blockIdx.x;
+  const int NP = P.NP ? P.NP : P.W;
+  double acc[EvalDualEpilogue::NQ];
+#pragma unroll
+  for (int q = 0; q < EvalDualEpilogue::NQ; ++q) acc[q] = SumOp::identity();
+  if (w >= NP) {
+    if (threadIdx.x == 0) {
+      const int r = P.own_row[w - NP];
+      e.row(r, src[r], acc);
+#pragma unroll
+      for (int q = 0; q < EvalDualEpilogue::NQ; ++q) part[(size_t)q * P.W + w] = acc[q];
+    }
+    return;
+  }
+  const int r0 = P.row0[w], nr = P.row0[w + 1] - r0;
+  if (P.own_ptr) {
+    for (int r = threadIdx.x; r < nr; r += kPanelThreads) own[r] = 0;
+    __syncthreads();
+    for (int q = P.own_ptr[w] + (int)threadIdx.x; q < P.own_ptr[w + 1]; q += kPanelThreads) own[P.own_row[q] - r0] = 1;
+    __syncthreads();
+  }
+  for (int r = threadIdx.x; r < nr; r += kPanelThreads)
+    if (!P.own_ptr || !own[r]) e.row(r0 + r, src[r0 + r], acc);
+  block_reduce<SumOp, EvalDualEpilogue::NQ, kPanelWaves>(acc, red);
+  if (threadIdx.x == 0) {
+#pragma unroll
+    for (int q = 0; q < EvalDualEpilogue::NQ; ++q) part[(size_t)q * P.W + w] = acc[q];
+  }
 }
 
 template __global__ void k_panel_a_dual<true>(PanelView P, const pdlpdev_ctl* __restrict__ ctl, const double* __restrict__ xbar,
diff --git a/cuopt_amd/csrc/pdlp_core_internal.hpp b/cuopt_amd/csrc/pdlp_core_internal.hpp
--- a/cuopt_amd/csrc/pdlp_core_internal.hpp
+++ b/cuopt_amd/csrc/pdlp_core_internal.hpp
@@ -9,6 +9,8 @@
 void launch_plain(pdlpdev_ctx* ctx, int transpose, const double* vec, double* out);
 void launch_at_cur(pdlpdev_ctx* ctx, double* out_override, int use_next);
 void dense_part(pdlpdev_ctx* ctx, int transpose, const double* v0, const double* v1, int mode, int in_loop);
+int enqueue_major_eval(pdlpdev_ctx* ctx, int average_mode, int rc_rule_finite_bounds, double eps_rel_primal, double eps_rel_dual, int guard);
+void read_major_eval(pdlpdev_ctx* ctx, double* out_current, double* out_average);
 }
 
 static inline int dual_partials(const pdlpdev_ctx* ctx) { return ctx->pba.on ? ctx->pba.v.B : ctx->ja.on ? ctx->ja.v.nblk + ctx->ja.v.nlong : ctx->pa.on ? ctx->pa.v.W : ctx->a_nb; }
@@ -16,7 +18,7 @@
 
 __global__ void __launch_bounds__(kBlock)
 k_flush_average(int n, int m, const pdlpdev_ctl* __restrict__ ctl, const double* __restrict__ x0, const double* __restrict__ x1, const double* __restrict__ y0,
-                const double* __restrict__ y1, double* __restrict__ sumx, double* __restrict__ sumy);
+                const double* __restrict__ y1, double* __restrict__ sumx, double* __restrict__ sumy, int guard);
 __global__ void __launch_bounds__(kBlock) k_finalize(const double* __restrict__ part, int nb, int nq, unsigned op_mask, double* __restrict__ out);
 __global__ void __launch_bounds__(kBlock) k_div_inplace(int n, double* __restrict__ v, const double* __restrict__ d);
 __global__ void __launch_bounds__(kBlock) k_div_to(int n, double* __restrict__ out, const double* __restrict__ v, const double* __restrict__ d);
diff --git a/cuopt_amd/csrc/pdlp_create.hip b/cuopt_amd/csrc/pdlp_create.hip
--- a/cuopt_amd/csrc/pdlp_create.hip
+++ b/cuopt_amd/csrc/pdlp_create.hip
@@ -521,6 +521,7 @@
   {
     const char* small_env = getenv("CUOPT_AMD_SMALL");
     const int tier        = resident_tier(m, n, ctx->nnz);
+    ctx->eval_reuse_aty   = cuopt_amd::tune_int("eval_reuse_aty", 1) != 0;
     ctx->small_resident   = tier >= 0 && !(small_env && atoi(small_env) == 0) && !ctx->dense.add_m && !ctx->dense.add_n;
     if (small_env && atoi(small_env) != 0 && tier < 0)
       return fail(-1, "CUOPT_AMD_SMALL=1: the LP does not fit the resident kernel (m, n <= 2048, nnz <= 4096 ...)");
diff --git a/cuopt_amd/csrc/pdlp_ctx.hpp b/cuopt_amd/csrc/pdlp_ctx.hpp
--- a/cuopt_amd/csrc/pdlp_ctx.hpp
+++ b/cuopt_amd/csrc/pdlp_ctx.hpp
@@ -403,6 +403,10 @@
   hipEvent_t prof_ev[2 * kProfPairs] = {};
   int prof_used = 0;
   int rejected_in_a_row = 0;
+  bool aty_valid = false, ctl_h_current = false;
+  int eval_reuse_aty = 1;
+  int spare_attempts = 0;
+  int64_t stat_eval_reused = 0, stat_eval_product = 0, stat_loop_syncs = 0, stat_empty_attempts = 0;
   int use_graph = 1;
   int batch_lanes = 0;
   bool comm_warm = false;
@@ -465,6 +469,9 @@
 
 constexpr int kGenericBlocks = 1024;
 constexpr int kScalars       = 64;
+constexpr int kCtlSlot       = 48;
+static_assert(kCtlSlot * sizeof(double) + sizeof(pdlpdev_ctl) <= kScalars * sizeof(double), "the control block fits behind the scalars");
+inline void loop_state_touched(pdlpdev_ctx* c) { c->aty_valid = false, c->ctl_h_current = false; }
 
 struct PerDeviceOnce {
   std::mutex m;
diff --git a/cuopt_amd/csrc/pdlp_device.hip b/cuopt_amd/csrc/pdlp_device.hip
--- a/cuopt_amd/csrc/pdlp_device.hip
+++ b/cuopt_amd/csrc/pdlp_device.hip
@@ -266,9 +266,9 @@
 __global__ void __launch_bounds__(kBlock)
 k_flush_average(int n, int m, const pdlpdev_ctl* __restrict__ ctl, const double* __restrict__ x0,
                 const double* __restrict__ x1, const double* __restrict__ y0,
-                const double* __restrict__ y1, double* __restrict__ sumx, double* __restrict__ sumy)
-{
-  if (ctl->pending_avg == 0) return;
+                const double* __restrict__ y1, double* __restrict__ sumx, double* __restrict__ sumy, int guard)
+{
+  if (ctl->pending_avg == 0 || (guard && !period_reached(ctl))) return;
   const int cur           = ctl->cur;
   const double w          = ctl->step_size;
   const double* __restrict__ x = cur ? x1 : x0;
@@ -500,6 +500,7 @@
 {
   HIP_TRY(hipMemcpyAsync(ctx->ctl_h, ctx->ctl, sizeof(pdlpdev_ctl), hipMemcpyDeviceToHost, ctx->stream));
   HIP_TRY(hipStreamSynchronize(ctx->stream));
+  ctx->ctl_h_current = true;
   if (out) *out = *ctx->ctl_h;
   return 0;
 }
@@ -549,6 +550,8 @@
   HIP_TRY(hipSetDevice(ctx->device));
   if (!ctx->scaled) return fail(-1, "pdlpdev_reset: the problem has not been scaled yet");
   ctx->rejected_in_a_row = 0;
+  ctx->spare_attempts    = 0;
+  loop_state_touched(ctx);
   hipStream_t s = ctx->stream;
   const size_t nb = (size_t)ctx->n * sizeof(double), mb = (size_t)ctx->m * sizeof(double);
   auto put = [&](const double* src, double* unscaled, double* scaled, size_t bytes) -> int {
@@ -630,6 +633,7 @@
 int pdlpdev_set_step(pdlpdev_ctx* ctx, double step_size, double primal_weight)
 {
   HIP_TRY(hipSetDevice(ctx->device));
+  ctx->ctl_h_current = false;
   k_set_step<<<1, 1, 0, ctx->stream>>>(ctx->ctl, step_size, primal_weight);
   LAUNCH_CHECK();
   return 0;
@@ -637,6 +641,7 @@
 int pdlpdev_set_k(pdlpdev_ctx* ctx, int32_t k)
 {
   HIP_TRY(hipSetDevice(ctx->device));
+  ctx->ctl_h_current = false;
   k_set_k<<<1, 1, 0, ctx->stream>>>(ctx->ctl, k);
   LAUNCH_CHECK();
   return 0;
@@ -645,6 +650,7 @@
 {
   HIP_TRY(hipSetDevice(ctx->device));
   TRY(fetch_ctl(ctx, nullptr));
+  ctx->aty_valid = false;
   const int cur = ctx->ctl_h->cur;
   if (x) {
     HIP_TRY(hipMemcpyAsync(ctx->x[cur], x, (size_t)ctx->n * sizeof(double), hipMemcpyHostToDevice, ctx->stream));
@@ -938,6 +944,101 @@
   return 0;
 }
 
+static int enqueue_attempts(pdlpdev_ctx* ctx, int remaining)
+{
+  const bool rccl_graphs = ctx->comm && !ctx->p2p.on && !ctx->soft && !ctx->graph_comm_failed;
+  bool replayed = false;
+  if (rccl_graphs && ctx->use_graph && !ctx->comm_warm) {
+    TRY(enqueue_attempt(ctx));
+    ctx->comm_warm = true;
+    remaining -= 1;
+  }
+  if (ctx->use_graph && (!ctx->comm || ctx->p2p.on || rccl_graphs)) {
+    replayed = true;
+    while (remaining > 0) {
+      int chunk = 1;
+      while (chunk * 2 <= remaining && chunk < 64) chunk *= 2;
+      hipGraphExec_t g;
+      const int grc = get_graph(ctx, chunk, &g);
+      if (grc != 0 && rccl_graphs) {
+        ctx->graph_comm_failed = true;
+        (void)hipGetLastError();
+        replayed = false;
+        break;
+      }
+      TRY(grc);
+      HIP_TRY(hipGraphLaunch(g, ctx->stream));
+      remaining -= chunk;
+    }
+  }
+  if (!replayed) {
+    for (int i = 0; i < remaining; ++i) TRY(enqueue_attempt(ctx));
+  }
+  return 0;
+}
+
+static int after_round(pdlpdev_ctx* ctx, int before, int attempts_before, int enqueued, int counted )
+{
+  const pdlpdev_ctl& c = *ctx->ctl_h;
+  const int made       = c.attempts - attempts_before;
+  if (!ctx->comm) ctx->stat_empty_attempts += enqueued - made;
+  if (c.steps_taken > before && c.error == 0 && !ctx->comm) ctx->aty_valid = true;
+  if (c.error != 0) ctx->aty_valid = false;
+  if (ctx->p2p.on && c.error != 0) {
+    int fault = 0;
+    HIP_TRY(hipMemcpy(&fault, ctx->p2p.fault, sizeof(int), hipMemcpyDeviceToHost));
+    if (fault) return fail(-6, "direct peer transport: rank %d waited 5 s for another rank's data (a peer failed or is stuck)", ctx->rank);
+  }
+  ctx->rejected_in_a_row = c.steps_taken == before ? ctx->rejected_in_a_row + counted : 0;
+  if (c.error == 0 && ctx->rejected_in_a_row >= 64) {
+    ctx->rejected_in_a_row = 0;
+    k_set_error<<<1, 1, 0, ctx->stream>>>(ctx->ctl);
+    LAUNCH_CHECK();
+    TRY(fetch_ctl(ctx, nullptr));
+    ctx->stat_loop_syncs += 1;
+    ctx->aty_valid = false;
+  }
+  return 0;
+}
+
+static int run_rounds(pdlpdev_ctx* ctx, int32_t target_steps, int* rounds)
+{
+  int guard = 0;
+  while (ctx->ctl_h->error == 0 && ctx->ctl_h->steps_taken < target_steps) {
+    const int before = ctx->ctl_h->steps_taken, attempts_before = ctx->ctl_h->attempts, asked = target_steps - before;
+    TRY(enqueue_attempts(ctx, asked));
+    TRY(fetch_ctl(ctx, nullptr));
+    ctx->stat_loop_syncs += 1;
+    TRY(after_round(ctx, before, attempts_before, asked, asked));
+    if (++guard > 100000) return fail(-6, "pdlpdev_run: no progress");
+  }
+  if (rounds) *rounds += guard;
+  return 0;
+}
+static int run_epilogue(pdlpdev_ctx* ctx, int rounds, pdlpdev_ctl* ctl)
+{
+  if (ctx->rsag && rounds > 0) {
+    const int cur = ctx->ctl_h->cur;
+    TRY(all_gather(ctx, ctx->x[cur], (size_t)ctx->slice));
+    TRY(all_gather(ctx, ctx->aty[cur], (size_t)ctx->slice));
+    TRY(all_gather(ctx, ctx->sumx, (size_t)ctx->slice));
+  }
+  if (ctl) *ctl = *ctx->ctl_h;
+  return 0;
+}
+static int set_target(pdlpdev_ctx* ctx, int32_t target_steps)
+{
+  k_set_target<<<1, 1, 0, ctx->stream>>>(ctx->ctl, target_steps);
+  LAUNCH_CHECK();
+  if (ctx->ctl_h_current && !ctx->comm) {
+    ctx->ctl_h->target_steps = target_steps;
+    return 0;
+  }
+  TRY(fetch_ctl(ctx, nullptr));
+  ctx->stat_loop_syncs += 1;
+  return 0;
+}
+
 int pdlpdev_run(pdlpdev_ctx* ctx, int32_t target_steps, pdlpdev_ctl* ctl)
 {
   roctx::Range range("pdlp: PDHG attempts");
@@ -947,63 +1048,56 @@
     if (ctl) *ctl = *ctx->ctl_h;
     return 0;
   }
-  k_set_target<<<1, 1, 0, ctx->stream>>>(ctx->ctl, target_steps);
-  LAUNCH_CHECK();
-  TRY(fetch_ctl(ctx, nullptr));
-  int guard = 0;
-  while (ctx->ctl_h->error == 0 && ctx->ctl_h->steps_taken < target_steps) {
-    int remaining = target_steps - ctx->ctl_h->steps_taken;
-    const bool rccl_graphs = ctx->comm && !ctx->p2p.on && !ctx->soft && !ctx->graph_comm_failed;
-    bool replayed = false;
-    if (rccl_graphs && ctx->use_graph && !ctx->comm_warm) {
-      TRY(enqueue_attempt(ctx));
-      ctx->comm_warm = true;
-      remaining -= 1;
-    }
-    if (ctx->use_graph && (!ctx->comm || ctx->p2p.on || rccl_graphs)) {
-      replayed = true;
-      while (remaining > 0) {
-        int chunk = 1;
-        while (chunk * 2 <= remaining && chunk < 64) chunk *= 2;
-        hipGraphExec_t g;
-        const int grc = get_graph(ctx, chunk, &g);
-        if (grc != 0 && rccl_graphs) {
-          ctx->graph_comm_failed = true;
-          (void)hipGetLastError();
-          replayed = false;
-          break;
-        }
-        TRY(grc);
-        HIP_TRY(hipGraphLaunch(g, ctx->stream));
-        remaining -= chunk;
-      }
-    }
-    if (!replayed) {
-      for (int i = 0; i < remaining; ++i) TRY(enqueue_attempt(ctx));
-    }
-    const int before = ctx->ctl_h->steps_taken, asked = target_steps - before;
-    TRY(fetch_ctl(ctx, nullptr));
-    if (ctx->p2p.on && ctx->ctl_h->error != 0) {
-      int fault = 0;
-      HIP_TRY(hipMemcpy(&fault, ctx->p2p.fault, sizeof(int), hipMemcpyDeviceToHost));
-      if (fault) return fail(-6, "direct peer transport: rank %d waited 5 s for another rank's data (a peer failed or is stuck)", ctx->rank);
-    }
-    ctx->rejected_in_a_row = ctx->ctl_h->steps_taken == before ? ctx->rejected_in_a_row + asked : 0;
-    if (ctx->ctl_h->error == 0 && ctx->rejected_in_a_row >= 64) {
-      ctx->rejected_in_a_row = 0;
-      k_set_error<<<1, 1, 0, ctx->stream>>>(ctx->ctl);
-      LAUNCH_CHECK();
+  TRY(set_target(ctx, target_steps));
+  int rounds = 0;
+  TRY(run_rounds(ctx, target_steps, &rounds));
+  return run_epilogue(ctx, rounds, ctl);
+}
+
+int pdlpdev_run_period(pdlpdev_ctx* ctx, int32_t target_steps, const pdlpdev_small_eval* rq, pdlpdev_ctl* ctl,
+                       double out_current[PDLPDEV_EV_COUNT], double out_average[PDLPDEV_EV_COUNT], int32_t* evaluated)
+{
+  *evaluated = 0;
+  HIP_TRY(hipSetDevice(ctx->device));
+  const bool dense_unfused = ctx->dense.on && !(ctx->pat.v.dn_pan_ptr != nullptr && ctx->pa.v.dn_own_seg != nullptr);
+  const bool eligible = !ctx->comm && !ctx->small_resident && ctx->pa.on && ctx->pat.on && !dense_unfused && ctx->ctl_h_current &&
+                        !(rq->eps_p >= 0.0 && rq->eps_d >= 0.0) && ctx->ctl_h->error == 0 && ctx->ctl_h->steps_taken < target_steps;
+  if (!eligible) return pdlpdev_run(ctx, target_steps, ctl);
+  roctx::Range range("pdlp: PDHG attempts + major iteration evaluation");
+  TRY(set_target(ctx, target_steps));
+  const int before = ctx->ctl_h->steps_taken, attempts_before = ctx->ctl_h->attempts, asked = target_steps - before;
+  const int spare = ctx->spare_attempts;
+  TRY(enqueue_attempts(ctx, asked));
+  if (spare > 0) TRY(enqueue_attempts(ctx, spare));
+  TRY(enqueue_major_eval(ctx, rq->mode, rq->rule_finite, rq->eps_p, rq->eps_d, 1));
+  HIP_TRY(hipMemcpyAsync(ctx->scal_h, ctx->scal, kCtlSlot * sizeof(double) + sizeof(pdlpdev_ctl), hipMemcpyDeviceToHost, ctx->stream));
+  HIP_TRY(hipStreamSynchronize(ctx->stream));
+  ctx->stat_loop_syncs += 1;
+  memcpy(ctx->ctl_h, ctx->scal_h + kCtlSlot, sizeof(pdlpdev_ctl));
+  ctx->ctl_h_current = true;
+  const int rejected  = (ctx->ctl_h->attempts - attempts_before) - (ctx->ctl_h->steps_taken - before);
+  ctx->spare_attempts = std::max(0, std::min(rejected, 4));
+  TRY(after_round(ctx, before, attempts_before, asked + spare, asked));
+  int rounds = 1;
+  if (ctx->ctl_h->error == 0 && ctx->ctl_h->steps_taken >= target_steps) {
+    *evaluated = 1;
+    read_major_eval(ctx, out_current, out_average);
+  } else {
+    if (ctx->ctl_h->error == 0 && ctx->ctl_h->steps_taken == before && spare > 0 && spare < asked) {
+      TRY(enqueue_attempts(ctx, asked - spare));
       TRY(fetch_ctl(ctx, nullptr));
-    }
-    if (++guard > 100000) return fail(-6, "pdlpdev_run: no progress");
-  }
-  if (ctx->rsag && guard > 0) {
-    const int cur = ctx->ctl_h->cur;
-    TRY(all_gather(ctx, ctx->x[cur], (size_t)ctx->slice));
-    TRY(all_gather(ctx, ctx->aty[cur], (size_t)ctx->slice));
-    TRY(all_gather(ctx, ctx->sumx, (size_t)ctx->slice));
-  }
-  if (ctl) *ctl = *ctx->ctl_h;
+      ctx->stat_loop_syncs += 1;
+      TRY(after_round(ctx, before, attempts_before + asked + spare, asked - spare, asked));
+      rounds += 1;
+    }
+    TRY(run_rounds(ctx, target_steps, &rounds));
+  }
+  return run_epilogue(ctx, rounds, ctl);
+}
+
+int pdlpdev_loop_stats(pdlpdev_ctx* ctx, int64_t out[4])
+{
+  out[0] = ctx->stat_eval_reused, out[1] = ctx->stat_eval_product, out[2] = ctx->stat_loop_syncs, out[3] = ctx->stat_empty_attempts;
   return 0;
 }
 
@@ -1052,6 +1146,7 @@
 int pdlpdev_clear_error(pdlpdev_ctx* ctx)
 {
   HIP_TRY(hipSetDevice(ctx->device));
+  ctx->ctl_h_current = false;
   k_clear_error<<<1, 1, 0, ctx->stream>>>(ctx->ctl);
   LAUNCH_CHECK();
   return 0;
@@ -1131,6 +1226,8 @@
     case PDLPDEV_BUF_RC_AVERAGE: src = ctx->rc[1], count = n; break;
     case PDLPDEV_BUF_LAST_RESTART_X: src = ctx->lrx, count = n; break;
     case PDLPDEV_BUF_LAST_RESTART_Y: src = ctx->lry, count = m; break;
+    case PDLPDEV_BUF_ATY_U_CURRENT: src = ctx->aty_u[PDLPDEV_CURRENT], count = n; break;
+    case PDLPDEV_BUF_ATY_U_AVERAGE: src = ctx->aty_u[PDLPDEV_AVERAGE], count = n; break;
     default: fail(-1, "unknown buffer %d", id); return -1;
   }
   *ptr = src;
@@ -1160,6 +1257,7 @@
     return -1;
   }
   count = std::min(count, elements);
+  ctx->aty_valid = false;
   if ((id == PDLPDEV_BUF_LB && ctx->ubd.lb_same) || (id == PDLPDEV_BUF_UB && ctx->ubd.ub_same)) {
     if (id == PDLPDEV_BUF_LB) ctx->ubd.lb_same = 0;
     else ctx->ubd.ub_same = 0;
@@ -1176,6 +1274,7 @@
 int pdlpdev_set_loop_state(pdlpdev_ctx* ctx, double sum_weights, int32_t its_since_restart, int32_t k)
 {
   HIP_TRY(hipSetDevice(ctx->device));
+  loop_state_touched(ctx);
   k_set_loop_state<<<1, 1, 0, ctx->stream>>>(ctx->ctl, sum_weights, its_since_restart, k);
   LAUNCH_CHECK();
   return 0;
@@ -1202,6 +1301,7 @@
   hipStream_t s = ctx->stream;
   if (reps < 1) reps = 1;
   TRY(fetch_ctl(ctx, nullptr));
+  loop_state_touched(ctx);
   pdlpdev_ctl saved = *ctx->ctl_h;
   pdlpdev_ctl forced = saved;
   forced.pending_avg  = 1;
diff --git a/cuopt_amd/csrc/pdlp_eval.hip b/cuopt_amd/csrc/pdlp_eval.hip
--- a/cuopt_amd/csrc/pdlp_eval.hip
+++ b/cuopt_amd/csrc/pdlp_eval.hip
@@ -9,8 +9,10 @@
                const double* __restrict__ x0, const double* __restrict__ x1,
                const double* __restrict__ y0, const double* __restrict__ y1,
                const double* __restrict__ sumx, const double* __restrict__ sumy,
-               double* __restrict__ avgx, double* __restrict__ avgy)
-{
+               double* __restrict__ avgx, double* __restrict__ avgy, int32_t* __restrict__ clear_pending)
+{
+  if (period_guard_skips(ctl, mode)) return;
+  if (clear_pending && blockIdx.x == 0 && threadIdx.x == 0) *clear_pending = 0;
   const int cur = ctl->cur;
   const double* __restrict__ x = cur ? x1 : x0;
   const double* __restrict__ y = cur ? y1 : y0;
@@ -275,32 +277,47 @@
   restart_block(R, blockIdx.x, gridDim.x, red);
 }
 
+__global__ void __launch_bounds__(kBlock)
+k_finalize_eval(const double* __restrict__ part_p, int nb_p, const double* __restrict__ part_d, int nb_d, int with_primal,
+                double* __restrict__ out, const pdlpdev_ctl* __restrict__ ctl, int guard, double* __restrict__ ctl_copy)
+{
+  __shared__ double red[8];
+  static_assert(sizeof(pdlpdev_ctl) % sizeof(int32_t) == 0, "copied word by word");
+  if (ctl_copy && threadIdx.x < sizeof(pdlpdev_ctl) / sizeof(int32_t))
+    reinterpret_cast<int32_t*>(ctl_copy)[threadIdx.x] = reinterpret_cast<const int32_t*>(ctl)[threadIdx.x];
+  if (guard && !period_reached(ctl)) return;
+  if (with_primal) finalize_rows(part_p, nb_p, 3, 0u, out, red);
+  finalize_rows(part_d, nb_d, 4, 0u, out + 4, red);
+}
+
 extern "C" {
 
 int pdlpdev_flush_average(pdlpdev_ctx* ctx)
 {
   HIP_TRY(hipSetDevice(ctx->device));
-  k_flush_average<<<grid_for(std::max(ctx->n, ctx->m)), kBlock, 0, ctx->stream>>>(ctx->n, ctx->m, ctx->ctl, ctx->x[0], ctx->x[1], ctx->y[0], ctx->y[1], ctx->sumx, ctx->sumy);
+  k_flush_average<<<grid_for(std::max(ctx->n, ctx->m)), kBlock, 0, ctx->stream>>>(ctx->n, ctx->m, ctx->ctl, ctx->x[0], ctx->x[1], ctx->y[0], ctx->y[1], ctx->sumx, ctx->sumy, 0);
   k_clear_pending<<<1, 1, 0, ctx->stream>>>(ctx->ctl);
   LAUNCH_CHECK();
+  ctx->ctl_h->pending_avg = 0;
   return 0;
 }
 int pdlpdev_make_average(pdlpdev_ctx* ctx, int mode)
 {
   HIP_TRY(hipSetDevice(ctx->device));
-  k_make_average<<<grid_for(std::max(ctx->n, ctx->m)), kBlock, 0, ctx->stream>>>(ctx->n, ctx->m, mode, ctx->ctl, ctx->x[0], ctx->x[1], ctx->y[0], ctx->y[1], ctx->sumx, ctx->sumy, ctx->avgx, ctx->avgy);
+  k_make_average<<<grid_for(std::max(ctx->n, ctx->m)), kBlock, 0, ctx->stream>>>(ctx->n, ctx->m, mode, ctx->ctl, ctx->x[0], ctx->x[1], ctx->y[0], ctx->y[1], ctx->sumx, ctx->sumy, ctx->avgx, ctx->avgy, nullptr);
   LAUNCH_CHECK();
   return 0;
 }
 
 static int enqueue_eval(pdlpdev_ctx* ctx, int which, int rc_rule_finite_bounds, double eps_rel_primal,
-                        double eps_rel_dual, double* sc)
+                        double eps_rel_dual, double* sc, int guard = 0, double* ctl_copy = nullptr)
 {
   hipStream_t s = ctx->stream;
   const int n = ctx->n, m = ctx->m;
   const double* altx = which == PDLPDEV_LAST_RESTART ? ctx->lrx : ctx->avgx;
   const double* alty = which == PDLPDEV_LAST_RESTART ? ctx->lry : ctx->avgy;
   const int kw       = which == PDLPDEV_CURRENT ? PDLPDEV_CURRENT : PDLPDEV_AVERAGE;
+  const int kwg      = kw | (guard ? kPeriodGuard : 0);
   const bool want_linf = eps_rel_primal >= 0.0 && eps_rel_dual >= 0.0;
   double* linf_m = want_linf ? ctx->tmp_m : nullptr;
   double* linf_n = want_linf ? ctx->tmp_n : nullptr;
@@ -313,17 +330,23 @@
   } else if (ctx->ja.on)
     (void)JAG_LAUNCH(ctx, k_jag_eval_primal, ctx->ja.v, ctx->ctl, kw, ctx->x[0], ctx->x[1], altx, ctx->y[0], ctx->y[1], alty, ctx->dr, ctx->lo_u, ctx->hi_u, eps_rel_primal, linf_m, ctx->ax_u[which], ctx->part_a);
   else if (ctx->pa.on)
-    (ctx->pa.v.seg ? k_panel_eval_primal<true> : k_panel_eval_primal<false>)<<<ctx->pa.v.W, kPanelThreads, 0, s>>>(ctx->pa.v, ctx->ctl, kw, ctx->x[0], ctx->x[1], altx, ctx->y[0], ctx->y[1], alty, ctx->dr, ctx->lo_u, ctx->hi_u, eps_rel_primal, linf_m, ctx->ax_u[which], ctx->part_a);
+    (ctx->pa.v.seg ? k_panel_eval_primal<true> : k_panel_eval_primal<false>)<<<ctx->pa.v.W, kPanelThreads, 0, s>>>(ctx->pa.v, ctx->ctl, kwg, ctx->x[0], ctx->x[1], altx, ctx->y[0], ctx->y[1], alty, ctx->dr, ctx->lo_u, ctx->hi_u, eps_rel_primal, linf_m, ctx->ax_u[which], ctx->part_a);
   else
     k_eval_primal<<<stream_grid(ctx->a_nb), kBlock, 0, s>>>(ctx->a_nb, ctx->a_rb, ctx->ha_off, ctx->ha_idx, ctx->ha_val, ctx->ctl, kw, ctx->x[0], ctx->x[1], altx, ctx->y[0], ctx->y[1], alty, ctx->dr, ctx->lo_u, ctx->hi_u, eps_rel_primal, linf_m, ctx->ax_u[which], ctx->part_a, ctx->dense.add_m);
-  k_finalize<<<1, kBlock, 0, s>>>(ctx->part_a, dual_partials(ctx), 3, 0u, sc + 0);
+  const bool one_finalize = !ctx->comm && !want_linf;
+  if (!one_finalize) k_finalize<<<1, kBlock, 0, s>>>(ctx->part_a, dual_partials(ctx), 3, 0u, sc + 0);
   if (want_linf) {
     const int g = std::min(grid_for(m), kGenericBlocks);
     k_max_partials<<<g, kBlock, 0, s>>>(m, ctx->tmp_m, ctx->part_g);
     k_finalize<<<1, kBlock, 0, s>>>(ctx->part_g, g, 1, 1u, sc + 3);
   }
   EvalDualCore core{nullptr, ctx->dc, ctx->c_u, ctx->lb_u, ctx->ub_u, eps_rel_dual, rc_rule_finite_bounds, which == PDLPDEV_LAST_RESTART ? ctx->rc_scratch : ctx->rc[which == PDLPDEV_AVERAGE ? 1 : 0], linf_n, ctx->aty_u[which]};
-  if (!ctx->comm) {
+  const bool reuse = which == PDLPDEV_CURRENT && ctx->eval_reuse_aty && !ctx->comm && ctx->pat.on && (ctx->aty_valid || guard);
+  if (which == PDLPDEV_CURRENT && !ctx->comm) (reuse ? ctx->stat_eval_reused : ctx->stat_eval_product) += 1;
+  if (reuse) {
+    k_panel_eval_dual_from_aty<<<ctx->pat.v.W, kPanelThreads, 0, s>>>(ctx->pat.v, ctx->ctl, ctx->x[0], ctx->x[1], ctx->aty[0], ctx->aty[1], core, ctx->part_at, guard);
+    k_finalize_eval<<<1, kBlock, 0, s>>>(ctx->part_a, dual_partials(ctx), ctx->part_at, step_partials(ctx), one_finalize ? 1 : 0, sc, ctx->ctl, guard, ctl_copy);
+  } else if (!ctx->comm) {
     if (kw == PDLPDEV_AVERAGE) dense_part(ctx, 1, alty, nullptr, 0, 0);
     else dense_part(ctx, 1, ctx->y[0], ctx->y[1], 2, 0);
     if (ctx->pbat.on) {
@@ -333,10 +356,10 @@
     } else if (ctx->jat.on)
       (void)JAG_LAUNCH(ctx, k_jag_eval_dual, ctx->jat.v, ctx->ctl, kw, ctx->x[0], ctx->x[1], altx, ctx->y[0], ctx->y[1], alty, core, ctx->part_at);
     else if (ctx->pat.on)
-      (ctx->pat.v.seg ? k_panel_eval_dual<true> : k_panel_eval_dual<false>)<<<ctx->pat.v.W, kPanelThreads, 0, s>>>(ctx->pat.v, ctx->ctl, kw, ctx->x[0], ctx->x[1], altx, ctx->y[0], ctx->y[1], alty, core, ctx->part_at);
+      (ctx->pat.v.seg ? k_panel_eval_dual<true> : k_panel_eval_dual<false>)<<<ctx->pat.v.W, kPanelThreads, 0, s>>>(ctx->pat.v, ctx->ctl, kwg, ctx->x[0], ctx->x[1], altx, ctx->y[0], ctx->y[1], alty, core, ctx->part_at);
     else
       k_eval_dual<<<stream_grid(ctx->at_nb), kBlock, 0, s>>>(ctx->at_nb, ctx->at_rb, ctx->hat_off, ctx->hat_idx, ctx->hat_val, ctx->ctl, kw, ctx->x[0], ctx->x[1], altx, ctx->y[0], ctx->y[1], alty, core, ctx->part_at, ctx->dense.add_n);
-    k_finalize<<<1, kBlock, 0, s>>>(ctx->part_at, step_partials(ctx), 4, 0u, sc + 4);
+    k_finalize_eval<<<1, kBlock, 0, s>>>(ctx->part_a, dual_partials(ctx), ctx->part_at, step_partials(ctx), one_finalize ? 1 : 0, sc, ctx->ctl, guard, ctl_copy);
   } else {
     if (kw == PDLPDEV_AVERAGE) {
       launch_plain(ctx, 1, alty, ctx->ar_buf);
@@ -378,15 +401,31 @@
   if (ctx->small_resident && !ctx->comm) {
     TRY(resident_major_eval(ctx, average_mode, rc_rule_finite_bounds, want_linf ? 1 : 0, eps_rel_primal, eps_rel_dual));
   } else {
-    TRY(pdlpdev_flush_average(ctx));
-    TRY(pdlpdev_make_average(ctx, average_mode));
-    TRY(enqueue_eval(ctx, PDLPDEV_CURRENT, rc_rule_finite_bounds, eps_rel_primal, eps_rel_dual, ctx->scal));
-    TRY(enqueue_eval(ctx, PDLPDEV_AVERAGE, rc_rule_finite_bounds, eps_rel_primal, eps_rel_dual, ctx->scal + 32));
+    TRY(enqueue_major_eval(ctx, average_mode, rc_rule_finite_bounds, eps_rel_primal, eps_rel_dual, 0));
     TRY(fetch_scalars(ctx, 41));
+    ctx->stat_loop_syncs += 1;
   }
   read_eval(ctx->scal_h, want_linf, out_current);
   read_eval(ctx->scal_h + 32, want_linf, out_average);
   return 0;
+}
+int enqueue_major_eval(pdlpdev_ctx* ctx, int average_mode, int rc_rule_finite_bounds, double eps_rel_primal, double eps_rel_dual, int guard)
+{
+  hipStream_t s = ctx->stream;
+  const int g   = grid_for(std::max(ctx->n, ctx->m));
+  k_flush_average<<<g, kBlock, 0, s>>>(ctx->n, ctx->m, ctx->ctl, ctx->x[0], ctx->x[1], ctx->y[0], ctx->y[1], ctx->sumx, ctx->sumy, guard);
+  k_make_average<<<g, kBlock, 0, s>>>(ctx->n, ctx->m, average_mode | (guard ? kPeriodGuard : 0), ctx->ctl, ctx->x[0], ctx->x[1], ctx->y[0], ctx->y[1], ctx->sumx,
+                                      ctx->sumy, ctx->avgx, ctx->avgy, &ctx->ctl->pending_avg);
+  LAUNCH_CHECK();
+  if (!guard) ctx->ctl_h->pending_avg = 0;
+  TRY(enqueue_eval(ctx, PDLPDEV_CURRENT, rc_rule_finite_bounds, eps_rel_primal, eps_rel_dual, ctx->scal, guard));
+  TRY(enqueue_eval(ctx, PDLPDEV_AVERAGE, rc_rule_finite_bounds, eps_rel_primal, eps_rel_dual, ctx->scal + 32, guard, guard ? ctx->scal + kCtlSlot : nullptr));
+  return 0;
+}
+void read_major_eval(pdlpdev_ctx* ctx, double* out_current, double* out_average)
+{
+  read_eval(ctx->scal_h, false, out_current);
+  read_eval(ctx->scal_h + 32, false, out_average);
 }
 
 int pdlpdev_eval_infeasibility(pdlpdev_ctx* ctx, int which, int rc_rule_finite_bounds, double out[4])
@@ -511,6 +550,7 @@
   HIP_TRY(hipSetDevice(ctx->device));
   hipStream_t s = ctx->stream;
   const int g = std::min(grid_for(std::max(ctx->n, ctx->m)), kGenericBlocks);
+  loop_state_touched(ctx);
   k_restart<<<g, kBlock, 0, s>>>(ctx->n, ctx->m, which, unscaled_distances, ctx->dc, ctx->dr, ctx->ctl, ctx->x[0], ctx->x[1], ctx->y[0], ctx->y[1], ctx->avgx, ctx->avgy, ctx->lrx, ctx->lry, ctx->sumx, ctx->sumy, ctx->part_g);
   k_finalize<<<1, kBlock, 0, s>>>(ctx->part_g, g, 2, 0u, ctx->scal);
   k_restart_ctl<<<1, 1, 0, s>>>(ctx->ctl);
diff --git a/cuopt_amd/csrc/pdlp_kernel_decls.hpp b/cuopt_amd/csrc/pdlp_kernel_decls.hpp
--- a/cuopt_amd/csrc/pdlp_kernel_decls.hpp
+++ b/cuopt_amd/csrc/pdlp_kernel_decls.hpp
@@ -125,6 +125,10 @@
                   const double* __restrict__ avgx, const double* __restrict__ y0,
                   const double* __restrict__ y1, const double* __restrict__ avgy, EvalDualCore core,
                   double* __restrict__ part);
+__global__ void __launch_bounds__(kPanelThreads)
+k_panel_eval_dual_from_aty(PanelView P, const pdlpdev_ctl* __restrict__ ctl, const double* __restrict__ x0, const double* __restrict__ x1,
+                           const double* __restrict__ aty0, const double* __restrict__ aty1, EvalDualCore core,
+                           double* __restrict__ part, int guard);
 template <int WAVES>
 __global__ void __launch_bounds__(WAVES * 64)
 k_jag_a_dual(JagView J, const pdlpdev_ctl* __restrict__ ctl, const double* __restrict__ xbar,
diff --git a/cuopt_amd/csrc/pdlp_kernels.hpp b/cuopt_amd/csrc/pdlp_kernels.hpp
--- a/cuopt_amd/csrc/pdlp_kernels.hpp
+++ b/cuopt_amd/csrc/pdlp_kernels.hpp
@@ -118,6 +118,14 @@
 __device__ __forceinline__ bool loop_active(const pdlpdev_ctl* ctl)
 {
   return ctl->error == 0 && ctl->steps_taken < ctl->target_steps;
+}
+__device__ __forceinline__ bool period_reached(const pdlpdev_ctl* ctl) { return ctl->steps_taken >= ctl->target_steps; }
+constexpr int kPeriodGuard = 0x100;
+__device__ __forceinline__ bool period_guard_skips(const pdlpdev_ctl* ctl, int& arg)
+{
+  const bool guarded = (arg & kPeriodGuard) != 0;
+  arg &= ~kPeriodGuard;
+  return guarded && !period_reached(ctl);
 }
 
 __device__ __forceinline__ int xcd_remap(int b, int nb)
diff --git a/cuopt_amd/csrc/pdlp_solver.cpp b/cuopt_amd/csrc/pdlp_solver.cpp
--- a/cuopt_amd/csrc/pdlp_solver.cpp
+++ b/cuopt_amd/csrc/pdlp_solver.cpp
@@ -77,6 +77,9 @@
   int32_t iteration_offset = 0;
   int32_t attempt_offset   = 0;
   int32_t major_done_at    = -1;
+  bool fused_eval_ready = false;
+  pdlpdev_small_eval fused_rq{};
+  double fused_ev[PDLPDEV_EV_COUNT] = {}, fused_ev_avg[PDLPDEV_EV_COUNT] = {};
   bool step_error = false, need_aty = true, last_restart_was_average = false;
   double last_candidate_kkt = 0.0, last_restart_kkt = 0.0;
   double gap_reduction_ratio_last_trial = 1.0;
@@ -290,12 +293,12 @@
   ~HostRange() { pdlpdev_range_pop(); }
 };
 
-pdlpdev_small_eval major_eval_request(const cuoptamd_solver* s)
+pdlpdev_small_eval major_eval_request_at(const cuoptamd_solver* s, int32_t total_iterations, int32_t its_since_restart)
 {
   int mode = 2;
-  if (s->total_iterations - s->iteration_offset <= 1 && !s->warm_started)
+  if (total_iterations - s->iteration_offset <= 1 && !s->warm_started)
     mode = 0;
-  else if (s->ctl.its_since_restart == 0)
+  else if (its_since_restart == 0)
     mode = 1;
   pdlpdev_small_eval r;
   r.mode        = mode;
@@ -304,6 +307,7 @@
   r.eps_d = s->S.per_constraint_residual ? s->S.relative_dual_tolerance : -1.0;
   return r;
 }
+pdlpdev_small_eval major_eval_request(const cuoptamd_solver* s) { return major_eval_request_at(s, s->total_iterations, s->ctl.its_since_restart); }
 struct MajorPlan {
   bool restart = false;
   int which = PDLPDEV_CURRENT, unscaled = 0;
@@ -319,7 +323,14 @@
   pdlpdev_ctx* dev = s->dev;
   const pdlpdev_small_eval rq = major_eval_request(s);
   double ev[PDLPDEV_EV_COUNT], ev_avg[PDLPDEV_EV_COUNT];
-  DEV(pdlpdev_major_eval(dev, rq.mode, rq.rule_finite, rq.eps_p, rq.eps_d, ev, ev_avg));
+  const pdlpdev_small_eval& fq = s->fused_rq;
+  if (s->fused_eval_ready && fq.mode == rq.mode && fq.rule_finite == rq.rule_finite && fq.eps_p == rq.eps_p && fq.eps_d == rq.eps_d) {
+    std::copy(s->fused_ev, s->fused_ev + PDLPDEV_EV_COUNT, ev);
+    std::copy(s->fused_ev_avg, s->fused_ev_avg + PDLPDEV_EV_COUNT, ev_avg);
+  } else {
+    DEV(pdlpdev_major_eval(dev, rq.mode, rq.rule_finite, rq.eps_p, rq.eps_d, ev, ev_avg));
+  }
+  s->fused_eval_ready = false;
   MajorPlan plan;
   int rc = major_head(s, ev, ev_avg, terminated, &plan);
   if (rc != 0 || *terminated || !plan.restart) return rc;
@@ -1052,6 +1063,7 @@
 {
   const cuoptamd_result blank{};
   s->total_iterations = 0, s->iteration_offset = 0, s->attempt_offset = 0, s->major_done_at = -1;
+  s->fused_eval_ready = false;
   s->step_error = false, s->need_aty = true, s->last_restart_was_average = false;
   s->last_candidate_kkt = 0.0, s->last_restart_kkt = 0.0, s->gap_reduction_ratio_last_trial = 1.0;
   s->best_quality = cuoptamd_solver::Quality{};
@@ -1206,13 +1218,25 @@
   }
   if (s->finished) return leave(0);
   const int32_t budget_end = advance_budget_end(s, max_new_iterations);
+  const bool period_path   = cuopt_amd::tune_int("period_path", 1) != 0;
   for (;;) {
     int32_t target = 0;
     bool stop      = false;
     int rc         = advance_to_attempts(s, budget_end, &target, &stop);
     if (rc != 0 || stop) return leave(rc);
-    rc = pdlpdev_run(s->dev, target, &s->ctl);
-    if (rc != 0) return leave(fail(rc, "pdlpdev_run: %s", pdlpdev_last_error()));
+    const cuoptamd_hyper& H   = s->H;
+    const int32_t total_after = s->iteration_offset + target;
+    const bool due_at_target  = (total_after % H.major_iteration == 0 && total_after > 0) || total_after <= H.min_iteration_restart;
+    if (period_path && s->world == 1 && !H.artificial_restart_in_main_loop && due_at_target) {
+      s->fused_rq       = major_eval_request_at(s, total_after, s->ctl.its_since_restart + (target - s->ctl.steps_taken));
+      int32_t evaluated = 0;
+      rc = pdlpdev_run_period(s->dev, target, &s->fused_rq, &s->ctl, s->fused_ev, s->fused_ev_avg, &evaluated);
+      if (rc != 0) return leave(fail(rc, "pdlpdev_run_period: %s", pdlpdev_last_error()));
+      s->fused_eval_ready = evaluated != 0;
+    } else {
+      rc = pdlpdev_run(s->dev, target, &s->ctl);
+      if (rc != 0) return leave(fail(rc, "pdlpdev_run: %s", pdlpdev_last_error()));
+    }
     advance_after_attempts(s);
   }
 }
diff --git a/include/cuopt_amd/pdlp_device.h b/include/cuopt_amd/pdlp_device.h
--- a/include/cuopt_amd/pdlp_device.h
+++ b/include/cuopt_amd/pdlp_device.h
@@ -74,6 +74,8 @@
   PDLPDEV_BUF_RC_CURRENT,
   PDLPDEV_BUF_RC_AVERAGE,
   PDLPDEV_BUF_LAST_RESTART_X, PDLPDEV_BUF_LAST_RESTART_Y,
+  PDLPDEV_BUF_ATY_U_CURRENT,
+  PDLPDEV_BUF_ATY_U_AVERAGE,
   PDLPDEV_BUF_COUNT
 };
 
@@ -194,6 +196,9 @@
                  double eps_rel_dual, double out[PDLPDEV_EV_COUNT]);
 int pdlpdev_major_eval(pdlpdev_ctx* ctx, int average_mode, int rc_rule_finite_bounds, double eps_rel_primal,
                        double eps_rel_dual, double out_current[PDLPDEV_EV_COUNT], double out_average[PDLPDEV_EV_COUNT]);
+int pdlpdev_run_period(pdlpdev_ctx* ctx, int32_t target_steps, const pdlpdev_small_eval* rq, pdlpdev_ctl* ctl,
+                       double out_current[PDLPDEV_EV_COUNT], double out_average[PDLPDEV_EV_COUNT], int32_t* evaluated);
+int pdlpdev_loop_stats(pdlpdev_ctx* ctx, int64_t out[4]);
 int pdlpdev_eval_infeasibility(pdlpdev_ctx* ctx, int which, int rc_rule_finite_bounds, double out[4]);
 int pdlpdev_restart(pdlpdev_ctx* ctx, int which, int unscaled_distances, double dist2[2]);
 int pdlpdev_trust_region_bounds(pdlpdev_ctx* ctx, int which, double primal_norm_weight,
```

New measurement: 6089 iterations/s, median of 6. +1.5%, better.
